# ndlongvn/MM-DTI

Measured on AMD Instinct MI355X. Metric: molecules/sec fwd+bwd (InfoNCE fine-tune), higher is better.
Workload: dtype fp16 forward / bf16 backward GEMM operands, fp32 accumulation

## Files before the change

### include/mmdti_hip.h

```cpp
#ifndef MMDTI_HIP_H
#define MMDTI_HIP_H

#ifdef __cplusplus
extern "C" {
#endif

typedef void* mmdti_stream_t;

#define MMDTI_OK 0
#define MMDTI_ERR_INVALID 1
#define MMDTI_ERR_LAUNCH 2

#define MMDTI_ACT_NONE 0
#define MMDTI_ACT_GELU 1
#define MMDTI_ACT_GELU_BWD 2
#define MMDTI_ACT_GELU_G 4
#define MMDTI_ACT_MUL_AUX 5

#define MMDTI_DT_F32 0
#define MMDTI_DT_BF16 1
#define MMDTI_DT_F32_ATOMIC 2
#define MMDTI_DT_F16 3
#define MMDTI_DT_AB_F16 16
#define MMDTI_DT_B_F16 32
// ... 105 lines not shown
                               float p_hid, float p_att, unsigned long long seed, unsigned int site_att, unsigned int site_o,
                               unsigned int site_f, const float* dout, float* ds1, float* ds2, const float* key_add,
                               const int* q_off, const int* k_off, const int* k_cnt, int q_rows, const void* q, const void* kv,
                               const float* stats, const float* y, const float* am, const float* ar, const void* u_aux,
                               int act_dx, const float* z, const float* zm, const float* zr, const void* w_q, const void* w_kv,
                               const void* w_o, const void* w_i, const void* w_o2, const float* g_ln1, const float* g_ln2,
                               float* db_o, float* db_o2, float* dg_ln1, float* dbt_ln1, float* dg_ln2, float* dbt_ln2, void* dzb,
                               void* du, void* dyb, void* dq, void* dkv, void* ws, long long ws_bytes);
int mmdti_bert_stack_layout(int Mq, int D, int F, long long stats_bytes, long long nrow, long long dw_slab_bytes, long long* out);
int mmdti_bert_stack_fwd(mmdti_stream_t stream, int nl, int Mq, int B, int L, int heads, int D, int F, float scale, float p_hid,
                         float p_att, unsigned long long seed, unsigned int site0, const float* s1_32_0, const void* s1_16_0,
                         const float* key_add, const int* q_off, const int* k_off, const int* k_cnt, int q_rows,
                         const void* const* params, int act_fwd, float eps, int ln_max_k, void* arena, long long arena_bytes,
                         long long stats_bytes, float* out32_last, int fwd_f16);
int mmdti_bert_stack_bwd(mmdti_stream_t stream, int nl, int Mq, int B, int L, int heads, int D, int F, float scale, float p_hid,
                         float p_att, unsigned long long seed, unsigned int site0, const float* dout, float* ds1_final,
                         const void* s1_16_0, const float* key_add, const int* q_off, const int* k_off, const int* k_cnt,
                         int q_rows, const void* const* bparams, int act_dx, void* const* grads, int lddw_qkv, const void* arena,
                         long long arena_bytes, long long stats_bytes, void* ws, long long ws_bytes, long long dw_slab_bytes,
                         int fwd_f16);


int mmdti_layernorm_fwd(mmdti_stream_t stream, const float* x, const float* gamma, const float* beta, float eps,
                        int rows, int D, float* y_f32, void* y_bf16, float* mean, float* rstd,
                        const unsigned char* row_zero, float drop_p, unsigned long long seed, unsigned int site,
                        int y16_f16 );
int mmdti_layernorm_bwd(mmdti_stream_t stream, const void* dy, int dy_dtype, const float* dy_add, const float* x, const float* gamma,
                        const float* mean, const float* rstd, int rows, int D, const float* dres, float* dx,
                        float* dgamma, float* dbeta, const unsigned char* row_zero, float drop_p,
                        unsigned long long seed, unsigned int site, void* dx_bf16, float drop2_p, unsigned int site2,
                        float* dx_colsum);

int mmdti_colsum_bf16(mmdti_stream_t stream, const void* x_bf16, int rows, int cols, int ld, float* out);
int mmdti_cast_f32_bf16(mmdti_stream_t stream, const float* x, void* y_bf16, long long n, float drop_p,
                        unsigned long long seed, unsigned int site);
int mmdti_cast_bf16_f32(mmdti_stream_t stream, const void* x_bf16, float* y, long long n);
int mmdti_cast_f32_f16(mmdti_stream_t stream, const float* x, void* y_f16, long long n, float drop_p, unsigned long long seed,
                       unsigned int site);
int mmdti_cast_f16_bf16(mmdti_stream_t stream, const void* x_f16, int rows, int cols, int ldx, void* y_bf16);
int mmdti_dropout_f32(mmdti_stream_t stream, const float* x, float* y, long long n, float drop_p,
                      unsigned long long seed, unsigned int site);
int mmdti_axpy_f32(mmdti_stream_t stream, const float* x, float* y, long long n, float a);

int mmdti_embedding_fwd(mmdti_stream_t stream, const long long* ids, const float* table, long long n, int D,
                        int vocab, float* out, int accumulate);
int mmdti_embedding_bwd(mmdti_stream_t stream, const long long* ids, const float* dout, long long n, int D,
                        int vocab, long long padding_idx, float* dtable);
int mmdti_embedding_fwd3(mmdti_stream_t stream, const long long* ids_a, const float* table_a, int vocab_a, const long long* ids_b,
                         const float* table_b, int vocab_b, const long long* ids_c, const float* table_c, int vocab_c, long long n, int D,
                         float* out);
int mmdti_onehot_bf16(mmdti_stream_t stream, const long long* ids, long long n, int vocab, int ld, long long padding_idx,
                      void* out_bf16);
int mmdti_roberta_position_ids(mmdti_stream_t stream, const long long* ids, int B, int L, long long pad_idx,
                               long long* out);

int mmdti_gbf_features_fwd(mmdti_stream_t stream, const float* dist, const long long* edge_type, const float* mul,
                           const float* bias, const float* means, const float* stds, long long P, int K, int E,
                           void* feat_bf16);
int mmdti_gbf_features_bwd(mmdti_stream_t stream, const float* dist, const long long* edge_type, const float* mul,
                           const float* bias, const float* means, const float* stds, long long P, int K, int E,
                           const void* dfeat_bf16, float* dmul, float* dbias, float* dmeans, float* dstds);
int mmdti_gbf_bias_fwd(mmdti_stream_t stream, const float* dist, const void* edge_type,
                       int edge_bytes , const float* mul,
                       const float* bias, const float* means, const float* stds, const void* w1_bf16, const float* b1,
                       const void* w2_bf16, const float* b2, int B, int N, int ld, int K, int F, int H, int E, void* out,
                       void* feat_bf16, void* u_bf16, void* h_bf16, int flags ,
                       const int* tile_prefix ,
                       const int* row_blocks );
int mmdti_gbf_bias_bwd(mmdti_stream_t stream, const void* g, const float* dist, const void* edge_type, int edge_bytes,
                       const float* mul, const float* bias, const float* means, const float* stds, const void* w1_bf16,
                       const void* w2_bf16, const void* u_bf16, int B, int N, int ld, int K, int F, int H, int E, int flags,
                       void* do_bf16, void* du_bf16, float* dmul, float* dbias, float* dmeans, float* dstds);
int mmdti_gbf_bias_bwd_full(mmdti_stream_t stream, const void* g, const float* dist, const void* edge_type, int edge_bytes,
                            const float* mul, const float* bias, const float* means, const float* stds, const void* w1_bf16,
                            const float* b1, const void* w2_bf16, int B, int N, int ld, int K, int F, int H, int E, int flags,
                            float* dw1, float* db1, float* dw2, float* db2, float* dmul, float* dbias, float* dmeans, float* dstds,
                            const int* tile_prefix ,
                            const int* row_blocks ,
                            void* workspace ,
                            long long workspace_bytes);
int mmdti_gbf_bias_bwd_full_workspace(int E);
int mmdti_pair_permute_fwd(mmdti_stream_t stream, const float* x, float* out, int B, int N, int H, int ld);
int mmdti_pair_permute_bwd(mmdti_stream_t stream, const float* g, void* out_bf16, int B, int N, int H, int ld, int tiled);

int mmdti_pair_attn_fwd(mmdti_stream_t stream, const void* qkv_bf16, const void* bias_in, void* s_out,
                        void* o_bf16, const unsigned char* key_pad, int B, int N, int H, int ld, float scale,
                        float drop_p, unsigned long long seed, unsigned int site, int layout,
                        const int* key_tiles ,
                        int rag_store,
                        const int* row_off ,
                        int qkv_f16 );
int mmdti_pair_attn_bwd(mmdti_stream_t stream, const void* qkv_bf16, const void* s, const void* do_bf16, void* g,
                        void* dqkv_bf16, int B, int N, int H, int ld, float scale, int g_in_zero, float drop_p,
                        unsigned long long seed, unsigned int site, int layout, const int* key_tiles,
                        const int* row_off ,
                        int qkv_f16 );

int mmdti_softmax_fwd(mmdti_stream_t stream, const float* s, const float* key_add, void* p_bf16, void* pd_bf16,
                      int B, int heads, int Lq, int Lk, int ld, float drop_p, unsigned long long seed,
                      unsigned int site);
int mmdti_softmax_bwd(mmdti_stream_t stream, const void* p_bf16, const float* dp, void* ds_bf16, int B, int heads,
                      int Lq, int Lk, int ld, float scale, float drop_p, unsigned long long seed,
                      unsigned int site);

int mmdti_attn_fwd(mmdti_stream_t stream, const void* q_bf16, const void* k_bf16, const void* v_bf16,
                   const float* key_add, void* ctx_bf16, float* stats, int B, int heads, int Lq, int Lk, int head_dim,
                   int ldq, int ldk, int ldo, float scale, float drop_p, unsigned long long seed, unsigned int site,
                   const int* q_off, const int* k_off, const int* k_cnt, int q_rows ,
                   int ctx_f16 );
int mmdti_attn_bwd(mmdti_stream_t stream, const void* q_bf16, const void* k_bf16, const void* v_bf16,
                   const float* key_add, const void* dctx_bf16, const float* stats, float* drow, void* dq_bf16,
                   void* dk_bf16, void* dv_bf16, int B, int heads, int Lq, int Lk, int head_dim, int ldq, int ldk, int ldo,
                   int lddq, int lddk, float scale, float drop_p, unsigned long long seed, unsigned int site,
                   const int* q_off, const int* k_off, const int* k_cnt, int q_rows );
int mmdti_attn_long_fwd(mmdti_stream_t stream, const void* q_bf16, const void* k_bf16, const void* v_bf16,
                        const float* key_add, void* ctx_bf16, float* stats, int B, int heads, int Lq, int Lk, int head_dim,
                        int ldq, int ldk, int ldo, float scale, float drop_p, unsigned long long seed, unsigned int site,
                        const int* q_off, const int* k_off, const int* k_cnt, int q_rows, int ctx_f16);
int mmdti_attn_long_bwd(mmdti_stream_t stream, const void* q_bf16, const void* k_bf16, const void* v_bf16,
                        const float* key_add, const void* dctx_bf16, const float* stats, float* drow, void* dq_bf16,
                        void* dk_bf16, void* dv_bf16, int B, int heads, int Lq, int Lk, int head_dim, int ldq, int ldk, int ldo,
                        int lddq, int lddk, float scale, float drop_p, unsigned long long seed, unsigned int site,
                        const int* q_off, const int* k_off, const int* k_cnt, int q_rows);

int mmdti_gelu_fwd_bf16(mmdti_stream_t stream, const void* u_bf16, void* y_bf16, long long n);

int mmdti_seq_mean_fwd(mmdti_stream_t stream, const void* x_bf16, int B, int S, int D, int ld, float* out);
int mmdti_seq_mean_bwd(mmdti_stream_t stream, const float* dout, int B, int S, int D, int ld, void* dx_bf16, const void* aux_bf16,
                       int ld_aux, int aux_mode);
int mmdti_seq_mean_packed_fwd(mmdti_stream_t stream, const void* x_bf16, int B, int S, int D, int ld, const int* row_off,
                              const int* n_real, float* out);
int mmdti_seq_mean_packed_bwd(mmdti_stream_t stream, const float* dout, int rows, int S, int D, int ld, const int* row_off,
                              const int* n_real, const int* row_seq, void* dx_bf16, const void* aux_bf16, int ld_aux, int aux_mode);
int mmdti_l2norm_fwd(mmdti_stream_t stream, const float* x, int B, int D, int ldx, float* xhat, float* inv_norm);
int mmdti_l2norm_bwd(mmdti_stream_t stream, const float* dxhat, const float* xhat, const float* inv_norm, int B,
                     int D, int ldx, float* dx);
int mmdti_infonce_dir(mmdti_stream_t stream, const float* qh_all, const float* kh_all, int Bg, int D, int row0,
                      int Bl, float temperature, float* loss_sum, float* dq_all, float* dk_all, float* scratch);

int mmdti_ct_loss_fwd(mmdti_stream_t stream, int mode, const float* fhat, int B, int D, const float* labels_f,
                      const long long* labels_i, int C, const float* pred, const float* weights, float w, float t,
                      float e, float coef, float* loss, float* G,
                      float* row_ws );
int mmdti_ct_loss_bwd(mmdti_stream_t stream, const float* fhat, const float* G, int B, int D, float t, float* dfhat);

int mmdti_fds_bins(mmdti_stream_t stream, const float* labels, int n, float min_value, float bin_width,
                   int bucket_start, int bucket_num, int* bins, int* flags);
int mmdti_fds_smooth(mmdti_stream_t stream, const float* x, const int* bins, const int* flags, int n, int D,
                     int bucket_start, int bucket_num, const float* m1, const float* v1, const float* m2,
                     const float* v2, float* y, float* scale_out);
int mmdti_fds_update_stats(mmdti_stream_t stream, const float* feats, const int* bins, const int* flags, int n,
                           int D, int bucket_start, int bucket_num, float factor, float* running_mean,
                           float* running_var, float* num_samples_tracked);
int mmdti_fds_smooth_stats(mmdti_stream_t stream, const float* stat, int nb, int D, const float* window, int ks,
                           float* out);

int mmdti_masked_pool_fwd(mmdti_stream_t stream, const float* a, const float* t, const unsigned char* mask_a,
                          const unsigned char* mask_t, int B, int Na, int Nt, int D, float* pooled);
int mmdti_masked_pool_bwd(mmdti_stream_t stream, const float* dpooled, const unsigned char* mask_a,
                          const unsigned char* mask_t, int B, int Na, int Nt, int D, float* da, float* dt);

int mmdti_masked_pool_packed_fwd(mmdti_stream_t stream, const float* a, const float* t, const int* a_off, const int* a_cnt,
                                 const int* t_off, const int* t_cnt, int B, int D, float* pooled);
int mmdti_masked_pool_packed_bwd(mmdti_stream_t stream, const float* dpooled, const int* a_off, const int* a_cnt, const int* a_seq,
                                 int rows_a, const int* t_off, const int* t_cnt, const int* t_seq, int rows_t, int D, float* da,
                                 float* dt);
// ... 40 lines not shown
```

### mm-dti_amd/csrc/common.h

```cpp
#pragma once
#include <hip/hip_runtime.h>
#include <stdint.h>
#include <math.h>

#include "../../include/mmdti_hip.h"

namespace mmdti {

typedef uint16_t bf16_t;

void set_error(const char* fmt, ...);
#define MMDTI_REQUIRE(cond, ...)                 \
  do {                                           \
    if (!(cond)) {                               \
      ::mmdti::set_error(__VA_ARGS__);           \
      return MMDTI_ERR_INVALID;                  \
    }                                            \
  } while (0)
#define MMDTI_LAUNCH_CHECK()                                              \
  do {                                                                    \
    hipError_t e__ = hipGetLastError();                                   \
    if (e__ != hipSuccess) {                                              \
      ::mmdti::set_error("%s:%d launch failed: %s", __FILE__, __LINE__,   \
                         hipGetErrorString(e__));                         \
// ... 16 lines not shown
  return __builtin_bit_cast(uint32_t, v);
}
__device__ __forceinline__ uint16_t f2h_sat(float f) { return (uint16_t)(f2h_sat2(f, f) & 0xffffu); }
__device__ __forceinline__ uint4 h2bf8(const uint4& u) {
  typedef _Float16 f16x8_t __attribute__((ext_vector_type(8)));
  typedef __bf16 bf16x8_t __attribute__((ext_vector_type(8)));
  const f16x8_t h = __builtin_bit_cast(f16x8_t, u);
  bf16x8_t o;
#pragma unroll
  for (int e = 0; e < 8; ++e) o[e] = (__bf16)(float)h[e];
  return __builtin_bit_cast(uint4, o);
}

template <int CTRL, int ROW_MASK = 0xf, int BANK_MASK = 0xf, bool BOUND_ZERO = true>
__device__ __forceinline__ float dpp_f32(float old, float src) {
  return __int_as_float(__builtin_amdgcn_update_dpp(__float_as_int(old), __float_as_int(src), CTRL, ROW_MASK, BANK_MASK, BOUND_ZERO));
}
constexpr int DPP_ROW_SHL = 0x100, DPP_ROW_SHR = 0x110, DPP_ROW_ROR = 0x120, DPP_ROW_BCAST15 = 0x142, DPP_ROW_BCAST31 = 0x143;
constexpr int DPP_QUAD_XOR1 = 0xB1, DPP_QUAD_XOR2 = 0x4E;

__device__ __forceinline__ float wave_sum(float v) {
  v += dpp_f32<DPP_ROW_SHR + 1>(0.f, v);
  v += dpp_f32<DPP_ROW_SHR + 2>(0.f, v);
  v += dpp_f32<DPP_ROW_SHR + 4>(0.f, v);
  v += dpp_f32<DPP_ROW_SHR + 8>(0.f, v);
  v += dpp_f32<DPP_ROW_BCAST15, 0xa>(0.f, v);
  v += dpp_f32<DPP_ROW_BCAST31, 0xc>(0.f, v);
  return __int_as_float(__builtin_amdgcn_readlane(__float_as_int(v), 63));
}
__device__ __forceinline__ float wave_max(float v) {
  const float NI = -INFINITY;
  v = fmaxf(v, dpp_f32<DPP_ROW_SHR + 1, 0xf, 0xf, false>(NI, v));
  v = fmaxf(v, dpp_f32<DPP_ROW_SHR + 2, 0xf, 0xf, false>(NI, v));
  v = fmaxf(v, dpp_f32<DPP_ROW_SHR + 4, 0xf, 0xf, false>(NI, v));
  v = fmaxf(v, dpp_f32<DPP_ROW_SHR + 8, 0xf, 0xf, false>(NI, v));
  v = fmaxf(v, dpp_f32<DPP_ROW_BCAST15, 0xa, 0xf, false>(NI, v));
  v = fmaxf(v, dpp_f32<DPP_ROW_BCAST31, 0xc, 0xf, false>(NI, v));
  return __int_as_float(__builtin_amdgcn_readlane(__float_as_int(v), 63));
}
__device__ __forceinline__ float wave_sum8_scatter(const float (&v)[8], int lane) {
  const bool b0 = lane & 1, b1 = lane & 2, b2 = lane & 4;
  float a[4];
#pragma unroll
  for (int i = 0; i < 4; ++i) {
    const float keep = b0 ? v[2 * i + 1] : v[2 * i];
    const float send = b0 ? v[2 * i] : v[2 * i + 1];
    a[i] = keep + dpp_f32<DPP_QUAD_XOR1>(0.f, send);
  }
  float b[2];
#pragma unroll
  for (int i = 0; i < 2; ++i) {
    const float keep = b1 ? a[2 * i + 1] : a[2 * i];
    const float send = b1 ? a[2 * i] : a[2 * i + 1];
    b[i] = keep + dpp_f32<DPP_QUAD_XOR2>(0.f, send);
  }
  const float keep = b2 ? b[1] : b[0];
  const float send = b2 ? b[0] : b[1];
  const float up = dpp_f32<DPP_ROW_SHL + 4>(0.f, send);
  const float dn = dpp_f32<DPP_ROW_SHR + 4>(0.f, send);
  float c = keep + (b2 ? dn : up);
  c += dpp_f32<DPP_ROW_ROR + 8>(0.f, c);
  c += __shfl_xor(c, 16, 64);
  c += __shfl_xor(c, 32, 64);
  return c;
}

struct Rand4 {
  uint32_t x, y, z, w;
};
static __device__ unsigned long long g_seed_salt = 0ull;
__device__ __forceinline__ uint64_t salted(uint64_t seed) { return seed ^ g_seed_salt; }
#define MMDTI_DEFINE_SALT_PULL(TU)                                                                                   \
  namespace mmdti {                                                                                                  \
  __global__ void seed_salt_pull_kernel_##TU(const unsigned long long* __restrict__ src) { g_seed_salt = *src; }     \
  void salt_pull_##TU(hipStream_t s, const unsigned long long* src) {                                                \
    hipLaunchKernelGGL(seed_salt_pull_kernel_##TU, dim3(1), dim3(1), 0, s, src);                                     \
  }                                                                                                                  \
  }
void salt_pull_gemm(hipStream_t s, const unsigned long long* src);
void salt_pull_layernorm(hipStream_t s, const unsigned long long* src);
void salt_pull_pair_attn(hipStream_t s, const unsigned long long* src);
void salt_pull_pair_attn_bwd(hipStream_t s, const unsigned long long* src);
void salt_pull_pair_attn_bwd_g16(hipStream_t s, const unsigned long long* src);
void salt_pull_attn(hipStream_t s, const unsigned long long* src);
void salt_pull_elementwise(hipStream_t s, const unsigned long long* src);
__device__ __forceinline__ uint32_t mix32(uint32_t x) {
  x ^= x >> 16; x *= 0x7feb352du; x ^= x >> 15; x *= 0x846ca68bu; x ^= x >> 16;
  return x;
}
__device__ __forceinline__ Rand4 philox4(uint64_t seed, uint32_t site, uint64_t ctr) {
  seed = salted(seed);
  const uint32_t k = mix32((uint32_t)seed ^ (site * 0x9E3779B9u)) ^ (uint32_t)(seed >> 32);
  const uint32_t a = mix32(((uint32_t)ctr ^ k) + (uint32_t)(ctr >> 32) * 0x85EBCA6Bu);
  const uint32_t b = mix32(a ^ 0xB5297A4Du);
  return Rand4{a << 16, a & 0xffff0000u, b << 16, b & 0xffff0000u};
}
__device__ __forceinline__ bool dropout_keep(uint64_t seed, uint32_t site, uint64_t idx, uint32_t thresh) {
  Rand4 r = philox4(seed, site, idx >> 2);
  uint32_t w = (idx & 3) == 0 ? r.x : (idx & 3) == 1 ? r.y : (idx & 3) == 2 ? r.z : r.w;
  return w >= thresh;
}
struct Rng24 {
  uint32_t k1, k2;
};
__device__ __forceinline__ Rng24 rng24_key(uint64_t seed, uint32_t site, uint32_t plane) {
  seed = salted(seed);
  const uint32_t a = mix32((mix32((uint32_t)seed ^ (site * 0x9E3779B9u)) ^ (uint32_t)(seed >> 32)) + plane * 0x85EBCA6Bu);
  return Rng24{a, mix32(a ^ 0xB5297A4Du)};
}
__device__ __forceinline__ uint32_t rng24_word(const Rng24& k, uint32_t ctr) {
  uint32_t h = __umul24(ctr ^ k.k1, 0x9E3779u);
  h = h ^ (h >> 12) ^ k.k2;
  h = __umul24(h, 0x85EBCBu);
  return h ^ (h >> 12);
}
__device__ __forceinline__ uint32_t rng24_row_t8(const Rng24& k, uint32_t row, uint32_t thresh8) {
  return (thresh8 >> 16) + ((rng24_word(k, row | 0x800000u) & 0xffffu) < (thresh8 & 0xffffu) ? 1u : 0u);
}
__device__ __forceinline__ bool rng24_kept(uint32_t word, int r, uint32_t t8) { return ((word >> (8 * r)) & 0xffu) >= t8; }
static inline uint32_t dropout_thresh8(float p) {
  if (!(p > 0.f)) return 0u;
  const double x = (double)p * 256.0;
  uint32_t t8 = (uint32_t)x, fr = (uint32_t)((x - (double)t8) * 65536.0 + 0.5);
  if (fr >= 65536u) { t8 += 1; fr = 0; }
  return (t8 << 16) | fr;
}
static inline uint32_t dropout_thresh(float p) {
  if (p <= 0.f) return 0u;
  double t = (double)p * 4294967296.0;
  if (t >= 4294967295.0) return 0xFFFFFFFFu;
  return (uint32_t)t;
}

__host__ __device__ __forceinline__ int pair_n4(int N) { return (N + 3) & ~3; }
__host__ __device__ __forceinline__ long long pair_plane(int N) { return ((long long)N * pair_n4(N) + 7) & ~7ll; }
__host__ __device__ __forceinline__ long long pair_off(int N, int i, int j) {
  const int q0 = i & ~15, vr = N - q0 < 16 ? N - q0 : 16;
  return (long long)q0 * pair_n4(N) + vr * (j & ~3) + ((i & 15) << 2) + (j & 3);
}

__device__ __forceinline__ float fast_erf(float x) {
  const float ax = fabsf(x);
  const float t = __builtin_amdgcn_rcpf(1.0f + 0.3275911f * ax);
  const float poly = ((((1.061405429f * t - 1.453152027f) * t + 1.421413741f) * t - 0.284496736f) * t + 0.254829592f) * t;
  const float r = 1.0f - poly * __expf(-ax * ax);
  return copysignf(r, x);
}
__device__ __forceinline__ float gelu_erf(float x) { return x * 0.5f * (1.0f + fast_erf(x * 0.70710678118654752440f)); }
__device__ __forceinline__ float gelu_erf_grad(float x) {
  const float kInvSqrt2Pi = 0.39894228040143267794f;
  const float ax = fabsf(x) * 0.70710678118654752440f;
  const float t = __builtin_amdgcn_rcpf(1.0f + 0.3275911f * ax);
  const float poly = ((((1.061405429f * t - 1.453152027f) * t + 1.421413741f) * t - 0.284496736f) * t + 0.254829592f) * t;
  const float e = __expf(-ax * ax);
  const float erfv = copysignf(1.0f - poly * e, x);
  return 0.5f * (1.0f + erfv) + x * kInvSqrt2Pi * e;
}

__device__ __forceinline__ int xcd_chunk(int orig, int nwg) {
  const int q = nwg >> 3, r = nwg & 7, xcd = orig & 7;
  return (xcd < r ? xcd * (q + 1) : r * (q + 1) + (xcd - r) * q) + (orig >> 3);
}

__device__ __forceinline__ void gelu_erf_both(float x, float& y, float& dy) {
  const float kInvSqrt2Pi = 0.39894228040143267794f;
  const float ax = fabsf(x) * 0.70710678118654752440f;
// ... 54 lines not shown
```

### mm-dti_amd/csrc/elementwise.hip

```cpp
#include "common.h"
#include <stdarg.h>
#include <stdio.h>

namespace mmdti {

static thread_local char g_err[512] = "";
void set_error(const char* fmt, ...) {
  va_list ap;
  va_start(ap, fmt);
  vsnprintf(g_err, sizeof(g_err), fmt, ap);
  va_end(ap);
}

static inline int grid_for(long long n, int per_block) {
  long long b = (n + per_block - 1) / per_block;
  if (b > 256 * 16) b = 256 * 16;
  if (b < 1) b = 1;
  return (int)b;
}

__device__ __forceinline__ bf16_t f2h16(float f) { return f2h_sat(f); }

template <bool F16>
__global__ __launch_bounds__(256) void cast_f32_bf16_kernel(const float* __restrict__ x, bf16_t* __restrict__ y,
// ... 813 lines not shown
  return MMDTI_OK;
}

extern "C" int mmdti_adam_step(mmdti_stream_t stream, float* p, const float* g, float* m, float* v, void* p_bf16,
                               long long n, float lr, float beta1, float beta2, float eps, float weight_decay,
                               int step, const float* grad_scale_dev, const float* step_state_dev, void* p_f16) {
  MMDTI_REQUIRE(p && g && m && v && n > 0 && (step >= 1 || step_state_dev), "adam_step: bad arguments");
  float bc1, bc2s;
  adam_bias_host(beta1, beta2, step, &bc1, &bc2s);
  hipLaunchKernelGGL(adam_kernel<false>, dim3(grid_for(n, 256 * 4)), dim3(256), 0, (hipStream_t)stream, p, g, m, v,
                     (bf16_t*)p_bf16, (bf16_t*)p_f16, n, lr, beta1, beta2, eps, weight_decay, bc1, bc2s, grad_scale_dev, step_state_dev, nullptr);
  MMDTI_LAUNCH_CHECK();
  return MMDTI_OK;
}

extern "C" int mmdti_sumsq_check_f32(mmdti_stream_t stream, const float* g, long long n, float* out, float* ws, int ws_floats, float* guard,
                                     const float* bias_table, int table_steps, float beta1, float beta2) {
  MMDTI_REQUIRE(g && out && ws && n > 0 && ws_floats >= 2, "sumsq_check_f32: bad arguments");
  MMDTI_REQUIRE(aligned16(g), "sumsq_check_f32: 16-byte alignment required");
  MMDTI_REQUIRE(!bias_table || table_steps >= 1, "sumsq_check_f32: empty bias-correction table");
  const int wgs = (int)min((long long)min(ws_floats / 2, SUMSQ_WGS), (n / 4 + 255) / 256 + 1);
  unsigned* cnt = reinterpret_cast<unsigned*>(ws + wgs);
  hipLaunchKernelGGL(sumsq_part_kernel<true>, dim3(wgs), dim3(256), 0, (hipStream_t)stream, g, n, ws, cnt);
  hipLaunchKernelGGL(sumsq_fold_kernel<true>, dim3(1), dim3(256), 0, (hipStream_t)stream, ws, wgs, out, cnt, guard, bias_table,
                     table_steps, beta1, beta2);
  MMDTI_LAUNCH_CHECK();
  return MMDTI_OK;
}

extern "C" int mmdti_adam_step_guarded(mmdti_stream_t stream, float* p, const float* g, float* m, float* v, void* p_bf16, long long n,
                                       float lr, float beta1, float beta2, float eps, float weight_decay, const float* grad_scale_dev,
                                       const float* step_state_dev, void* p_f16, const float* guard) {
  MMDTI_REQUIRE(p && g && m && v && n > 0 && guard, "adam_step_guarded: bad arguments");
  hipLaunchKernelGGL(adam_kernel<true>, dim3(grid_for(n, 256 * 4)), dim3(256), 0, (hipStream_t)stream, p, g, m, v,
                     (bf16_t*)p_bf16, (bf16_t*)p_f16, n, lr, beta1, beta2, eps, weight_decay, 1.f, 1.f, grad_scale_dev, step_state_dev,
                     guard);
  MMDTI_LAUNCH_CHECK();
  return MMDTI_OK;
}

extern "C" int mmdti_adam_step_masked(mmdti_stream_t stream, float* p, const float* g, float* m, float* v, void* p_bf16, long long n,
                                      float lr, float beta1, float beta2, float eps, float weight_decay, int step,
                                      const float* grad_scale_dev, const float* step_state_dev, void* p_f16, const float* guard,
                                      const unsigned char* skip) {
  MMDTI_REQUIRE(p && g && m && v && n > 0 && skip && (guard || step >= 1 || step_state_dev), "adam_step_masked: bad arguments");
  if (guard) {
    hipLaunchKernelGGL((adam_kernel<true, true>), dim3(grid_for(n, 256 * 4)), dim3(256), 0, (hipStream_t)stream, p, g, m, v,
                       (bf16_t*)p_bf16, (bf16_t*)p_f16, n, lr, beta1, beta2, eps, weight_decay, 1.f, 1.f, grad_scale_dev, step_state_dev,
                       guard, skip);
  } else {
    float bc1, bc2s;
    adam_bias_host(beta1, beta2, step, &bc1, &bc2s);
    hipLaunchKernelGGL((adam_kernel<false, true>), dim3(grid_for(n, 256 * 4)), dim3(256), 0, (hipStream_t)stream, p, g, m, v,
                       (bf16_t*)p_bf16, (bf16_t*)p_f16, n, lr, beta1, beta2, eps, weight_decay, bc1, bc2s, grad_scale_dev, step_state_dev,
                       nullptr, skip);
  }
  MMDTI_LAUNCH_CHECK();
  return MMDTI_OK;
}

extern "C" int mmdti_adam_bias_table(float beta1, float beta2, int steps, float* table_host) {
  MMDTI_REQUIRE(table_host && steps >= 1, "adam_bias_table: bad arguments");
  for (int t = 1; t <= steps; ++t) adam_bias_host(beta1, beta2, t, &table_host[2 * (t - 1)], &table_host[2 * (t - 1) + 1]);
  return MMDTI_OK;
}

extern "C" int mmdti_step_state_advance(mmdti_stream_t stream, float* state, unsigned long long* salt, float base_lr, int warmup_steps,
                                        int total_steps, float beta1, float beta2) {
  MMDTI_REQUIRE(state && salt, "step_state_advance: null pointer");
  MMDTI_REQUIRE(total_steps > 0 && warmup_steps >= 0, "step_state_advance: bad schedule");
  hipLaunchKernelGGL(step_state_advance_kernel, dim3(1), dim3(1), 0, (hipStream_t)stream, state, salt, base_lr, warmup_steps, total_steps, beta1, beta2);
  MMDTI_LAUNCH_CHECK();
  return MMDTI_OK;
}

extern "C" int mmdti_seed_salt_pull(mmdti_stream_t stream, const unsigned long long* salt) {
  MMDTI_REQUIRE(salt != nullptr, "seed_salt_pull: null pointer");
  hipStream_t s = (hipStream_t)stream;
  salt_pull_gemm(s, salt);
  salt_pull_layernorm(s, salt);
  salt_pull_pair_attn(s, salt);
  salt_pull_pair_attn_bwd(s, salt);
  salt_pull_pair_attn_bwd_g16(s, salt);
  salt_pull_attn(s, salt);
  salt_pull_elementwise(s, salt);
  MMDTI_LAUNCH_CHECK();
  return MMDTI_OK;
}

extern "C" int mmdti_probe_tr_read(mmdti_stream_t stream, int row_stride_elems, unsigned short* out) {
  MMDTI_REQUIRE(out && row_stride_elems >= 16 && row_stride_elems <= 64 && row_stride_elems % 4 == 0, "probe_tr_read: bad stride");
  hipLaunchKernelGGL(probe_tr_kernel, dim3(1), dim3(64), 0, (hipStream_t)stream, row_stride_elems, out);
  MMDTI_LAUNCH_CHECK();
  return MMDTI_OK;
}
```

### mm-dti_amd/csrc/gbf.hip

```cpp
#include "common.h"

namespace mmdti {

constexpr float GBF_A = 2.5066272160f;

__global__ __launch_bounds__(256) void gbf_fwd_kernel(const float* __restrict__ dist, const long long* __restrict__ et,
                                                      const float* __restrict__ mul, const float* __restrict__ bias,
                                                      const float* __restrict__ means, const float* __restrict__ stds,
                                                      long long P, int K, int E, bf16_t* __restrict__ feat) {
  const int kc = threadIdx.x & 15;
  const int pl = threadIdx.x >> 4;
  for (int k0 = kc * 8; k0 < K; k0 += 128) {
    float mu[8], sg[8], cf[8];
#pragma unroll
    for (int i = 0; i < 8; ++i) {
      mu[i] = means[k0 + i];
      sg[i] = fabsf(stds[k0 + i]) + 1e-5f;
      cf[i] = 1.0f / (GBF_A * sg[i]);
    }
    for (long long p = (long long)blockIdx.x * 16 + pl; p < P; p += (long long)gridDim.x * 16) {
      long long e = et[p];
      e = e < 0 ? 0 : (e >= E ? E - 1 : e);
      const float y = mul[e] * dist[p] + bias[e];
      uint32_t w[4];
#pragma unroll
      for (int i = 0; i < 4; ++i) {
        float z0 = (y - mu[2 * i]) / sg[2 * i], z1 = (y - mu[2 * i + 1]) / sg[2 * i + 1];
        float v0 = __expf(-0.5f * z0 * z0) * cf[2 * i], v1 = __expf(-0.5f * z1 * z1) * cf[2 * i + 1];
        w[i] = (uint32_t)f2bf(v0) | ((uint32_t)f2bf(v1) << 16);
      }
      *reinterpret_cast<uint4*>(feat + p * K + k0) = make_uint4(w[0], w[1], w[2], w[3]);
    }
  }
}

constexpr int GBF_MAXE = 4096;

__global__ __launch_bounds__(256) void gbf_bwd_kernel(const float* __restrict__ dist, const long long* __restrict__ et,
                                                      const float* __restrict__ mul, const float* __restrict__ bias,
                                                      const float* __restrict__ means, const float* __restrict__ stds,
                                                      long long P, int K, int E, const bf16_t* __restrict__ dfeat,
                                                      float* __restrict__ dmul, float* __restrict__ dbias,
                                                      float* __restrict__ dmeans, float* __restrict__ dstds) {
  extern __shared__ float hist[];
  const bool use_hist = E <= GBF_MAXE;
  if (use_hist) {
    for (int i = threadIdx.x; i < 2 * E; i += 256) hist[i] = 0.f;
    __syncthreads();
  }
  const int kc = threadIdx.x & 15, pl = threadIdx.x >> 4;
  for (int kb = 0; kb < K; kb += 128) {
    const int k0 = kb + kc * 8;
    const bool kact = k0 < K;
    float mu[8], sg[8], cf[8], amu[8], asg[8];
#pragma unroll
    for (int i = 0; i < 8; ++i) {
      mu[i] = kact ? means[k0 + i] : 0.f;
      sg[i] = kact ? fabsf(stds[k0 + i]) + 1e-5f : 1.f;
      cf[i] = 1.0f / (GBF_A * sg[i]);
      amu[i] = asg[i] = 0.f;
    }
    for (long long p0 = (long long)blockIdx.x * 16; p0 < P; p0 += (long long)gridDim.x * 16) {
      const long long p = p0 + pl;
      float dy = 0.f;
      long long e = 0;
      float d = 0.f;
      if (p < P && kact) {
        e = et[p];
        e = e < 0 ? 0 : (e >= E ? E - 1 : e);
        d = dist[p];
        const float y = mul[e] * d + bias[e];
        const uint4 u = *reinterpret_cast<const uint4*>(dfeat + p * K + k0);
        const uint32_t w[4] = {u.x, u.y, u.z, u.w};
#pragma unroll
        for (int i = 0; i < 8; ++i) {
          const float dv = __uint_as_float((i & 1) ? (w[i >> 1] & 0xffff0000u) : (w[i >> 1] << 16));
          const float z = (y - mu[i]) / sg[i];
          const float val = __expf(-0.5f * z * z) * cf[i];
          const float t = dv * val;
          const float zs = z / sg[i];
          dy -= t * zs;
          amu[i] += t * zs;
          asg[i] += t * (z * zs - 1.0f / sg[i]);
// ... 41 lines not shown
  const float* src = x + (long long)bi * N * H;
  const int HP = H + 1;
  for (int t = threadIdx.x; t < N * H; t += 256) tile[(t / H) * HP + (t % H)] = src[t];
  __syncthreads();
  for (int t = threadIdx.x; t < H * N; t += 256) {
    const int h = t / N, j = t - h * N;
    out[(((long long)b * H + h) * N + i) * ld + j] = tile[j * HP + h];
  }
}

__global__ __launch_bounds__(256) void pair_permute_bwd_kernel(const float* __restrict__ g, bf16_t* __restrict__ out,
                                                               int N, int H, int ld, int tiled) {
  extern __shared__ float tile[];
  const int bi = blockIdx.x, b = bi / N, i = bi - b * N;
  const int NP = N | 1;
  for (int t = threadIdx.x; t < H * N; t += 256) {
    const int h = t / N, j = t - h * N;
    const long long off = tiled ? (long long)(b * H + h) * pair_plane(N) + pair_off(N, i, j) : (((long long)b * H + h) * N + i) * ld + j;
    tile[h * NP + j] = g[off];
  }
  __syncthreads();
  bf16_t* dst = out + (long long)bi * N * H;
  for (int t = threadIdx.x; t < N * H; t += 256) {
    const int j = t / H, h = t - j * H;
    dst[t] = f2bf(tile[h * NP + j]);
  }
}

typedef __bf16 gbf16x8 __attribute__((ext_vector_type(8)));
typedef float gf32x4 __attribute__((ext_vector_type(4)));
constexpr int GBF_K = 128, GBF_F = 128, GBF_H = 64;
constexpr int GBF_WS = 136;

__device__ __forceinline__ gbf16x8 gbf_pack8(const float* v) {
  gbf16x8 r;
#pragma unroll
  for (int e = 0; e < 8; ++e) r[e] = (__bf16)v[e];
  return r;
}
__device__ __forceinline__ uint2 gbf_pack4(const gf32x4& a) {
  uint2 pk;
  pk.x = (uint32_t)f2bf(a[0]) | ((uint32_t)f2bf(a[1]) << 16);
  pk.y = (uint32_t)f2bf(a[2]) | ((uint32_t)f2bf(a[3]) << 16);
  return pk;
}

__device__ __forceinline__ int gbf_edge(const void* et, long long base, unsigned off, int esz) {
  const char* pb = reinterpret_cast<const char*>(et) + base * esz;
  const unsigned bo = off * (unsigned)esz;
  const int w = *reinterpret_cast<const int*>(pb + (bo & ~3u));
  return esz == 2 ? (int)(short)(w >> ((bo & 2u) * 8u)) : w;
}
__device__ __forceinline__ int gbf_edge(const void* et, long long p, int esz) { return gbf_edge(et, p, 0u, esz); }

typedef float gf32x2 __attribute__((ext_vector_type(2)));
constexpr float GBF_SQ = 0.84932180028801907f;

__device__ __forceinline__ gbf16x8 gbf_basis8(float y, const float* mu, const float* isq, const float* cf) {
  const gf32x4 m0 = *reinterpret_cast<const gf32x4*>(mu), m1 = *reinterpret_cast<const gf32x4*>(mu + 4);
  const gf32x4 s0 = *reinterpret_cast<const gf32x4*>(isq), s1 = *reinterpret_cast<const gf32x4*>(isq + 4);
  const gf32x4 c0 = *reinterpret_cast<const gf32x4*>(cf), c1 = *reinterpret_cast<const gf32x4*>(cf + 4);
  const gf32x2 yy = {y, y};
  float v[8];
#define GBF_B2(M, S, C, LO, OUT)                                                       \
  {                                                                                    \
    const gf32x2 z = (yy - gf32x2{M[LO], M[LO + 1]}) * gf32x2{S[LO], S[LO + 1]};       \
    const gf32x2 q = -(z * z);                                                         \
    const gf32x2 e = {__builtin_amdgcn_exp2f(q[0]), __builtin_amdgcn_exp2f(q[1])};     \
    const gf32x2 r = e * gf32x2{C[LO], C[LO + 1]};                                     \
    v[OUT] = r[0]; v[OUT + 1] = r[1];                                                  \
  }
  GBF_B2(m0, s0, c0, 0, 0) GBF_B2(m0, s0, c0, 2, 2) GBF_B2(m1, s1, c1, 0, 4) GBF_B2(m1, s1, c1, 2, 6)
#undef GBF_B2
  return gbf_pack8(v);
}

constexpr int GBF_FWD_MAXE = 4096;
__device__ __forceinline__ void gbf_put(float* p, float v) { *p = v; }
__device__ __forceinline__ void gbf_put(_Float16* p, float v) { *p = (_Float16)fminf(v, 65504.f); }
__device__ __forceinline__ float gbf_get(const float* p) { return *p; }
__device__ __forceinline__ float gbf_get(const __bf16* p) {
  return __builtin_bit_cast(float, (uint32_t)(*reinterpret_cast<const unsigned short*>(p)) << 16);
}

template <bool SAVE, bool TILED, typename OT>
__global__ __launch_bounds__(512, 2) void gbf_bias_fwd_kernel(const float* __restrict__ dist, const void* __restrict__ et, int esz,
                                                              const float* __restrict__ mul, const float* __restrict__ bias,
                                                              const float* __restrict__ means, const float* __restrict__ stds,
                                                              const bf16_t* __restrict__ W1, const float* __restrict__ b1,
                                                              const bf16_t* __restrict__ W2, const float* __restrict__ b2,
                                                              OT* __restrict__ out, bf16_t* __restrict__ feat_out,
                                                              bf16_t* __restrict__ u_out, bf16_t* __restrict__ h_out, int B, int N,
                                                              int ld, int E, int tpm, int ugrad, int ltab,
                                                              const int* __restrict__ tile_prefix, const int* __restrict__ row_blocks) {
  static_assert(TILED || sizeof(OT) == 4, "compact pair planes exist in the tiled layout only");
  extern __shared__ __attribute__((aligned(16))) unsigned char gbf_smem[];
  bf16_t* sW1 = reinterpret_cast<bf16_t*>(gbf_smem);
  bf16_t* sW2 = sW1 + GBF_F * GBF_WS;
  float* sMu = reinterpret_cast<float*>(sW2 + GBF_H * GBF_WS);
  float* sIq = sMu + GBF_K;
  float* sCf = sIq + GBF_K;
  float* sB1 = sCf + GBF_K;
  float* sB2 = sB1 + GBF_F;
  float* sMul = sB2 + GBF_H;
  float* sBia = sMul + E;
  const int tid = threadIdx.x, lane = tid & 63;
  for (int c = tid; c < GBF_F * (GBF_K / 8); c += 512) {
    const int row = c >> 4, col = (c & 15) * 8;
    *reinterpret_cast<uint4*>(sW1 + row * GBF_WS + col) = *reinterpret_cast<const uint4*>(W1 + row * GBF_K + col);
  }
  for (int c = tid; c < GBF_H * 32; c += 512) {
    const int row = c >> 5, pc = c & 31, u = pc >> 3, g = (pc >> 1) & 3, hf = pc & 1;
    *reinterpret_cast<uint2*>(sW2 + row * GBF_WS + 32 * u + 8 * g + 4 * hf) =
        *reinterpret_cast<const uint2*>(W2 + row * GBF_F + 32 * u + 16 * hf + 4 * g);
  }
  if (tid < GBF_K) {
    const float sg = fabsf(stds[tid]) + 1e-5f;
    sMu[tid] = means[tid];
    sIq[tid] = GBF_SQ / sg;
    sCf[tid] = 1.0f / (GBF_A * sg);
    sB1[tid] = b1[tid];
    if (tid < GBF_H) sB2[tid] = b2[tid];
  }
  if (ltab)
    for (int c = tid; c < E; c += 512) {
      sMul[c] = mul[c];
      sBia[c] = bias[c];
    }
  __syncthreads();
  const int g = lane >> 4, i = lane & 15;
  const bool rag = TILED && tile_prefix != nullptr;
  const int ntiles = rag ? tile_prefix[B] : B * tpm;
  const int nwaves = (int)gridDim.x * 8;
  int b_run = 0;
  const int nblk = (N + 3) >> 2;
  const long long plane = TILED ? pair_plane(N) : (long long)N * ld;
  auto fetch = [&](int tile, int& b, int& q, int& flags, unsigned& pl, int& e, float& d) {
    tile = __builtin_amdgcn_readfirstlane(tile < ntiles ? tile : ntiles - 1);
    int tq;
    if (rag) {
      while (b_run + 1 < B && tile >= tile_prefix[b_run + 1]) ++b_run;
      b = b_run;
      tq = tile - tile_prefix[b];
    } else {
      b = (int)((unsigned)tile / (unsigned)tpm);
      tq = tile - b * tpm;
    }
    int ii, jj;
    bool inplane = true, past = false;
    if (TILED) {
      const int rbk = (rag && row_blocks) ? row_blocks[b] : nblk;
      const int cb = (int)((unsigned)tq / (unsigned)rbk), rb = tq - cb * rbk;
      past = 4 * rb >= N || 4 * cb >= N;
      ii = 4 * rb + (i >> 2);
      jj = 4 * cb + (i & 3);
      inplane = ii < N;
      q = (int)pair_off(N, inplane ? ii : 0, jj);
    } else {
      q = tq * 16 + i;
      ii = (int)((unsigned)q / (unsigned)ld);
      jj = q - ii * ld;
      inplane = q < plane;
    }
    const bool valid = ii < N && jj < N;
    flags = (valid ? 1 : 0) | (inplane ? 2 : 0) | (past ? 4 : 0);
    pl = (unsigned)((valid ? ii : 0) * N + (valid ? jj : 0));
// ... 218 lines not shown
    float dy = 0.f;
#pragma unroll
    for (int kt = 0; kt < 8; ++kt) {
      gf32x4 acc = {0.f, 0.f, 0.f, 0.f};
#pragma unroll
      for (int u = 0; u < 4; ++u) {
        const gbf16x8 wf = *reinterpret_cast<const gbf16x8*>(sW1T + (16 * kt + i) * GBF_WS + 32 * u + 8 * g);
        acc = __builtin_amdgcn_mfma_f32_16x16x32_bf16(wf, uB[u], acc, 0, 0, 0);
      }
      const gf32x4 mu = *reinterpret_cast<const gf32x4*>(sMu + 16 * kt + 4 * g);
      const gf32x4 is = *reinterpret_cast<const gf32x4*>(sIs + 16 * kt + 4 * g);
      const gf32x4 cf = *reinterpret_cast<const gf32x4*>(sCf + 16 * kt + 4 * g);
#pragma unroll
      for (int r = 0; r < 4; ++r) {
        const float dvr = __uint_as_float(((uint32_t)f2bf(acc[r])) << 16);
        const float z = (y - mu[r]) * is[r];
        const float val = __expf(-0.5f * z * z) * cf[r];
        const float t = valid ? dvr * val : 0.f;
        const float zs = z * is[r];
        dy -= t * zs;
        amu[kt][r] += t * zs;
        asg[kt][r] += t * (z * zs - is[r]);
      }
      __builtin_amdgcn_sched_barrier(0);
    }
    dy += __shfl_xor(dy, 16, 64);
    dy += __shfl_xor(dy, 32, 64);
    if (g == 0 && valid) {
      atomicAdd(&hist[e], dy * d);
      atomicAdd(&hist[E + e], dy);
    }
    }
    act = n_act; valid = n_valid; p = n_p; e = n_e; d = n_d;
#pragma unroll
    for (int j = 0; j < 16; ++j) gv[j] = n_gv[j];
#pragma unroll
    for (int j = 0; j < 8; ++j) upre[j] = n_up[j];
  }
#pragma unroll
  for (int kt = 0; kt < 8; ++kt)
#pragma unroll
    for (int r = 0; r < 4; ++r) {
      float a = amu[kt][r], sgv = asg[kt][r];
      a += __shfl_xor(a, 1, 64); a += __shfl_xor(a, 2, 64); a += __shfl_xor(a, 4, 64); a += __shfl_xor(a, 8, 64);
      sgv += __shfl_xor(sgv, 1, 64); sgv += __shfl_xor(sgv, 2, 64); sgv += __shfl_xor(sgv, 4, 64); sgv += __shfl_xor(sgv, 8, 64);
      if (i == 0) {
        const int k = 16 * kt + 4 * g + r;
        atomicAdd(dmeans + k, a);
        atomicAdd(dstds + k, stds[k] < 0.f ? -sgv : sgv);
      }
    }
  __syncthreads();
  for (int c = tid; c < E; c += 256) {
    const float a = hist[c], bb = hist[E + c];
    if (a != 0.f) atomicAdd(dmul + c, a);
    if (bb != 0.f) atomicAdd(dbias + c, bb);
  }
}

constexpr int GBF_LW = 144;
constexpr int GBF_FULL_MAXE = 1536;
constexpr int GBF_SLAB_B1 = GBF_F * GBF_K + GBF_H * GBF_F, GBF_SLAB_B2 = GBF_SLAB_B1 + GBF_F, GBF_SLAB_MU = GBF_SLAB_B2 + GBF_H,
              GBF_SLAB_SG = GBF_SLAB_MU + GBF_K, GBF_SLAB = GBF_SLAB_SG + GBF_K;
constexpr size_t gbf_full_smem(int E) {
  return (size_t)(GBF_F * GBF_LW + GBF_F * GBF_W2S + 2 * 128 * GBF_LW) * 2 + (size_t)(4 * GBF_K + GBF_F + 2 * 128 + 4 * E) * 4;
}

typedef short gs16x4 __attribute__((ext_vector_type(4)));
typedef short gs16x8 __attribute__((ext_vector_type(8)));
typedef __attribute__((address_space(3))) gs16x4 glds_s16x4;
__device__ __forceinline__ gbf16x8 gbf_tr8(const bf16_t* a0, const bf16_t* a1) {
  const gs16x4 lo = __builtin_amdgcn_ds_read_tr16_b64_v4i16((glds_s16x4*)a0);
  const gs16x4 hi = __builtin_amdgcn_ds_read_tr16_b64_v4i16((glds_s16x4*)a1);
  const gs16x8 v = __builtin_shufflevector(lo, hi, 0, 1, 2, 3, 4, 5, 6, 7);
  return __builtin_bit_cast(gbf16x8, v);
}

template <bool TILED, typename GT>
__global__ __launch_bounds__(512, 1) void gbf_bias_bwd_full_kernel(
    const GT* __restrict__ gsrc, const float* __restrict__ dist, const void* __restrict__ et, int esz, const float* __restrict__ mul,
    const float* __restrict__ bias, const float* __restrict__ means, const float* __restrict__ stds, const bf16_t* __restrict__ W1,
    const float* __restrict__ b1, const bf16_t* __restrict__ W2, float* __restrict__ dW1, float* __restrict__ db1, float* __restrict__ dW2,
    float* __restrict__ db2, float* __restrict__ dmul, float* __restrict__ dbias, float* __restrict__ dmeans, float* __restrict__ dstds, int B,
    int N, int ld, int E, int tpm, const int* __restrict__ tile_prefix, const int* __restrict__ row_blocks, float* __restrict__ slab) {
  extern __shared__ __attribute__((aligned(16))) unsigned char gbf_smem[];
  bf16_t* sW1 = reinterpret_cast<bf16_t*>(gbf_smem);
  bf16_t* sW2T = sW1 + GBF_F * GBF_LW;
  bf16_t* T0 = sW2T + GBF_F * GBF_W2S;
  bf16_t* T1 = T0 + 128 * GBF_LW;
  float* sMu = reinterpret_cast<float*>(T1 + 128 * GBF_LW);
  float* sIs = sMu + GBF_K;
  float* sCf = sIs + GBF_K;
  float* sIq = sCf + GBF_K;
  float* sB1 = sIq + GBF_K;
  float* sY = sB1 + GBF_F;
  float* sDy = sY + 128;
  float* hist = sDy + 128;
  float* sMul = hist + 2 * E;
  float* sBia = sMul + E;
  const int tid = threadIdx.x, lane = tid & 63, wave = tid >> 6;
  for (int c = tid; c < E; c += 512) {
    sMul[c] = mul[c];
    sBia[c] = bias[c];
  }
  for (int c = tid; c < GBF_F * (GBF_K / 8); c += 512) {
    const int row = c >> 4, col = (c & 15) * 8;
    *reinterpret_cast<uint4*>(sW1 + row * GBF_LW + col) = *reinterpret_cast<const uint4*>(W1 + row * GBF_K + col);
  }
  for (int c = tid; c < GBF_H * GBF_F; c += 512) {
    const int h = c >> 7, f = c & 127;
    sW2T[f * GBF_W2S + h] = W2[c];
  }
  if (tid < GBF_K) {
    const float sg = fabsf(stds[tid]) + 1e-5f;
    sMu[tid] = means[tid];
    sIs[tid] = 1.0f / sg;
    sCf[tid] = 1.0f / (GBF_A * sg);
    sIq[tid] = GBF_SQ / sg;
    sB1[tid] = b1[tid];
    sDy[tid] = 0.f;
  }
  for (int c = tid; c < 2 * E; c += 512) hist[c] = 0.f;
  __syncthreads();
  const int g = lane >> 4, i = lane & 15;
  const int ploc = 16 * wave + i;
  const int pswz = ((ploc >> 3) & 1) << 6;
#define GBF_SWZ(lo, hi, c) ((c) < 64 ? (lo) + (c) : (hi) + ((c) - 64))
  bf16_t* const r0lo = T0 + ploc * GBF_LW + pswz;
  bf16_t* const r0hi = T0 + ploc * GBF_LW + (64 ^ pswz);
  bf16_t* const r1lo = r0lo + 128 * GBF_LW;
  bf16_t* const r1hi = r0hi + 128 * GBF_LW;
  const int tswz = (g & 1) << 6;
  const int trow = (8 * g + (i >> 2)) * GBF_LW + 4 * (i & 3);
  const bf16_t* const t0lo = T0 + trow + tswz;
  const bf16_t* const t0hi = T0 + trow + (64 ^ tswz);
  const bf16_t* const t1lo = t0lo + 128 * GBF_LW;
  const bf16_t* const t1hi = t0hi + 128 * GBF_LW;
  const bf16_t* const t0w = T0 + trow + ((16 * wave) ^ tswz);
  const bf16_t* const t1w = t0w + 128 * GBF_LW;
  const int rswz = ((i >> 3) & 1) << 6;
  const bf16_t* const d1lo = T1 + i * GBF_LW + 8 * g + rswz;
  const bf16_t* const d1hi = T1 + i * GBF_LW + 8 * g + (64 ^ rswz);
  unsigned o_w1row = (unsigned)(i * GBF_LW + 8 * g) * 2;
  unsigned o_w2row = (unsigned)(GBF_F * GBF_LW + i * GBF_W2S + 8 * g) * 2;
  unsigned o_w1tr = (unsigned)((8 * g + (i >> 2)) * GBF_LW + 16 * wave + 4 * (i & 3)) * 2;
  const unsigned o_f32 = (unsigned)(GBF_F * GBF_LW + GBF_F * GBF_W2S + 2 * 128 * GBF_LW) * 2;
  unsigned o_gconst = o_f32 + (unsigned)(8 * g) * 4;
  unsigned o_b1row = o_f32 + (unsigned)(4 * GBF_K + 4 * g) * 4;
  unsigned o_kconst = o_f32 + (unsigned)(16 * wave + 4 * g) * 4;
  const bool rag = TILED && tile_prefix != nullptr;
  const int ntiles = rag ? tile_prefix[B] : B * tpm;
  int b_run = 0;
  const int nb = (N + 3) >> 2;
  const long long plane = TILED ? pair_plane(N) : (long long)N * ld;
  gf32x4 amu = {0.f, 0.f, 0.f, 0.f}, asg = {0.f, 0.f, 0.f, 0.f};
  gf32x4 aW1[8], aW2[4], aB1 = {0.f, 0.f, 0.f, 0.f}, aB2 = {0.f, 0.f, 0.f, 0.f};
#pragma unroll
  for (int t = 0; t < 8; ++t) aW1[t] = gf32x4{0.f, 0.f, 0.f, 0.f};
#pragma unroll
  for (int t = 0; t < 4; ++t) aW2[t] = gf32x4{0.f, 0.f, 0.f, 0.f};
  const gs16x8 o16 = {0x3F80, 0x3F80, 0x3F80, 0x3F80, 0x3F80, 0x3F80, 0x3F80, 0x3F80};
  const gbf16x8 ones = __builtin_bit_cast(gbf16x8, o16);

  auto fetch = [&](int tile, bool& act, bool& valid, float& d, int& e, float (&gv)[16]) {
    tile = __builtin_amdgcn_readfirstlane(tile);
    act = tile < ntiles;
    tile = act ? tile : ntiles - 1;
    int b, tq;
    if (rag) {
      while (b_run + 1 < B && tile >= tile_prefix[b_run + 1]) ++b_run;
      b = b_run;
      tq = tile - tile_prefix[b];
    } else {
      b = (int)((unsigned)tile / (unsigned)tpm);
      tq = tile - b * tpm;
    }
    int q, ii, jj;
    if (TILED) {
      const int rbk = (rag && row_blocks) ? row_blocks[b] : nb;
      const int cb = (int)((unsigned)tq / (unsigned)rbk), rb = tq - cb * rbk;
      ii = 4 * rb + (i >> 2);
      jj = 4 * cb + (i & 3);
      q = (int)pair_off(N, ii < N ? ii : 0, jj);
    } else {
      q = tq * 16 + i;
      ii = (int)((unsigned)q / (unsigned)ld);
      jj = q - ii * ld;
    }
    valid = act && ii < N && jj < N;
    const long long mol = (long long)b * N * N;
    const unsigned pl = (unsigned)((valid ? ii : 0) * N + (valid ? jj : 0));
    const int e32 = gbf_edge(et, mol, pl, esz);
    e = e32 < 0 ? 0 : (e32 >= E ? E - 1 : e32);
    d = (dist + mol)[pl];
    const GT* mb = gsrc + (long long)b * GBF_H * plane;
    const unsigned voff = (unsigned)(8 * g) * (unsigned)plane + (unsigned)(valid ? q : 0);
#pragma unroll
    for (int c = 0; c < 2; ++c)
#pragma unroll
      for (int j = 0; j < 8; ++j) gv[c * 8 + j] = gbf_get(mb + (long long)(32 * c + j) * plane + voff);
  };

  bool act, valid, n_act, n_valid;
  float d, n_d, gv[16], n_gv[16];
  int e, n_e;
  const int stride = (int)gridDim.x * 8;
  int tile = (int)blockIdx.x * 8 + wave;
  fetch(tile, act, valid, d, e, gv);
  for (int base = (int)blockIdx.x * 8; base < ntiles; base += stride, tile += stride) {
    asm volatile("" : "+v"(o_w1row), "+v"(o_w2row), "+v"(o_w1tr), "+v"(o_gconst), "+v"(o_b1row), "+v"(o_kconst));
    const bf16_t* w1row = reinterpret_cast<const bf16_t*>(gbf_smem + o_w1row);
    const bf16_t* w2row = reinterpret_cast<const bf16_t*>(gbf_smem + o_w2row);
    const bf16_t* w1tr = reinterpret_cast<const bf16_t*>(gbf_smem + o_w1tr);
    const float* gconst = reinterpret_cast<const float*>(gbf_smem + o_gconst);
    const float* b1row = reinterpret_cast<const float*>(gbf_smem + o_b1row);
    const float* kconst = reinterpret_cast<const float*>(gbf_smem + o_kconst);
    fetch(tile + stride, n_act, n_valid, n_d, n_e, n_gv);
    constexpr bool SPLIT_G = sizeof(GT) == 4;
    gbf16x8 oB[2], oL[2], hB[4];
    if (!valid) {
#pragma unroll
      for (int j = 0; j < 16; ++j) gv[j] = 0.f;
    }
    oB[0] = gbf_pack8(gv);
    oB[1] = gbf_pack8(gv + 8);
    if constexpr (SPLIT_G) {
      float lo[16];
#pragma unroll
      for (int j = 0; j < 16; ++j) lo[j] = gv[j] - (float)oB[j >> 3][j & 7];
      oL[0] = gbf_pack8(lo);
      oL[1] = gbf_pack8(lo + 8);
    }
    const float y = sMul[e] * d + sBia[e];
    if (g == 0) sY[ploc] = y;
    if (act) {
      gbf16x8 fB[4];
#pragma unroll
      for (int c = 0; c < 4; ++c) {
        const float* gc = gconst + 32 * c;
        fB[c] = gbf_basis8(y, gc, gc + 3 * GBF_K, gc + 2 * GBF_K);
        *reinterpret_cast<gbf16x8*>(GBF_SWZ(r0lo, r0hi, 32 * c) + 8 * g) = fB[c];
      }
#pragma unroll
      for (int u = 0; u < 4; ++u) {
        gf32x4 hv[2];
#pragma unroll
        for (int hf = 0; hf < 2; ++hf) {
          const int ft = 2 * u + hf;
          gf32x4 acc = {0.f, 0.f, 0.f, 0.f}, ua = {0.f, 0.f, 0.f, 0.f};
#pragma unroll
          for (int c = 0; c < 2; ++c) {
            const gbf16x8 wf = *reinterpret_cast<const gbf16x8*>(w2row + 16 * ft * GBF_W2S + 32 * c);
            acc = __builtin_amdgcn_mfma_f32_16x16x32_bf16(wf, oB[c], acc, 0, 0, 0);
            if constexpr (SPLIT_G) acc = __builtin_amdgcn_mfma_f32_16x16x32_bf16(wf, oL[c], acc, 0, 0, 0);
          }
#pragma unroll
          for (int c = 0; c < 4; ++c) {
            const gbf16x8 wf = *reinterpret_cast<const gbf16x8*>(w1row + 16 * ft * GBF_LW + 32 * c);
            ua = __builtin_amdgcn_mfma_f32_16x16x32_bf16(wf, fB[c], ua, 0, 0, 0);
          }
          ua += *reinterpret_cast<const gf32x4*>(b1row + 16 * ft);
          {
            f32x2_t y0, g0, y1, g1;
            gelu_erf_both2(f32x2_t{ua[0], ua[1]}, y0, g0);
            gelu_erf_both2(f32x2_t{ua[2], ua[3]}, y1, g1);
            hv[hf] = gf32x4{y0[0], y0[1], y1[0], y1[1]};
            const uint2 gb = gbf_pack4(gf32x4{g0[0], g0[1], g1[0], g1[1]});
            acc[0] *= __uint_as_float(gb.x << 16);
            acc[1] *= __uint_as_float(gb.x & 0xffff0000u);
            acc[2] *= __uint_as_float(gb.y << 16);
            acc[3] *= __uint_as_float(gb.y & 0xffff0000u);
          }
          *reinterpret_cast<uint2*>(GBF_SWZ(r1lo, r1hi, 16 * ft) + 4 * g) = gbf_pack4(acc);
          __builtin_amdgcn_sched_barrier(0);
        }
        float w[8] = {hv[0][0], hv[0][1], hv[0][2], hv[0][3], hv[1][0], hv[1][1], hv[1][2], hv[1][3]};
        hB[u] = gbf_pack8(w);
      }
    } else {
      const uint4 z4 = make_uint4(0u, 0u, 0u, 0u);
#pragma unroll
      for (int c = 0; c < 4; ++c) {
        *reinterpret_cast<uint4*>(GBF_SWZ(r0lo, r0hi, 32 * c) + 8 * g) = z4;
        *reinterpret_cast<uint4*>(GBF_SWZ(r1lo, r1hi, 32 * c) + 8 * g) = z4;
        hB[c] = __builtin_bit_cast(gbf16x8, z4);
      }
    }
    __syncthreads();
#define GBF_TFRAG(P, S) gbf_tr8((P) + 32 * (S) * GBF_LW, (P) + (32 * (S) + 4) * GBF_LW)
#pragma unroll
    for (int sstep = 0; sstep < 4; ++sstep) {
      const gbf16x8 fa = GBF_TFRAG(t1w, sstep);
      aB1 = __builtin_amdgcn_mfma_f32_16x16x32_bf16(fa, ones, aB1, 0, 0, 0);
#pragma unroll
      for (int kb = 0; kb < 8; ++kb) {
        const gbf16x8 fb = GBF_TFRAG(GBF_SWZ(t0lo, t0hi, 16 * kb), sstep);
        aW1[kb] = __builtin_amdgcn_mfma_f32_16x16x32_bf16(fa, fb, aW1[kb], 0, 0, 0);
      }
    }
    {
      gbf16x8 wfr[4];
// ... 283 lines not shown
                GBF_K, GBF_F, GBF_H, K, F, H);
  MMDTI_REQUIRE(B > 0 && N > 0 && ld >= N && ld % 4 == 0 && E > 0, "gbf_bias_fwd: bad shape");
  MMDTI_REQUIRE(aligned16(w1_bf16) && aligned16(w2_bf16) && aligned16(out), "gbf_bias_fwd: 16-byte alignment required");
  const bool save = feat_bf16 || u_bf16 || h_bf16;
  MMDTI_REQUIRE(!save || (feat_bf16 && u_bf16 && h_bf16 && aligned16(feat_bf16) && aligned16(u_bf16) && aligned16(h_bf16)),
                "gbf_bias_fwd: the three saved intermediates come together, 16-byte aligned");
  const int nb4 = (N + 3) / 4;
  const int tpm = tiled ? nb4 * nb4 : cdiv((long long)N * ld, 16);
  const long long ntiles = (long long)B * tpm;
  MMDTI_REQUIRE(ntiles < (1ll << 30) && (long long)N * N < (1ll << 30), "gbf_bias_fwd: batch too large for 32-bit tile indices");
  const int grid = (int)((ntiles + 7) / 8 < 512 ? (ntiles + 7) / 8 : 512);
  const int ltab = E <= GBF_FWD_MAXE ? 1 : 0;
  const size_t smem = (size_t)(GBF_F + GBF_H) * GBF_WS * 2 + (size_t)(3 * GBF_K + GBF_F + GBF_H + (ltab ? 2 * E : 0)) * 4;
  static bool attr_done = false;
  if (!attr_done) {
    const int cap = (int)((size_t)(GBF_F + GBF_H) * GBF_WS * 2 + (size_t)(3 * GBF_K + GBF_F + GBF_H + 2 * GBF_FWD_MAXE) * 4);
    const void* fns[6] = {reinterpret_cast<const void*>(gbf_bias_fwd_kernel<true, true, float>), reinterpret_cast<const void*>(gbf_bias_fwd_kernel<true, false, float>),
                          reinterpret_cast<const void*>(gbf_bias_fwd_kernel<false, true, float>), reinterpret_cast<const void*>(gbf_bias_fwd_kernel<false, false, float>),
                          reinterpret_cast<const void*>(gbf_bias_fwd_kernel<true, true, _Float16>), reinterpret_cast<const void*>(gbf_bias_fwd_kernel<false, true, _Float16>)};
    for (int f = 0; f < 6; ++f)
      if (hipFuncSetAttribute(fns[f], hipFuncAttributeMaxDynamicSharedMemorySize, cap) != hipSuccess) {
        set_error("gbf_bias_fwd: hipFuncSetAttribute failed");
        return MMDTI_ERR_LAUNCH;
      }
    attr_done = true;
  }
#define GBF_L(SAVE, TILED, OT)                                                                                                      \
  hipLaunchKernelGGL((gbf_bias_fwd_kernel<SAVE, TILED, OT>), dim3(grid), dim3(512), smem, (hipStream_t)stream, dist, edge_type, edge_bytes, mul, bias, \
                     means, stds, (const bf16_t*)w1_bf16, b1, (const bf16_t*)w2_bf16, b2, (OT*)out, (bf16_t*)feat_bf16, (bf16_t*)u_bf16, \
                     (bf16_t*)h_bf16, B, N, ld, E, tpm, ugrad, ltab, tile_prefix, row_blocks)
  if (compact) { if (save) GBF_L(true, true, _Float16); else GBF_L(false, true, _Float16); }
  else if (save) { if (tiled) GBF_L(true, true, float); else GBF_L(true, false, float); }
  else           { if (tiled) GBF_L(false, true, float); else GBF_L(false, false, float); }
#undef GBF_L
  MMDTI_LAUNCH_CHECK();
  return MMDTI_OK;
}

extern "C" int mmdti_gbf_bias_bwd(mmdti_stream_t stream, const void* g, const float* dist, const void* edge_type, int edge_bytes,
                                  const float* mul, const float* bias, const float* means, const float* stds,
                                  const void* w1_bf16, const void* w2_bf16, const void* u_bf16, int B, int N, int ld, int K,
                                  int F, int H, int E, int flags, void* do_bf16, void* du_bf16, float* dmul, float* dbias,
                                  float* dmeans, float* dstds) {
  const int tiled = flags & 1, ugrad = (flags >> 1) & 1, compact = (flags >> 2) & 1;
  MMDTI_REQUIRE(!compact || tiled, "gbf_bias_bwd: compact planes (flags bit 2) exist in the tiled layout only");
  MMDTI_REQUIRE(g && dist && edge_type && mul && bias && means && stds && w1_bf16 && w2_bf16 && u_bf16 && do_bf16 && du_bf16 && dmul &&
                    dbias && dmeans && dstds, "gbf_bias_bwd: null argument");
  MMDTI_REQUIRE(K == GBF_K && F == GBF_F && H == GBF_H, "gbf_bias_bwd: built for %d gaussians, %d hidden, %d heads (got %d,%d,%d)",
                GBF_K, GBF_F, GBF_H, K, F, H);
  MMDTI_REQUIRE(B > 0 && N > 0 && ld >= N && ld % 4 == 0 && E > 0 && E <= GBF_MAXE, "gbf_bias_bwd: bad shape (E <= %d)", GBF_MAXE);
  MMDTI_REQUIRE(edge_bytes_ok(edge_bytes), "gbf_bias_bwd: edge types must be int64, int32 or int16 (edge_bytes=%d)", edge_bytes);
  MMDTI_REQUIRE(aligned16(u_bf16) && aligned16(do_bf16) && aligned16(du_bf16), "gbf_bias_bwd: 16-byte alignment required");
  const int nb4 = (N + 3) / 4;
  const int tpm = tiled ? nb4 * nb4 : cdiv((long long)N * ld, 16);
  const long long ntiles = (long long)B * tpm;
  const int grid = (int)(ntiles / 4 + 1 < 1024 ? ntiles / 4 + 1 : 1024);
  const size_t smem = (size_t)GBF_K * GBF_WS * 2 + (size_t)GBF_F * GBF_W2S * 2 + (size_t)(3 * GBF_K + 4 * E) * 4;
  MMDTI_REQUIRE(smem <= 96 * 1024, "gbf_bias_bwd: %d edge types do not fit the LDS tables", E);
  static bool attr_done = false;
  if (!attr_done) {
    if (hipFuncSetAttribute(reinterpret_cast<const void*>(gbf_bias_bwd_kernel<true, float>), hipFuncAttributeMaxDynamicSharedMemorySize, 96 * 1024) != hipSuccess ||
        hipFuncSetAttribute(reinterpret_cast<const void*>(gbf_bias_bwd_kernel<false, float>), hipFuncAttributeMaxDynamicSharedMemorySize, 96 * 1024) != hipSuccess ||
        hipFuncSetAttribute(reinterpret_cast<const void*>(gbf_bias_bwd_kernel<true, __bf16>), hipFuncAttributeMaxDynamicSharedMemorySize, 96 * 1024) != hipSuccess) {
      set_error("gbf_bias_bwd: hipFuncSetAttribute failed");
      return MMDTI_ERR_LAUNCH;
    }
    attr_done = true;
  }
#define GBF_B(TILED, GT)                                                                                                      \
  hipLaunchKernelGGL((gbf_bias_bwd_kernel<TILED, GT>), dim3(grid), dim3(256), smem, (hipStream_t)stream, (const GT*)g, dist, edge_type, edge_bytes, mul, bias, \
                     means, stds, (const bf16_t*)w1_bf16, (const bf16_t*)w2_bf16, (const bf16_t*)u_bf16, (bf16_t*)do_bf16,    \
                     (bf16_t*)du_bf16, dmul, dbias, dmeans, dstds, B, N, ld, E, tpm, ugrad)
  if (compact) GBF_B(true, __bf16); else if (tiled) GBF_B(true, float); else GBF_B(false, float);
#undef GBF_B
  MMDTI_LAUNCH_CHECK();
  return MMDTI_OK;
}

extern "C" int mmdti_gbf_bias_bwd_full(mmdti_stream_t stream, const void* g, const float* dist, const void* edge_type, int edge_bytes,
                                       const float* mul, const float* bias, const float* means, const float* stds, const void* w1_bf16,
                                       const float* b1, const void* w2_bf16, int B, int N, int ld, int K, int F, int H, int E, int flags,
                                       float* dw1, float* db1, float* dw2, float* db2, float* dmul, float* dbias, float* dmeans,
                                       float* dstds, const int* tile_prefix, const int* row_blocks, void* workspace, long long workspace_bytes) {
  const int tiled = flags & 1, compact = (flags >> 2) & 1;
  MMDTI_REQUIRE(!compact || tiled, "gbf_bias_bwd_full: compact planes (flags bit 2) exist in the tiled layout only");
  MMDTI_REQUIRE(!tile_prefix || tiled, "gbf_bias_bwd_full: tile_prefix (ragged batches) needs the tiled pair layout");
  MMDTI_REQUIRE(!row_blocks || tile_prefix, "gbf_bias_bwd_full: row_blocks (packed token rows) comes with tile_prefix");
  MMDTI_REQUIRE(g && dist && edge_type && mul && bias && means && stds && w1_bf16 && b1 && w2_bf16 && dw1 && db1 && dw2 && db2 && dmul && dbias &&
                    dmeans && dstds, "gbf_bias_bwd_full: null argument");
  MMDTI_REQUIRE(edge_bytes_ok(edge_bytes), "gbf_bias_bwd_full: edge types must be int64, int32 or int16 (edge_bytes=%d)", edge_bytes);
  MMDTI_REQUIRE(K == GBF_K && F == GBF_F && H == GBF_H, "gbf_bias_bwd_full: built for %d gaussians, %d hidden, %d heads (got %d,%d,%d)",
                GBF_K, GBF_F, GBF_H, K, F, H);
  MMDTI_REQUIRE(B > 0 && N > 0 && ld >= N && ld % 4 == 0 && E > 0 && E <= GBF_FULL_MAXE, "gbf_bias_bwd_full: bad shape (E <= %d)", GBF_FULL_MAXE);
  MMDTI_REQUIRE((long long)N * ld * GBF_H < (1ll << 29) && (long long)B * N * ld / 16 < (1ll << 30), "gbf_bias_bwd_full: batch too large for 32-bit tile offsets");
  MMDTI_REQUIRE(aligned16(w1_bf16), "gbf_bias_bwd_full: W1 must be 16-byte aligned");
  const int nb = (N + 3) / 4;
  const int tpm = tiled ? nb * nb : cdiv((long long)N * ld, 16);
  const long long ntiles = (long long)B * tpm;
  const int grid = (int)((ntiles + 7) / 8 < 256 ? (ntiles + 7) / 8 : 256);
  const size_t smem = gbf_full_smem(E);
  static bool attr_done = false;
  if (!attr_done) {
    const int cap = (int)gbf_full_smem(GBF_FULL_MAXE);
    if (hipFuncSetAttribute(reinterpret_cast<const void*>(gbf_bias_bwd_full_kernel<true, float>), hipFuncAttributeMaxDynamicSharedMemorySize, cap) != hipSuccess ||
        hipFuncSetAttribute(reinterpret_cast<const void*>(gbf_bias_bwd_full_kernel<false, float>), hipFuncAttributeMaxDynamicSharedMemorySize, cap) != hipSuccess ||
        hipFuncSetAttribute(reinterpret_cast<const void*>(gbf_bias_bwd_full_kernel<true, __bf16>), hipFuncAttributeMaxDynamicSharedMemorySize, cap) != hipSuccess) {
      set_error("gbf_bias_bwd_full: hipFuncSetAttribute failed");
      return MMDTI_ERR_LAUNCH;
    }
    attr_done = true;
  }
#define GBF_FB(TILED, GT)                                                                                                          \
  hipLaunchKernelGGL((gbf_bias_bwd_full_kernel<TILED, GT>), dim3(grid), dim3(512), smem, (hipStream_t)stream, (const GT*)g, dist, edge_type, edge_bytes, mul, \
                     bias, means, stds, (const bf16_t*)w1_bf16, b1, (const bf16_t*)w2_bf16, dw1, db1, dw2, db2, dmul, dbias, dmeans, dstds, B, \
                     N, ld, E, tpm, tile_prefix, row_blocks, slab)
  const long long SL = GBF_SLAB + 2 * (long long)E;
  float* slab = (workspace && aligned16(workspace) && workspace_bytes >= (long long)grid * SL * 4) ? reinterpret_cast<float*>(workspace) : nullptr;
  if (compact) GBF_FB(true, __bf16); else if (tiled) GBF_FB(true, float); else GBF_FB(false, float);
#undef GBF_FB
  if (slab)
    hipLaunchKernelGGL(gbf_slab_reduce_kernel, dim3(cdiv(SL, 64)), dim3(256), 0, (hipStream_t)stream, slab, grid, E, dw1, db1, dw2, db2, dmul, dbias, dmeans, dstds);
  MMDTI_LAUNCH_CHECK();
  return MMDTI_OK;
}

extern "C" int mmdti_gbf_bias_bwd_full_workspace(int E) { return (int)(256ll * (GBF_SLAB + 2ll * (E > 0 ? E : 0)) * 4); }
```

### mm-dti_amd/csrc/pair_attn.h

```cpp
#pragma once
#include <type_traits>

#include "common.h"

namespace mmdti {

constexpr int HD = 8;

__device__ __forceinline__ void load8_bf16(const bf16_t* p, float (&o)[8]) {
  uint4 u = *reinterpret_cast<const uint4*>(p);
  uint32_t w[4] = {u.x, u.y, u.z, u.w};
#pragma unroll
  for (int i = 0; i < 4; ++i) {
    o[2 * i] = __uint_as_float(w[i] << 16);
    o[2 * i + 1] = __uint_as_float(w[i] & 0xffff0000u);
  }
}
__device__ __forceinline__ void store8_bf16(bf16_t* p, const float (&v)[8]) {
  uint4 u;
  u.x = (uint32_t)f2bf(v[0]) | ((uint32_t)f2bf(v[1]) << 16);
  u.y = (uint32_t)f2bf(v[2]) | ((uint32_t)f2bf(v[3]) << 16);
  u.z = (uint32_t)f2bf(v[4]) | ((uint32_t)f2bf(v[5]) << 16);
  u.w = (uint32_t)f2bf(v[6]) | ((uint32_t)f2bf(v[7]) << 16);
  *reinterpret_cast<uint4*>(p) = u;
// ... 5 lines not shown
typedef short pa_s16x4 __attribute__((ext_vector_type(4)));
typedef __bf16 pa_bf16x4 __attribute__((ext_vector_type(4)));
typedef __attribute__((address_space(3))) pa_s16x4 pa_lds_s16x4;

__device__ __forceinline__ pa_s16x4 pa_pack4(const f32x4& v) {
  pa_bf16x4 h;
  h[0] = (__bf16)v[0]; h[1] = (__bf16)v[1]; h[2] = (__bf16)v[2]; h[3] = (__bf16)v[3];
  return __builtin_bit_cast(pa_s16x4, h);
}
__device__ __forceinline__ void pa_split4(const f32x4& v, pa_s16x4& hi, pa_s16x4& lo) {
  pa_bf16x4 h;
  h[0] = (__bf16)v[0]; h[1] = (__bf16)v[1]; h[2] = (__bf16)v[2]; h[3] = (__bf16)v[3];
  f32x4 r;
  r[0] = v[0] - (float)h[0]; r[1] = v[1] - (float)h[1]; r[2] = v[2] - (float)h[2]; r[3] = v[3] - (float)h[3];
  hi = __builtin_bit_cast(pa_s16x4, h);
  lo = pa_pack4(r);
}
#define PA_MFMA16(A, B, C) __builtin_amdgcn_mfma_f32_16x16x16bf16_1k(A, B, C, 0, 0, 0)
typedef _Float16 pa_h16x4 __attribute__((ext_vector_type(4)));
template <bool F16>
__device__ __forceinline__ f32x4 pa_mfma16(const pa_s16x4& a, const pa_s16x4& b, const f32x4& c) {
  if constexpr (F16) return __builtin_amdgcn_mfma_f32_16x16x16f16(__builtin_bit_cast(pa_h16x4, a), __builtin_bit_cast(pa_h16x4, b), c, 0, 0, 0);
  else return __builtin_amdgcn_mfma_f32_16x16x16bf16_1k(a, b, c, 0, 0, 0);
}
template <bool F16>
__device__ __forceinline__ void pa_split4_t(const f32x4& v, pa_s16x4& hi, pa_s16x4& lo) {
  if constexpr (F16) {
    pa_h16x4 h, l;
#pragma unroll
    for (int r = 0; r < 4; ++r) {
      h[r] = (_Float16)v[r];
      l[r] = (_Float16)(v[r] - (float)h[r]);
    }
    hi = __builtin_bit_cast(pa_s16x4, h);
    lo = __builtin_bit_cast(pa_s16x4, l);
  } else {
    pa_split4(v, hi, lo);
  }
}
#define PA_LOG2E 1.44269504088896340736f

typedef _Float16 pa_f16x4 __attribute__((ext_vector_type(4)));
__device__ __forceinline__ f32x4 pa_load4(const float* p) { return *reinterpret_cast<const f32x4*>(p); }
__device__ __forceinline__ f32x4 pa_load4_nt(const float* p) { return __builtin_nontemporal_load(reinterpret_cast<const f32x4*>(p)); }
__device__ __forceinline__ void pa_store4_nt(float* p, f32x4 v) { __builtin_nontemporal_store(v, reinterpret_cast<f32x4*>(p)); }
__device__ __forceinline__ f32x4 pa_round4(f32x4& keep, f32x4 v) { keep = v; return v; }

__device__ __forceinline__ f32x4 pa_widen_f16(const pa_f16x4& h) {
  f32x4 v;
#pragma unroll
  for (int r = 0; r < 4; ++r) v[r] = (float)h[r];
  return v;
}
__device__ __forceinline__ pa_f16x4 pa_narrow_f16(const f32x4& v) {
  pa_f16x4 h;
#pragma unroll
  for (int r = 0; r < 4; ++r) h[r] = (_Float16)v[r];
  return h;
}
__device__ __forceinline__ f32x4 pa_load4(const _Float16* p) { return pa_widen_f16(*reinterpret_cast<const pa_f16x4*>(p)); }
__device__ __forceinline__ f32x4 pa_load4_nt(const _Float16* p) { return pa_widen_f16(__builtin_nontemporal_load(reinterpret_cast<const pa_f16x4*>(p))); }
__device__ __forceinline__ void pa_store4_nt(_Float16* p, const f32x4& v) {
  __builtin_nontemporal_store(pa_narrow_f16(v), reinterpret_cast<pa_f16x4*>(p));
}
__device__ __forceinline__ f32x4 pa_round4(pa_f16x4& keep, const f32x4& v) {
  f32x4 c;
#pragma unroll
  for (int r = 0; r < 4; ++r) c[r] = __builtin_amdgcn_fmed3f(v[r], -INFINITY, 65504.f);
  keep = pa_narrow_f16(c);
  return pa_widen_f16(keep);
}
__device__ __forceinline__ void pa_store4_nt(_Float16* p, const pa_f16x4& h) { __builtin_nontemporal_store(h, reinterpret_cast<pa_f16x4*>(p)); }

__device__ __forceinline__ f32x4 pa_widen_bf16(const pa_s16x4& h) {
  f32x4 v;
#pragma unroll
  for (int r = 0; r < 4; ++r) v[r] = __builtin_bit_cast(float, (uint32_t)(uint16_t)h[r] << 16);
  return v;
}
__device__ __forceinline__ f32x4 pa_load4(const __bf16* p) { return pa_widen_bf16(*reinterpret_cast<const pa_s16x4*>(p)); }
__device__ __forceinline__ f32x4 pa_load4_nt(const __bf16* p) { return pa_widen_bf16(__builtin_nontemporal_load(reinterpret_cast<const pa_s16x4*>(p))); }
__device__ __forceinline__ void pa_store4_nt(__bf16* p, const f32x4& v) { __builtin_nontemporal_store(pa_pack4(v), reinterpret_cast<pa_s16x4*>(p)); }

__host__ __device__ constexpr int pa_kt_step(int nt) { return nt <= 9 ? 1 : (nt <= 13 ? 2 : 4); }
__host__ __device__ constexpr int pa_kt_effective(int kt, int nt) {
  const int s = pa_kt_step(nt), k = ((kt < 1 ? 1 : kt) + s - 1) / s * s;
  return k >= nt ? nt : k;
}
template <int NT, int K, typename F>
__device__ __forceinline__ void pa_dispatch_kt(int ke, F&& f) {
  constexpr int step = pa_kt_step(NT);
  constexpr int below = (K == NT) ? ((NT - 1) / step) * step : K - step;
  if constexpr (below < 1) {
    f(std::integral_constant<int, K>{});
  } else {
    if (ke >= K) f(std::integral_constant<int, K>{});
    else pa_dispatch_kt<NT, below>(ke, f);
  }
}

}

#define PA_MAX_NT 17

static inline int check_common(const char* fn, int B, int N, int H, int ld) {
  MMDTI_REQUIRE(B > 0 && N > 0 && H > 0, "%s: B,N,H must be positive", fn);
  MMDTI_REQUIRE(N <= 320, "%s: N=%d exceeds the supported 320 atoms (+BOS/EOS)", fn, N);
  MMDTI_REQUIRE(ld >= N, "%s: ld (%d) < N (%d)", fn, ld, N);
  MMDTI_REQUIRE((long long)B * H <= 2147483647LL, "%s: grid too large", fn);
  return MMDTI_OK;
}
```

### mm-dti_amd/csrc/pair_attn_bwd.hip

```cpp
#include "pair_attn_bwd_mfma.h"

namespace mmdti {

template <int NCH>
__global__ __launch_bounds__(256) void pair_attn_bwd_kernel(const bf16_t* __restrict__ qkv, const float* __restrict__ s,
                                                            const bf16_t* __restrict__ dO, float* __restrict__ g,
                                                            bf16_t* __restrict__ dqkv, int N, int H, int ld,
                                                            float scale, int g_in_zero, uint32_t thresh, float dscale,
                                                            uint64_t seed, uint32_t site) {
  __shared__ __attribute__((aligned(16))) float sq[NCH * 64][HD];
  __shared__ __attribute__((aligned(16))) float sdo[NCH * 64][HD];
  __shared__ __attribute__((aligned(16))) float red[NCH * 64][2 * HD];
  const int bh = xcd_chunk(blockIdx.x, gridDim.x), b = bh / H, h = bh - b * H;
  const int D = H * HD, D3 = 3 * D;
  const int tid = threadIdx.x, lane = tid & 63, wave = tid >> 6;
  const bf16_t* base = qkv + (long long)b * N * D3 + h * HD;
  for (int t = tid; t < NCH * 64; t += 256) {
    float q[8] = {0, 0, 0, 0, 0, 0, 0, 0}, d_[8] = {0, 0, 0, 0, 0, 0, 0, 0};
    if (t < N) {
      load8_bf16(base + (long long)t * D3, q);
      load8_bf16(dO + ((long long)b * N + t) * D + h * HD, d_);
    }
#pragma unroll
    for (int d = 0; d < 8; ++d) {
// ... 45 lines not shown
#pragma unroll
      for (int c = 0; c < NCH; ++c) {
        const int j = c * 64 + lane;
        ns[c] = (j < N) ? s[rowoff + 4LL * ld + j] : NEG_INF;
        ng[c] = (j < N && !g_in_zero) ? g[rowoff + 4LL * ld + j] : 0.f;
      }
    }
    m = wave_max(m);
    float sum = 0.f;
#pragma unroll
    for (int c = 0; c < NCH; ++c) {
      p[c] = __expf(p[c] - m);
      sum += p[c];
    }
    const float inv = 1.0f / wave_sum(sum);
    float dl = 0.f;
#pragma unroll
    for (int c = 0; c < NCH; ++c) {
      p[c] *= inv;
      float dp = 0.f;
#pragma unroll
      for (int d = 0; d < 8; ++d) dp += dd[d] * v[c][d];
      float keepscale = 1.f;
      if (thresh) {
        const int j = c * 64 + lane;
        keepscale = dropout_keep(seed, site, ((uint64_t)bh * N + i) * ld + j, thresh) ? dscale : 0.f;
      }
      dpp[c] = dp * keepscale;
      pd[c] = p[c] * keepscale;
      dl += dpp[c] * p[c];
    }
    dl = wave_sum(dl);
    float dq[8] = {0.f, 0.f, 0.f, 0.f, 0.f, 0.f, 0.f, 0.f};
#pragma unroll
    for (int c = 0; c < NCH; ++c) {
      const int j = c * 64 + lane;
      float gg = 0.f;
      if (j < N) {
        gg = p[c] * (dpp[c] - dl) + gin[c];
        g[rowoff + j] = gg;
      }
#pragma unroll
      for (int d = 0; d < 8; ++d) {
        dq[d] += gg * k[c][d];
        dk[c][d] += gg * q[d];
        dv[c][d] += pd[c] * dd[d];
      }
    }
    const float tot = wave_sum8_scatter(dq, lane) * scale;
    if (lane < 8) dqkv[((long long)b * N + i) * D3 + h * HD + lane] = f2bf(tot);
  }
#pragma unroll
  for (int c = 0; c < NCH; ++c) {
    const int j = c * 64 + lane;
    if (j < N) {
#pragma unroll
      for (int d = 0; d < 8; ++d) {
        atomicAdd(&red[j][d], dk[c][d] * scale);
        atomicAdd(&red[j][8 + d], dv[c][d]);
      }
    }
  }
  __syncthreads();
  for (int t = tid; t < N; t += 256) {
    float a[8], c2[8];
#pragma unroll
    for (int d = 0; d < 8; ++d) {
      a[d] = red[t][d];
      c2[d] = red[t][8 + d];
    }
    bf16_t* dst = dqkv + ((long long)b * N + t) * D3 + h * HD;
    store8_bf16(dst + D, a);
    store8_bf16(dst + 2 * D, c2);
  }
}
}
MMDTI_DEFINE_SALT_PULL(pair_attn_bwd)
using namespace mmdti;

extern "C" int mmdti_pair_attn_bwd(mmdti_stream_t stream, const void* qkv_bf16, const void* s, const void* do_bf16,
                                   void* g, void* dqkv_bf16, int B, int N, int H, int ld, float scale,
                                   int g_in_zero, float drop_p, unsigned long long seed, unsigned int site, int layout,
                                   const int* key_tiles, const int* row_off, int qkv_f16) {
  const int tiled = layout & 1, compact = (layout >> 1) & 1, g16 = (layout >> 2) & 1;
  if (int e = check_common("pair_attn_bwd", B, N, H, ld)) return e;
  MMDTI_REQUIRE((layout & ~7) == 0 && (!compact || tiled) && (!g16 || compact),
                "pair_attn_bwd: layout must be 0 (row-major fp32), 1 (tiled fp32), 3 (tiled, fp16 logits) or 7 (tiled, fp16 logits, bf16 gradients)");
  MMDTI_REQUIRE(!key_tiles || compact, "pair_attn_bwd: key_tiles (ragged batches) needs the compact planes (layout 3 or 7: tiled, fp16 logits)");
  MMDTI_REQUIRE(!row_off || key_tiles, "pair_attn_bwd: packed token rows (row_off) need key_tiles");
  MMDTI_REQUIRE(!tiled || (ld % 4 == 0 && N <= 16 * PA_MAX_NT), "pair_attn_bwd: the tiled pair layout needs ld %% 4 == 0 and N <= 272");
  MMDTI_REQUIRE(qkv_bf16 && s && do_bf16 && g && dqkv_bf16, "pair_attn_bwd: null pointer");
  MMDTI_REQUIRE(aligned16(qkv_bf16) && aligned16(do_bf16) && aligned16(dqkv_bf16), "pair_attn_bwd: alignment");
  MMDTI_REQUIRE(!tiled || (aligned16(s) && aligned16(g)), "pair_attn_bwd: tiled pair tensors must be 16-byte aligned");
  const uint32_t th = dropout_thresh(drop_p);
  const uint32_t th8 = dropout_thresh8(drop_p);
  const float sc = drop_p > 0.f ? 1.f / (1.f - drop_p) : 1.f;
  dim3 grid(B * H), block(256);
  hipStream_t st = (hipStream_t)stream;
  if (ld % 4 == 0 && aligned16(s) && aligned16(g) && N <= 16 * PA_MAX_NT) {
    const int nqb = (N + 15) / 16;
    dim3 blk((nqb % 3 == 0 || nqb >= 16 || nqb == 5) ? 192 : (nqb < 4 ? 64 * nqb : 256));
#define PA_MB(NT, TL, FL, NWV, RG, ST, GT)                                                                                     \
  hipLaunchKernelGGL((pair_attn_bwd_mfma_kernel<NT, TL, FL, NWV, RG, ST, GT>), grid, blk, 0, st, (const bf16_t*)qkv_bf16,      \
                     (const ST*)s, (const bf16_t*)do_bf16, (const GT*)g, (GT*)g, (bf16_t*)dqkv_bf16, N, H, ld, scale,           \
                     g_in_zero, th8, sc, (uint64_t)seed, (uint32_t)site, key_tiles, row_off, qkv_f16)
#define PA_MBW(NT, TL, FL, RG, ST, GT)                                                      \
  do {                                                                                      \
    if (blk.x == 192) PA_MB(NT, TL, FL, 3, RG, ST, GT); else PA_MB(NT, TL, FL, 4, RG, ST, GT); \
  } while (0)
#define PA_MBT(NT)                                                                          \
  do {                                                                                      \
    if (!tiled) PA_MBW(NT, false, false, false, float, float);                              \
    else { if (nqb == NT) PA_MBW(NT, true, true, false, float, float); else PA_MBW(NT, true, false, false, float, float); } \
  } while (0)
    if (compact) {
      if (g16) pa_bwd_compact_launch_g16(nqb, grid, blk, st, qkv_bf16, s, do_bf16, g, dqkv_bf16, N, H, ld, scale, g_in_zero, th8, sc, seed, site, key_tiles, row_off, qkv_f16);
      else pa_bwd_compact_launch<float>(nqb, grid, blk, st, qkv_bf16, s, do_bf16, g, dqkv_bf16, N, H, ld, scale, g_in_zero, th8, sc, seed, site, key_tiles, row_off, qkv_f16);
    } else if (nqb <= 5) PA_MBT(5); else if (nqb <= 9) PA_MBT(9); else if (nqb <= 13) PA_MBT(13); else PA_MBT(17);
#undef PA_MBW
#undef PA_MBT
#undef PA_MB
    MMDTI_LAUNCH_CHECK();
    return MMDTI_OK;
  }
  MMDTI_REQUIRE(!qkv_f16, "pair_attn_bwd: fp16 q | k | v are read by the MFMA kernels only (ld %% 4 == 0, N <= 272, 16-byte aligned pair tensors)");
#define PA_B(NCH)                                                                                                   \
  hipLaunchKernelGGL((pair_attn_bwd_kernel<NCH>), grid, block, 0, st, (const bf16_t*)qkv_bf16, (const float*)s,    \
                     (const bf16_t*)do_bf16, (float*)g, (bf16_t*)dqkv_bf16, N, H, ld, scale, g_in_zero, th, sc,            \
                     (uint64_t)seed, (uint32_t)site)
  switch ((N + 63) / 64) {
    case 1: PA_B(1); break;
    case 2: PA_B(2); break;
    case 3: PA_B(3); break;
    case 4: PA_B(4); break;
    default: PA_B(5); break;
  }
#undef PA_B
  MMDTI_LAUNCH_CHECK();
  return MMDTI_OK;
}
```

### mm-dti_amd/csrc/pair_attn_bwd_mfma.h

```cpp
#pragma once
#include "pair_attn.h"

namespace mmdti {

template <int NT, bool TILED, bool FULL, int NW, bool RAG, typename ST, typename GT>
__global__ __launch_bounds__(64 * NW, NT > 9 ? ((NT >= 16 && NW == 3) ? 2 : 1) : 3) void pair_attn_bwd_mfma_kernel(const bf16_t* __restrict__ qkv, const ST* __restrict__ s_in,
                                                                 const bf16_t* __restrict__ dO, const GT* __restrict__ gin, GT* __restrict__ gout,
                                                                 bf16_t* __restrict__ dqkv, int N, int H, int ld, float scale,
                                                                 int g_in_zero, uint32_t thresh, float dscale, uint64_t seed,
                                                                 uint32_t site, const int* __restrict__ key_tiles,
                                                                 const int* __restrict__ row_off, int qkv_f16) {
  static_assert(TILED || (sizeof(ST) == 4 && sizeof(GT) == 4), "compact pair tensors exist in the tiled layout only");
  static_assert(!RAG || sizeof(ST) == 2, "key-tile skipping is built for the compact layout only");
  constexpr int NP = NT * 16;
  constexpr int KSTR = NP + 8;
  __shared__ __attribute__((aligned(16))) bf16_t sQ[NP * 8 + 16];
  __shared__ __attribute__((aligned(16))) bf16_t sD[NP * 8 + 16];
  __shared__ __attribute__((aligned(16))) bf16_t sV[NP * 8];
  __shared__ __attribute__((aligned(16))) bf16_t sKT[8 * KSTR];
  __shared__ __attribute__((aligned(16))) float redw[NW * NT * 2 * 128];
  __shared__ __attribute__((aligned(16))) bf16_t patch[NW][2][256];
  const int bh = xcd_chunk(blockIdx.x, gridDim.x), b = bh / H, h = bh - b * H;
  const int D = H * HD, D3 = 3 * D;
  const int tid = threadIdx.x, lane = tid & 63, wave = tid >> 6, nwaves = blockDim.x >> 6;
  const int nKB = (N + 15) >> 4;
  const int kt = RAG ? pa_kt_effective(min(__builtin_amdgcn_readfirstlane(key_tiles[b]), nKB), NT) : NT;
  const bool packed = RAG && row_off != nullptr;
  const int row0 = packed ? __builtin_amdgcn_readfirstlane(row_off[b]) : b * N;
  const int rows = packed ? __builtin_amdgcn_readfirstlane(row_off[b + 1]) - row0 : N;
  const bf16_t* base = qkv + (long long)row0 * D3 + h * HD;
  for (int t = tid; t < NP + 2; t += blockDim.x) {
    uint4 q = make_uint4(0u, 0u, 0u, 0u), kk = q, vv = q, dd = q;
    if (t < rows) {
      q = *reinterpret_cast<const uint4*>(base + (long long)t * D3);
      kk = *reinterpret_cast<const uint4*>(base + (long long)t * D3 + D);
      vv = *reinterpret_cast<const uint4*>(base + (long long)t * D3 + 2 * D);
      dd = *reinterpret_cast<const uint4*>(dO + ((long long)row0 + t) * D + h * HD);
      if (qkv_f16) { q = h2bf8(q); kk = h2bf8(kk); vv = h2bf8(vv); }
    }
    *reinterpret_cast<uint4*>(sQ + t * 8) = q;
    *reinterpret_cast<uint4*>(sD + t * 8) = dd;
    if (t < NP) {
      *reinterpret_cast<uint4*>(sV + t * 8) = vv;
      const uint32_t kw[4] = {kk.x, kk.y, kk.z, kk.w};
#pragma unroll
      for (int d = 0; d < 8; ++d) sKT[d * KSTR + t] = (bf16_t)((d & 1) ? (kw[d >> 1] >> 16) : (kw[d >> 1] & 0xffffu));
    }
  }
  for (int t = tid; t < 8 * 8; t += blockDim.x) sKT[(t >> 3) * KSTR + NP + (t & 7)] = 0;
  for (int t = tid; t < NW * NT * 2 * 128; t += blockDim.x) redw[t] = 0.f;
  __syncthreads();
  const int g = lane >> 4, c16 = lane & 15;
  const bool dlane = c16 < 8;
  const float NEG_INF = -INFINITY;
  bf16_t* pw = &patch[wave][0][0];
  const int pwr = c16 * 16 + ((g ^ ((c16 >> 3) << 1)) << 2);
  const int prd = (4 * g + (c16 >> 2)) * 16 + (((c16 & 3) ^ ((g >> 1) << 1)) << 2);
  const pa_s16x4 zero4 = {0, 0, 0, 0};
  const int nlast = nKB - 1;
  const bool colok = 4 * g < N - 16 * nlast;
  const Rng24 rk = rng24_key(seed, site, (uint32_t)bh);
  auto body = [&](int qb, auto edge_c, auto kt_c) {
    constexpr bool EDGE = decltype(edge_c)::value;
    constexpr int KT = decltype(kt_c)::value;
    const int qi = qb * 16 + c16;
    const uint32_t t8 = thresh ? rng24_row_t8(rk, (uint32_t)qi, thresh) : 0u;
    const bool qvalid = EDGE ? qi < rows : true;
    const long long rowoff = ((long long)bh * N + (qvalid ? qi : 0)) * ld;
    const int vr = EDGE ? min(16, N - qb * 16) : 16;
    const long long tbase = (long long)bh * pair_plane(N) + (long long)qb * 16 * pair_n4(N) + ((4 * g < pair_n4(N) ? g : 0) * vr + (qvalid ? c16 : 0)) * 4;
    const ST* sin_p = s_in + (TILED ? tbase : rowoff);
    const GT* gin_p = gin + (TILED ? tbase : rowoff);
    GT* gout_p = gout + (TILED ? tbase : rowoff);
    const int TSTEP = TILED ? (EDGE ? vr * 16 : 256) : 16;
    const int goff = TILED ? 0 : 4 * g;
#define PA_PRED(T) (!TILED ? (qvalid && (T) * 16 + 4 * g < N) \
                           : (qvalid && (FULL ? ((T) < NT - 1 || colok) : ((T) < nlast || ((T) == nlast && colok)))))
#define PA_FAST(T) (TILED && !EDGE && (FULL ? (T) < NT - 1 : false))
    const pa_s16x4 dob = g < 2 ? *reinterpret_cast<const pa_s16x4*>(sD + (qb * 16 + c16) * 8 + 4 * g) : zero4;
    const int trq = (qb * 16 + 4 * g + (c16 >> 2)) * 8 + 4 * (c16 & 3);
    const pa_s16x4 bD = __builtin_amdgcn_ds_read_tr16_b64_v4i16((pa_lds_s16x4*)(sD + trq));
    const pa_s16x4 bQ = __builtin_amdgcn_ds_read_tr16_b64_v4i16((pa_lds_s16x4*)(sQ + trq));
    f32x4 P[KT];
    float m = NEG_INF;
#pragma unroll
    for (int t = 0; t < KT; ++t) {
      {
        const int kcol = t * 16 + 4 * g;
        f32x4 c;
        if (PA_FAST(t)) {
          c = pa_load4_nt(sin_p + t * TSTEP + goff);
        } else {
          const bool inrow = PA_PRED(t);
          const f32x4 ld4 = pa_load4(sin_p + (inrow ? t * TSTEP + goff : 0));
          c = inrow ? ld4 : f32x4{NEG_INF, NEG_INF, NEG_INF, NEG_INF};
        }
        if (!TILED) {
#pragma unroll
          for (int r = 0; r < 4; ++r) c[r] = (kcol + r < N) ? c[r] : NEG_INF;
        }
        P[t] = c;
        m = fmaxf(fmaxf(m, c[0]), c[1]);
        m = fmaxf(fmaxf(m, c[2]), c[3]);
      }
    }
    m = fmaxf(m, __shfl_xor(m, 16, 64));
    m = fmaxf(m, __shfl_xor(m, 32, 64));
    if (m == NEG_INF) m = 0.f;
    const float mneg = -m * PA_LOG2E;
    float lsum = 0.f;
#pragma unroll
    for (int t = 0; t < KT; ++t) {
      {
#pragma unroll
        for (int r = 0; r < 4; ++r) {
          const float e = __builtin_amdgcn_exp2f(fmaf(P[t][r], PA_LOG2E, mneg));
          P[t][r] = e;
          lsum += e;
        }
      }
    }
    lsum += __shfl_xor(lsum, 16, 64);
    lsum += __shfl_xor(lsum, 32, 64);
    const float inv = lsum > 0.f ? 1.0f / lsum : 0.f;
    float dl = 0.f;
#pragma unroll
    for (int t = 0; t < KT; ++t) {
      {
        const pa_s16x4 va = g < 2 ? *reinterpret_cast<const pa_s16x4*>(sV + (t * 16 + c16) * 8 + 4 * g) : zero4;
        f32x4 dp = {0.f, 0.f, 0.f, 0.f};
        dp = PA_MFMA16(va, dob, dp);
        f32x4 pr = P[t] * inv;
        if (thresh) {
          const uint32_t kw = rng24_word(rk, ((uint32_t)qi * (uint32_t)ld + t * 16 + 4 * g) >> 2);
#pragma unroll
          for (int r = 0; r < 4; ++r) {
            const bool kp = rng24_kept(kw, r, t8);
            dp[r] = kp ? dp[r] * dscale : 0.f;
            dl += dp[r] * pr[r];
            pr[r] = kp ? pr[r] : -pr[r];
          }
        } else {
          dl += dp[0] * pr[0] + dp[1] * pr[1] + dp[2] * pr[2] + dp[3] * pr[3];
        }
        P[t] = pr;
      }
    }
    dl += __shfl_xor(dl, 16, 64);
    dl += __shfl_xor(dl, 32, 64);
    constexpr int PA_LA = 3;
    auto load_gin = [&](int t) -> f32x4 {
      if (PA_FAST(t)) {
        const f32x4 ld4 = pa_load4_nt(gin_p + (g_in_zero ? 0 : t * TSTEP + goff));
        return g_in_zero ? f32x4{0.f, 0.f, 0.f, 0.f} : ld4;
      }
      const bool inrow = PA_PRED(t) && !g_in_zero;
      const f32x4 ld4 = pa_load4(gin_p + (inrow ? t * TSTEP + goff : 0));
      return inrow ? ld4 : f32x4{0.f, 0.f, 0.f, 0.f};
    };
    f32x4 Gq[PA_LA];
#pragma unroll
    for (int t = 0; t < PA_LA && t < KT; ++t) Gq[t] = load_gin(t);
    f32x4 dq = {0.f, 0.f, 0.f, 0.f};
    const int dcol = dlane ? c16 : 0;
#pragma unroll
    for (int t = 0; t < KT; ++t) {
      const int kcol = t * 16 + 4 * g;
      const f32x4 Gin = Gq[t % PA_LA];
      if (t + PA_LA < KT) Gq[t % PA_LA] = load_gin(t + PA_LA);
      __builtin_amdgcn_sched_barrier(0);
      const pa_s16x4 va = g < 2 ? *reinterpret_cast<const pa_s16x4*>(sV + (t * 16 + c16) * 8 + 4 * g) : zero4;
      f32x4 dp = {0.f, 0.f, 0.f, 0.f};
      dp = PA_MFMA16(va, dob, dp);
      f32x4 G;
#pragma unroll
      for (int r = 0; r < 4; ++r) G[r] = fabsf(P[t][r]) * ((P[t][r] > 0.f ? dp[r] * dscale : 0.f) - dl) + Gin[r];
      if (!TILED && t * 16 + 16 > N) {
#pragma unroll
        for (int r = 0; r < 4; ++r) G[r] = (kcol + r < N) ? G[r] : 0.f;
      }
      if (EDGE && !qvalid) G = f32x4{0.f, 0.f, 0.f, 0.f};
      if (PA_FAST(t)) {
        pa_store4_nt(gout_p + t * TSTEP + goff, G);
      } else if (PA_PRED(t)) {
        pa_store4_nt(gout_p + t * TSTEP + goff, G);
      }
      f32x4 Pd;
#pragma unroll
      for (int r = 0; r < 4; ++r) Pd[r] = P[t][r] > 0.f ? P[t][r] * dscale : 0.f;
      if (EDGE && !qvalid) Pd = f32x4{0.f, 0.f, 0.f, 0.f};
      pa_s16x4 Gh, Gl, Ph, Pl;
      pa_split4(G, Gh, Gl);
      pa_split4(Pd, Ph, Pl);
      *reinterpret_cast<pa_s16x4*>(pw + pwr) = Ph;
      *reinterpret_cast<pa_s16x4*>(pw + 256 + pwr) = Gh;
      const pa_s16x4 ka = *reinterpret_cast<const pa_s16x4*>(sKT + (c16 & 7) * KSTR + t * 16 + 4 * g);
      dq = PA_MFMA16(ka, Gh, dq);
      dq = PA_MFMA16(ka, Gl, dq);
      __builtin_amdgcn_fence(__ATOMIC_RELEASE, "wavefront");
      __builtin_amdgcn_wave_barrier();
      __builtin_amdgcn_fence(__ATOMIC_ACQUIRE, "wavefront");
      const pa_s16x4 aPh = __builtin_amdgcn_ds_read_tr16_b64_v4i16((pa_lds_s16x4*)(pw + prd));
      const pa_s16x4 aGh = __builtin_amdgcn_ds_read_tr16_b64_v4i16((pa_lds_s16x4*)(pw + 256 + prd));
      __builtin_amdgcn_fence(__ATOMIC_RELEASE, "wavefront");
      __builtin_amdgcn_wave_barrier();
      __builtin_amdgcn_fence(__ATOMIC_ACQUIRE, "wavefront");
      *reinterpret_cast<pa_s16x4*>(pw + pwr) = Pl;
      *reinterpret_cast<pa_s16x4*>(pw + 256 + pwr) = Gl;
      __builtin_amdgcn_fence(__ATOMIC_RELEASE, "wavefront");
      __builtin_amdgcn_wave_barrier();
      __builtin_amdgcn_fence(__ATOMIC_ACQUIRE, "wavefront");
      const pa_s16x4 aPl = __builtin_amdgcn_ds_read_tr16_b64_v4i16((pa_lds_s16x4*)(pw + prd));
      const pa_s16x4 aGl = __builtin_amdgcn_ds_read_tr16_b64_v4i16((pa_lds_s16x4*)(pw + 256 + prd));
      float* accK = redw + ((wave * NT + t) * 2 + 0) * 128 + (g * 8 + dcol) * 4;
      float* accV = accK + 128;
      f32x4 dKt = *reinterpret_cast<const f32x4*>(accK), dVt = *reinterpret_cast<const f32x4*>(accV);
      dVt = PA_MFMA16(aPh, bD, dVt);
      dKt = PA_MFMA16(aGh, bQ, dKt);
      dVt = PA_MFMA16(aPl, bD, dVt);
      dKt = PA_MFMA16(aGl, bQ, dKt);
      if (dlane) {
        *reinterpret_cast<f32x4*>(accK) = dKt;
        *reinterpret_cast<f32x4*>(accV) = dVt;
      }
      __builtin_amdgcn_fence(__ATOMIC_RELEASE, "wavefront");
      __builtin_amdgcn_wave_barrier();
      __builtin_amdgcn_fence(__ATOMIC_ACQUIRE, "wavefront");
    }
    if (qvalid && g < 2) {
      uint2 pk;
      pk.x = (uint32_t)f2bf(dq[0] * scale) | ((uint32_t)f2bf(dq[1] * scale) << 16);
      pk.y = (uint32_t)f2bf(dq[2] * scale) | ((uint32_t)f2bf(dq[3] * scale) << 16);
      *reinterpret_cast<uint2*>(dqkv + ((long long)row0 + qi) * D3 + h * HD + 4 * g) = pk;
    }
#undef PA_PRED
#undef PA_FAST
  };
  const int nQB = packed ? (rows + 15) >> 4 : nKB;
  auto run = [&](auto kt_c) {
    for (int qb = wave; qb < nQB; qb += nwaves) {
      if (TILED && qb * 16 + 16 <= rows) body(qb, std::false_type{}, kt_c);
      else body(qb, std::true_type{}, kt_c);
    }
  };
  if constexpr (RAG) pa_dispatch_kt<NT, NT>(kt, run);
  else run(std::integral_constant<int, NT>{});
  __syncthreads();
  for (int key = tid; key < rows; key += blockDim.x) {
    const int t = key >> 4, kg = (key & 15) >> 2, r = key & 3;
    float a[8] = {0, 0, 0, 0, 0, 0, 0, 0}, c2[8] = {0, 0, 0, 0, 0, 0, 0, 0};
    for (int w = 0; w < nwaves; ++w) {
      const float* bk = redw + ((w * NT + t) * 2) * 128 + kg * 32 + r;
#pragma unroll
      for (int d = 0; d < 8; ++d) {
        a[d] += bk[d * 4];
        c2[d] += bk[128 + d * 4];
      }
    }
#pragma unroll
    for (int d = 0; d < 8; ++d) a[d] *= scale;
    bf16_t* dst = dqkv + ((long long)row0 + key) * D3 + h * HD;
    store8_bf16(dst + D, a);
    store8_bf16(dst + 2 * D, c2);
  }
}


template <typename GT>
static inline void pa_bwd_compact_launch(int nqb, dim3 grid, dim3 blk, hipStream_t st, const void* qkv_bf16, const void* s, const void* do_bf16,
                                         void* g, void* dqkv_bf16, int N, int H, int ld, float scale, int g_in_zero, uint32_t th8, float sc,
                                         unsigned long long seed, unsigned int site, const int* key_tiles, const int* row_off, int qkv_f16) {
#define PA_MBH(NT, NWV, RG)                                                                                                   \
  hipLaunchKernelGGL((pair_attn_bwd_mfma_kernel<NT, true, true, NWV, RG, _Float16, GT>), grid, blk, 0, st, (const bf16_t*)qkv_bf16, \
                     (const _Float16*)s, (const bf16_t*)do_bf16, (const GT*)g, (GT*)g, (bf16_t*)dqkv_bf16, N, H, ld, scale,    \
                     g_in_zero, th8, sc, (uint64_t)seed, (uint32_t)site, key_tiles, row_off, qkv_f16)
#define PA_MBC(NT)                                                                                   \
  case NT:                                                                                           \
    if (key_tiles) PA_MBH(NT, ((NT % 3 == 0 || NT >= 16 || NT == 5) ? 3 : 4), true);                 \
    else PA_MBH(NT, ((NT % 3 == 0 || NT >= 16 || NT == 5) ? 3 : 4), false);                          \
    break
  switch (nqb) {
    PA_MBC(1); PA_MBC(2); PA_MBC(3); PA_MBC(4); PA_MBC(5); PA_MBC(6); PA_MBC(7); PA_MBC(8); PA_MBC(9); PA_MBC(10); PA_MBC(11);
    PA_MBC(12); PA_MBC(13); PA_MBC(14); PA_MBC(15); PA_MBC(16); PA_MBC(17);
  }
#undef PA_MBC
#undef PA_MBH
}
void pa_bwd_compact_launch_g16(int nqb, dim3 grid, dim3 blk, hipStream_t st, const void* qkv_bf16, const void* s, const void* do_bf16, void* g,
                               void* dqkv_bf16, int N, int H, int ld, float scale, int g_in_zero, uint32_t th8, float sc,
                               unsigned long long seed, unsigned int site, const int* key_tiles, const int* row_off, int qkv_f16);

}
```

### mm-dti_amd/mmdti_hip/functional.py

```python
from __future__ import annotations

import ctypes
import os
import weakref

import math
from types import SimpleNamespace
from typing import List, Optional

import torch

from . import ops, paths
from .ops import BF16, F32
from .runtime import fused_views, wbf16, wfwd, gbuf, dropout_state, notify_grads_ready
from .freeze import layer_trainable, plan_tower, trainable_flags


def _lin_bwd_params(dy_bf16, x_bf16, weight, bias, rows=None, bias_done=False):
    gw = gbuf(weight)
    gb = gbuf(bias) if (bias is not None and not bias_done) else None
    if gw is not None:
        ops.linear_bwd_weight(dy_bf16, x_bf16, gw, rows=rows, db=gb if (gb is not None and gb.numel() == gw.shape[0]) else None)
        if gb is not None and gb.numel() == gw.shape[0]:
            gb = None
    if gb is not None:
        ops.colsum(dy_bf16, gb, cols=bias.numel())


def _lin_bwd_params_many(calls, raw_items=()):
    items, late = list(raw_items), []
    for args, kw in calls:
        dy, x, weight, bias = args[:4]
        rows, bias_done = kw.get("rows"), kw.get("bias_done", False)
        gw = gbuf(weight)
        gb = gbuf(bias) if (bias is not None and not bias_done) else None
        if gw is None:
            if gb is not None:
                late.append((dy, gb, bias.numel()))
            continue
        rides = gb is not None and gb.numel() == gw.shape[0]
        items.append((dy, x, gw, gb if rides else None, rows))
        if gb is not None and not rides:
            late.append((dy, gb, bias.numel()))
    if items:
        ops.linear_bwd_weight_grouped(items)
    for dy, gb, cols in late:
        ops.colsum(dy, gb, cols=cols)


LAYER_SEQ = os.environ.get("MMDTI_LAYER_SEQ", "1") != "0"
POOL_THEN_PROJECT = os.environ.get("MMDTI_INFONCE_POOL_FIRST", "1") != "0"


def _join_stream_after_backward():
    here = torch.cuda.current_stream()
    if here == torch.cuda.default_stream():
        return

    def _join(stream=here):
        cur = torch.cuda.current_stream()
        if cur != stream:
            cur.wait_stream(stream)

    torch.autograd.Variable._execution_engine.queue_callback(_join)


DEFER_WGRAD_LAYERS = int(os.environ.get("MMDTI_DEFER_WGRAD", "4"))
_wgrad_stream_obj = None
_wgrad_keep = []


def _launch_deferred_wgrads(deferred, layers):
    if not deferred:
        return
    main = torch.cuda.current_stream()
    ws = _wgrad_stream()
    ws.wait_stream(main)
    with torch.cuda.stream(ws):
        for group in deferred:
            _lin_bwd_params_many(group)
        for layer in layers:
            notify_grads_ready(layer.parameters())
    _wgrad_keep.append(deferred)

    def _join(stream=ws):
        torch.cuda.current_stream().wait_stream(stream)
        _wgrad_keep.clear()

    torch.autograd.Variable._execution_engine.queue_callback(_join)


def _wgrad_stream():
    global _wgrad_stream_obj
    if _wgrad_stream_obj is None:
        _wgrad_stream_obj = torch.cuda.Stream()
    return _wgrad_stream_obj


def _switches():
    return paths.Switches(LAYER_SEQ, STACK_SEQ, STACK_MAX_ROWS, ops.GROUPED_DW, ops.GROUPED_DW_MIN_ROWS, ops.FWD_F16, bool(ops.kernel_timer.names))


def _pair_grad_chain(s, key_tiles):
    return (torch.empty if key_tiles is None else torch.zeros)(s.shape, device=s.device, dtype=ops.pair_grad_dtype(s))


def _kept(L, li, plan):
    if li >= plan.lowest:
        return L
    return SimpleNamespace(site_f=getattr(L, "site_f", None))


class _Sites:

    def __init__(self):
        self.n = 0

    def next(self):
        self.n += 1
        return self.n


class PairEncoderFn(torch.autograd.Function):

    @staticmethod
    def forward(ctx, emb, bias, padding_mask, mod, training, key_tiles=None, pack=None, aux_grads=False, anchor=None):
        if pack is not None:
            B, N, D = pack.B, pack.S, emb.shape[-1]
            if emb.dim() != 2 or emb.shape[0] != pack.M:
                raise ops.MMDTIError("PairEncoderFn: packed rows expect emb [pack.M, D]")
        else:
            B, N, D = emb.shape
        H = mod.attention_heads
        tiled = ops.pair_is_tiled(bias)
        compact = tiled and bias.dtype == torch.float16
        if not compact:
            key_tiles = None
        if pack is not None and key_tiles is None:
            raise ops.MMDTIError("PairEncoderFn: packed rows need the compact tiled pair layout and key_tiles")
        if aux_grads and (compact or pack is not None):
            raise ops.MMDTIError("PairEncoderFn: differentiable auxiliary outputs need fp32 pair planes on padded rows")
        row_off = None if pack is None else pack.off
        slot = getattr(bias, "_mmdti_grad_slot", None) if compact else None
        if compact and slot is None and bias.requires_grad:
            raise ops.MMDTIError("PairEncoderFn: an fp16 pair bias that needs a gradient must come from PairBiasFn")
        ld = ops.pair_ld(N) if tiled else bias.shape[-1]
        M = B * N if pack is None else pack.M
        p_emb = mod.emb_dropout if training else 0.0
        p_res = mod.dropout if training else 0.0
        p_att = mod.attention_dropout if training else 0.0
        seed = dropout_state.next_seed()
        sites = _Sites()
        st = SimpleNamespace(B=B, N=N, D=D, H=H, ld=ld, M=M, seed=seed, p_emb=p_emb, p_res=p_res, p_att=p_att, layers=[], kt=key_tiles, slot=slot,
                             row_off=row_off, packed=pack is not None)
        keep = any(ctx.needs_input_grad)
        if keep:
            eln = mod.emb_layer_norm
            st.plan = plan_tower(layer_trainable(mod.layers), ctx.needs_input_grad[0] or eln.weight.requires_grad or eln.bias.requires_grad,
                                 ctx.needs_input_grad[1])
        emb = emb.contiguous()
        st.emb = emb
        st.pad = padding_mask
        st.site_emb = sites.next()
        eln = mod.emb_layer_norm
        x, _, st.emb_mean, st.emb_rstd = ops.layernorm_fwd(emb.view(M, D), eln.weight, eln.bias, eln.eps, want_f32=True, want_bf16=False,
                                                           row_zero=None if padding_mask is None else padding_mask.reshape(-1),
                                                           drop_p=p_emb, seed=seed, site=st.site_emb)
        scale = (D // H) ** -0.5
        s_prev = bias.contiguous()
        st.bias0 = s_prev if not mod.layers else None
        nlayers = len(mod.layers)
        nxt = None
        out = None
        sw = _switches()
        path = paths.unimol_layer_fwd(sw, emb.is_cuda, compact, D, H)
        seq = path == paths.LAYER
        kp0 = ops._u8(padding_mask) if seq else None
        st.stack = None
        T = None
        if paths.unimol_tower_fwd(sw, path, keep, nlayers, M, aux_grads, mod.final_layer_norm is not None) == paths.STACK:
            T = _stack_tables(_unimol_stack_desc, mod, M, sw)
        if T is not None:
            x, out, s_prev = _unimol_stack_fwd(st, T, mod, x, s_prev, kp0, key_tiles, pack is None, row_off, scale, sites, tiled)
        for li, layer in enumerate(mod.layers if T is None else ()):
            L = SimpleNamespace(x=x)
            ln1, ln2 = layer.self_attn_layer_norm, layer.final_layer_norm
            att = layer.self_attn
# ... 27 lines not shown
            L.a = ops.linear_fwd(L.h2, wfwd(layer.fc1.weight), layer.fc1.bias, act=ops.ACT_GELU_FWD, aux_out=L.u)
            L.site_f = sites.next()
            if li + 1 < nlayers:
                nl = mod.layers[li + 1].self_attn_layer_norm
                x, _, h1n, m1n, r1n = ops.linear_ln_fwd(L.a, wfwd(layer.fc2.weight), layer.fc2.bias, nl.weight, nl.bias, nl.eps, residual=L.x1,
                                                        drop_p=p_res, seed=seed, site=L.site_f)
                nxt = (h1n, m1n, r1n)
            elif mod.final_layer_norm is not None:
                fl = mod.final_layer_norm
                x, out, _, st.f_mean, st.f_rstd = ops.linear_ln_fwd(L.a, wfwd(layer.fc2.weight), layer.fc2.bias, fl.weight, fl.bias, fl.eps,
                                                                    residual=L.x1, drop_p=p_res, seed=seed, site=L.site_f, want_f32=True, want_bf16=False)
            else:
                x = ops.linear_fwd(L.a, wfwd(layer.fc2.weight), layer.fc2.bias, residual=L.x1, out_dtype=F32, drop_p=p_res, seed=seed, site=L.site_f)
            if keep:
                st.layers.append(_kept(L, li, st.plan))
        st.x_last = x
        if out is None:
            if mod.final_layer_norm is not None:
                fl = mod.final_layer_norm
                out, _, st.f_mean, st.f_rstd = ops.layernorm_fwd(x, fl.weight, fl.bias, fl.eps, want_f32=True, want_bf16=False)
            else:
                out = x
        if keep:
            ctx.st, ctx.mod = st, mod
        x_last = x.view(B, N, D) if pack is None else x
        if not aux_grads:
            ctx.mark_non_differentiable(s_prev, x_last)
        ctx.set_materialize_grads(False)
        return (out.view(B, N, D) if pack is None else out), s_prev, x_last

    @staticmethod
    def backward(ctx, dout, ds_last, dx_pre):
        st, mod = ctx.st, ctx.mod
        if getattr(st, "consumed", False):
            raise ops.MMDTIError("PairEncoderFn: backward through the same forward twice (retain_graph) is not supported")
        st.consumed = True
        B, N, D, H, ld, M, seed = st.B, st.N, st.D, st.H, st.ld, st.M, st.seed
        scale = (D // H) ** -0.5
        if dout is None:
            dout = torch.zeros(M, D, device=st.emb.device, dtype=F32)
        dout = dout.contiguous().view(M, D)
        if dx_pre is not None:
            dx_pre = dx_pre.contiguous().view(M, D).float()
        if mod.final_layer_norm is not None:
            fl = mod.final_layer_norm
            nxt = (st.p_res, st.layers[-1].site_f, gbuf(mod.layers[-1].fc2.bias)) if st.layers else None
            if st.stack is not None:
                nxt = (st.p_res, st.stack.site0 + 3 * (st.stack.T.nl - 1) + 2, gbuf(mod.layers[-1].fc2.bias))
            dx = ops.layernorm_bwd(dout, st.x_last, fl.weight, st.f_mean, st.f_rstd, gbuf(fl.weight), gbuf(fl.bias), dres=dx_pre, bf16_copy=nxt)
            dx, dx16 = dx if nxt is not None else (dx, None)
        else:
            dx, dx16 = (dout if dx_pre is None else dout + dx_pre), None
        G = None
        if ds_last is not None:
            G = ds_last.to(F32).contiguous().clone()
            if st.pad is not None and not ops.pair_is_tiled(G):
                G.masked_fill_(st.pad.view(B, 1, 1, N), 0.0)
            if G.shape[-1] > N and not ops.pair_is_tiled(G):
                G[..., N:] = 0.0
        if st.stack is not None:
            dx, G = _unimol_stack_bwd(st, dx, dx16, scale)
            notify_grads_ready(st.stack.T.params)
            st.stack = None
        below = [Lb.site_f for Lb in st.layers[:-1]]
        deferred, deferred_layers = [], []
        n_defer = DEFER_WGRAD_LAYERS if (dout.is_cuda and M >= 8192) else 0
        plan = st.plan
        full = [all(p.requires_grad for p in l.parameters()) for l in mod.layers] if st.layers else []
        seq_path, seq_ws = _unimol_seq_workspace(st, mod, full, dout.is_cuda)
        for li, layer, L in zip(range(len(st.layers) - 1, -1, -1), reversed(mod.layers), reversed(st.layers)):
            if li < plan.lowest:
                L.__dict__.clear()
                continue
            att, ln1, ln2 = layer.self_attn, layer.self_attn_layer_norm, layer.final_layer_norm
            hold = li < n_defer
            pending = []
            lowest = not plan.needs_dx(li)

            def _wgrad(*args, **kw):
                pending.append((args, kw))
            if paths.unimol_layer_bwd(seq_path, dx16 is not None, hold, full[li]) == paths.LAYER:
                g_zero = G is None
                if g_zero:
                    G = _pair_grad_chain(L.s, st.kt)
                dx, dx16 = _unimol_layer_bwd_seq(st, layer, L, dx, dx16, G, g_zero, scale, seq_ws,
                                                 None if (li == 0 or lowest) else (below[li - 1], gbuf(mod.layers[li - 1].fc2.bias)))
                L.__dict__.clear()
                notify_grads_ready(layer.parameters())
                continue
            dy2 = dx16 if dx16 is not None else ops.cast_bf16(dx, st.p_res, seed, L.site_f)
            _wgrad(dy2, L.a, layer.fc2.weight, layer.fc2.bias, bias_done=dx16 is not None)
            du = ops.linear_bwd_input(dy2, wbf16(layer.fc2.weight), act=ops.ACT_GELU_DX, aux_in=L.u)
            _wgrad(du, L.h2, layer.fc1.weight, layer.fc1.bias)
            dh2 = ops.linear_bwd_input(du, wbf16(layer.fc1.weight))
            dx, dy1 = ops.layernorm_bwd(dh2, L.x1, ln2.weight, L.m2, L.r2, gbuf(ln2.weight), gbuf(ln2.bias), dres=dx,
                                        bf16_copy=(st.p_res, L.site_o, gbuf(att.out_proj.bias)))
            _wgrad(dy1, L.o, att.out_proj.weight, att.out_proj.bias, bias_done=True)
            do = ops.linear_bwd_input(dy1, wbf16(att.out_proj.weight))
            g_zero = G is None
            if g_zero:
                G = _pair_grad_chain(L.s, st.kt)
            dqkv = ops.pair_attn_bwd(L.qkv, L.s, do, G, B, N, H, ld, scale, g_zero, st.p_att, seed, L.site_att, key_tiles=st.kt, row_off=st.row_off)
            _wgrad(dqkv, L.h1, att.in_proj.weight, att.in_proj.bias)
            if lowest and not (ln1.weight.requires_grad or ln1.bias.requires_grad):
                dh1 = None
            else:
                dh1 = ops.linear_bwd_input(dqkv, wbf16(att.in_proj.weight))
            if dh1 is None:
                dx, dx16 = None, None
            elif lowest or li == 0:
                dx, dx16 = ops.layernorm_bwd(dh1, L.x, ln1.weight, L.m1, L.r1, gbuf(ln1.weight), gbuf(ln1.bias), dres=dx), None
            else:
                dx, dx16 = ops.layernorm_bwd(dh1, L.x, ln1.weight, L.m1, L.r1, gbuf(ln1.weight), gbuf(ln1.bias), dres=dx,
                                             bf16_copy=(st.p_res, below[li - 1], gbuf(mod.layers[li - 1].fc2.bias)))
            if hold:
                deferred.append(pending)
                deferred_layers.append(layer)
            else:
                _lin_bwd_params_many(pending)
            L.__dict__.clear()
            if not hold:
                notify_grads_ready(layer.parameters())
        eln = mod.emb_layer_norm
        demb = None
        if plan.below:
            demb = ops.layernorm_bwd(dx, st.emb.view(M, D), eln.weight, st.emb_mean, st.emb_rstd, gbuf(eln.weight), gbuf(eln.bias),
                                     row_zero=None if st.pad is None else st.pad.reshape(-1), drop_p=st.p_emb, seed=seed, site=st.site_emb)
            if not ctx.needs_input_grad[0]:
                demb = None
        notify_grads_ready(list(eln.parameters()) + ([] if mod.final_layer_norm is None else list(mod.final_layer_norm.parameters())))
        if not ctx.needs_input_grad[1]:
            G = None
        elif G is None:
            G = torch.zeros_like(st.bias0)
        if G is not None and st.slot is not None:
            st.slot.g = G
            G = torch.zeros((), device=G.device, dtype=torch.float16).expand(G.shape)
        _launch_deferred_wgrads(deferred, deferred_layers)
        _join_stream_after_backward()
        if demb is not None and not st.packed:
            demb = demb.view(B, N, D)
        return demb, G, None, None, None, None, None, None, None


STACK_SEQ = os.environ.get("MMDTI_STACK_SEQ", "1") != "0"
STACK_MAX_ROWS = int(os.environ.get("MMDTI_STACK_MAX_ROWS", "8192"))
STACK_SIDE_WGRAD = os.environ.get("MMDTI_STACK_SIDE_WGRAD", "0") != "0"
_stack_layouts = {}
_stack_sides = {}


def _ptr_table(ptrs):
    arr = (ctypes.c_void_p * len(ptrs))(*ptrs)
    return arr, ctypes.addressof(arr)


def bert_weights(layer) -> SimpleNamespace:
    a, o = layer.attention.self, layer.attention.output
    return SimpleNamespace(q_w=a.query.weight, q_b=a.query.bias, k_w=a.key.weight, k_b=a.key.bias, v_w=a.value.weight, v_b=a.value.bias,
                           o_w=o.dense.weight, o_b=o.dense.bias, ln1_w=o.LayerNorm.weight, ln1_b=o.LayerNorm.bias,
                           i_w=layer.intermediate.dense.weight, i_b=layer.intermediate.dense.bias,
                           o2_w=layer.output.dense.weight, o2_b=layer.output.dense.bias,
                           ln2_w=layer.output.LayerNorm.weight, ln2_b=layer.output.LayerNorm.bias)


def _unimol_stack_desc(l):
    a, ln1, ln2 = l.self_attn, l.self_attn_layer_norm, l.final_layer_norm
    w_in, b_in, w_out, b_out, w1, b1, w2, b2 = a.in_proj.weight, a.in_proj.bias, a.out_proj.weight, a.out_proj.bias, l.fc1.weight, l.fc1.bias, l.fc2.weight, l.fc2.bias
    g1, bt1, g2, bt2 = ln1.weight, ln1.bias, ln2.weight, ln2.bias
    ps = [w_in, b_in, w_out, b_out, g2, bt2, w1, b1, w2, b2, g1, bt1]
    return SimpleNamespace(params=ps, w16=(w_in, w_out, w1, w2), fwd=ps, bwd=(w2, w1, w_out, w_in, g2, g1), recast=(w_in, w_out, w1, w2), probe=w1,
                           grads=(w2, w1, w_out, w_in, b2, b1, b_out, b_in, g2, bt2, g1, bt1), eps=(ln2.eps, ln1.eps), runs=())


def _bert_stack_desc(l):
    W = bert_weights(l)
    return SimpleNamespace(params=[W.q_w, W.k_w, W.v_w, W.q_b, W.k_b, W.v_b, W.o_w, W.o_b, W.ln1_w, W.ln1_b, W.i_w, W.i_b, W.o2_w, W.o2_b, W.ln2_w, W.ln2_b],
                           w16=(W.q_w, W.o_w, W.i_w, W.o2_w),
                           fwd=(W.q_w, W.q_b, W.o_w, W.o_b, W.ln1_w, W.ln1_b, W.i_w, W.i_b, W.o2_w, W.o2_b, W.ln2_w, W.ln2_b),
                           bwd=(W.q_w, W.o_w, W.i_w, W.o2_w, W.ln1_w, W.ln2_w), recast=(W.q_w, W.k_w, W.v_w, W.o_w, W.i_w, W.o2_w), probe=W.i_w,
                           grads=(W.q_w, W.q_b, W.o_w, W.o_b, W.i_w, W.i_b, W.o2_w, W.o2_b, W.ln1_w, W.ln1_b, W.ln2_w, W.ln2_b), eps=(),
                           runs=((W.q_w, W.k_w, W.v_w), (W.q_b, W.k_b, W.v_b)))


_unimol_stack_desc.probe = lambda l: l.fc1.weight
_bert_stack_desc.probe = lambda l: l.intermediate.dense.weight


def _stack_tables(desc, mod, rows, sw, attn_ok=True):
    layers = list(mod.layers)
    probe0 = desc.probe(layers[0])
    arena = getattr(probe0, "_mmdti_arena", None)
    F, D = probe0.shape
    if paths.stack_call(sw, arena is not None, D, F, rows, attn_ok) != paths.STACK:
        return None
    cache = arena.__dict__.setdefault("_stack_tables", {})
    flags = trainable_flags(q for l in layers for q in l.parameters())
    key = (weakref.ref(mod), ops.FWD_F16, desc, flags)
    T = cache.get(key)
    if T is None:
        ds = [desc(l) for l in layers]
        d0 = ds[0]
        off = arena.offsets
        same_arena = all(q is not None and getattr(q, "_mmdti_arena", None) is arena for d in ds for q in d.params)
        uniform = all(tuple(d.probe.shape) == (F, D) and len(list(l.parameters())) == len(d.params) and all(e == d0.eps[0] for e in d.eps)
                      for l, d in zip(layers, ds))
        adjacent = same_arena and all(off[id(q)] == off[id(p)] + p.numel() for d in ds for run in d.runs for p, q in zip(run, run[1:]))
        if paths.stack_model(flags, same_arena, uniform, adjacent) != paths.STACK:
            cache[key] = False
            return None
        if ops.FWD_F16:
            arena._fresh16()
        sh16 = (arena.shadow16 if ops.FWD_F16 else arena.shadow).data_ptr()
        shb, gr = arena.shadow.data_ptr(), arena.grad.data_ptr()
        fwd, bwd, grads, weights, probes = [], [], [], [], []
        for d in ds:
            w16 = {id(q) for q in d.w16}
# ... 19 lines not shown
    return T


def _dw_slab_bytes(D, F, rows):
    tiles = (D // 256) * (F // 256) * 2 + (D // 256) ** 2 * 4
    return ops.lib()._dll.mmdti_linear_dw_grouped_splits(tiles, rows) * (2 * D * F + 4 * D * D) * 4


def _unimol_layer_ws_bytes(M, D, F):
    return (M * F + 7 * M * D) * 2 + M * D * 4 + _dw_slab_bytes(D, F, M)


def _bert_layer_ws_bytes(Mq, D, F, nrow):
    return (Mq * F + 7 * Mq * D) * 2 + Mq * D * 4 + (nrow * 4 + 15) // 16 * 16 + _dw_slab_bytes(D, F, Mq)


def _bert_cross_layer_ws_bytes(Mq, D, nrow):
    return 4 * Mq * D + 4 * Mq * D + (nrow * 4 + 15) // 16 * 16


def _attn_stat_rows(st, heads):
    return heads * st.Mq if st.vl is not None else st.B * heads * st.Lq


def _stack_layout(query, rows, D, F, *sizes):
    key = (query, rows, D, F) + sizes
    r = _stack_layouts.get(key)
    if r is None:
        slab = _dw_slab_bytes(D, F, rows)
        out = (ctypes.c_longlong * 2)()
        getattr(ops.lib(), query)(rows, D, F, *sizes, slab, ctypes.addressof(out))
        if len(_stack_layouts) > 4096:
            _stack_layouts.clear()
        r = _stack_layouts[key] = (int(out[0]), int(out[1]), slab)
    return r


def _stack_side():
    if not STACK_SIDE_WGRAD or torch.cuda.is_current_stream_capturing():
        return 0, 0
    main = torch.cuda.current_stream()
    key = (main.device.index, main.cuda_stream)
    ent = _stack_sides.get(key)
    if ent is None:
        side = torch.cuda.Stream(device=main.device)
        evs = [torch.cuda.Event() for _ in range(3)]
        for e in evs:
            e.record(main)
        ent = _stack_sides[key] = (side, evs, _ptr_table([e.cuda_event for e in evs]))
    return ent[0].cuda_stream, ent[2][1]


def _unimol_stack_fwd(st, T, mod, x, s_prev, key_pad, key_tiles, rag_store_last, row_off, scale, sites, tiled):
    M, D, F, B, N, H, ld = st.M, st.D, T.F, st.B, st.N, st.H, st.ld
    dev = x.device
    l0 = mod.layers[0]
    ln1, fl = l0.self_attn_layer_norm, mod.final_layer_norm
    _, h1, m1, r1 = ops.layernorm_fwd(x, ln1.weight, ln1.bias, ln1.eps)
    e = torch.empty
    s_last = torch.empty_like(s_prev) if tiled else e(B, H, N, ld, device=dev, dtype=F32)
    s_bytes = s_last.numel() * s_last.element_size()
    stride, ws_bytes, slab = _stack_layout("mmdti_unimol_stack_layout", M, D, F, s_bytes)
    arena = e(stride * T.nl, device=dev, dtype=torch.uint8)
    x_last, out = e(M, D, device=dev, dtype=F32), e(M, D, device=dev, dtype=F32)
    st.f_mean, st.f_rstd = e(M, device=dev, dtype=F32), e(M, device=dev, dtype=F32)
    site0 = sites.n + 1
    sites.n += 3 * T.nl
    p = ops._p
    ops.lib().mmdti_unimol_stack_fwd(
        ops._stream(), T.nl, M, B, N, H, D, F, ld, float(scale), float(st.p_res), float(st.p_att), int(st.seed), site0, x.data_ptr(), h1.data_ptr(),
        s_prev.data_ptr(), p(key_pad), ops._pair_layout_s(s_prev, "pair_attn.bias"), p(key_tiles), int(rag_store_last), p(row_off), T.fwd[1],
        ops.ACT_GELU_FWD, float(l0.final_layer_norm.eps), fl.weight.data_ptr(), fl.bias.data_ptr(), float(fl.eps), ops.GEMM_LN_MAX_K if ops.GEMM_LN else 0, arena.data_ptr(),
        arena.numel(), s_bytes, x_last.data_ptr(), s_last.data_ptr(), out.data_ptr(), st.f_mean.data_ptr(), st.f_rstd.data_ptr(),
        int(h1.dtype == torch.float16))
    st.stack = SimpleNamespace(T=T, arena=arena, s_bytes=s_bytes, ws_bytes=ws_bytes, slab=slab, site0=site0, x0=x, h1=h1, m1=m1, r1=r1, s_last=s_last)
    return x_last, out, s_last


def _unimol_stack_bwd(st, dx, dx16, scale):
    S = st.stack
    T = S.T
    M, D = st.M, st.D
    dev = dx.device
    G = _pair_grad_chain(S.s_last, st.kt)
    layout = ops._pair_layout_s(S.s_last, "pair_attn_bwd.s") | (4 if G.dtype == BF16 else 0)
    dx_final = torch.empty_like(dx)
    ws = torch.empty(S.ws_bytes, device=dev, dtype=torch.uint8)
    side, events = _stack_side()
    p = ops._p
    ops.lib().mmdti_unimol_stack_bwd(
        ops._stream(), T.nl, M, st.B, st.N, st.H, D, T.F, st.ld, float(scale), float(st.p_res), float(st.p_att), int(st.seed), S.site0, dx.data_ptr(),
        dx16.data_ptr(), dx_final.data_ptr(), S.x0.data_ptr(), S.h1.data_ptr(), S.m1.data_ptr(), S.r1.data_ptr(), S.s_last.data_ptr(), T.bwd[1],
        ops.ACT_GELU_DX, T.grads[1], G.data_ptr(), layout, 1, p(st.kt), p(st.row_off), S.arena.data_ptr(), S.arena.numel(), S.s_bytes, ws.data_ptr(),
        ws.numel(), S.slab, int(S.h1.dtype == torch.float16), side, events)
    return dx_final, G


def _unimol_layer_fwd_seq(st, layer, L, s_prev, key_pad, key_tiles, rag_store, row_off, scale, nl, next_mode):
    att, ln2 = layer.self_attn, layer.final_layer_norm
    M, D, F = st.M, st.D, layer.fc1.weight.shape[0]
    dev = L.x.device
    e = torch.empty
    a16 = L.h1.dtype
    L.qkv, L.o = e(M, 3 * D, device=dev, dtype=a16), e(M, D, device=dev, dtype=a16)
    L.s = torch.empty_like(s_prev) if ops.pair_is_tiled(s_prev) else e(st.B, st.H, st.N, st.ld, device=dev, dtype=F32)
    L.x1, L.h2 = e(M, D, device=dev, dtype=F32), e(M, D, device=dev, dtype=a16)
    L.m2, L.r2 = e(M, device=dev, dtype=F32), e(M, device=dev, dtype=F32)
    L.u, L.a = e(M, F, device=dev, dtype=BF16), e(M, F, device=dev, dtype=a16)
    x_out = e(M, D, device=dev, dtype=F32)
    ln_out = mn = rn = None
    if next_mode:
        ln_out = e(M, D, device=dev, dtype=a16 if next_mode == 1 else F32)
        mn, rn = e(M, device=dev, dtype=F32), e(M, device=dev, dtype=F32)
    p = ops._p
    ops.lib().mmdti_unimol_layer_fwd(
        ops._stream(), M, st.B, st.N, st.H, D, F, st.ld, float(scale), float(st.p_res), float(st.p_att), int(st.seed), int(L.site_att), int(L.site_o),
        int(L.site_f), L.x.data_ptr(), L.h1.data_ptr(), s_prev.data_ptr(), p(key_pad), ops._pair_layout_s(s_prev, "pair_attn.bias"), p(key_tiles),
        int(rag_store), p(row_off), wfwd(att.in_proj.weight).data_ptr(), p(att.in_proj.bias), wfwd(att.out_proj.weight).data_ptr(), p(att.out_proj.bias),
        ln2.weight.data_ptr(), ln2.bias.data_ptr(), float(ln2.eps), wfwd(layer.fc1.weight).data_ptr(), p(layer.fc1.bias), ops.ACT_GELU_FWD,
        wfwd(layer.fc2.weight).data_ptr(), p(layer.fc2.bias), next_mode, p(nl.weight) if nl is not None else 0, p(nl.bias) if nl is not None else 0,
        float(nl.eps) if nl is not None else 0.0, ops.GEMM_LN_MAX_K if ops.GEMM_LN else 0, L.qkv.data_ptr(), L.s.data_ptr(), L.o.data_ptr(),
        L.x1.data_ptr(), L.h2.data_ptr(), L.m2.data_ptr(), L.r2.data_ptr(), L.u.data_ptr(), L.a.data_ptr(), x_out.data_ptr(), p(ln_out), p(mn), p(rn),
        int(a16 == torch.float16))
    return x_out, ln_out, mn, rn


def _unimol_seq_workspace(st, mod, full, on_gpu):
    nkept, lowest = len(st.layers), st.plan.lowest
    D, F, M = st.D, (mod.layers[0].fc1.weight.shape[0] if nkept else 0), st.M
    L0 = st.layers[lowest] if lowest < nkept else None
    path = paths.unimol_tower_bwd(_switches(), on_gpu, nkept, lowest, L0 is not None and L0.h1.dtype == torch.float16,
                                  L0 is not None and L0.s.dtype == torch.float16, D, F, M, full)
    if path != paths.LAYER:
        return path, None
    return path, torch.empty(_unimol_layer_ws_bytes(M, D, F) + 256, device=st.emb.device, dtype=torch.uint8)


def _unimol_layer_bwd_seq(st, layer, L, dx, dx16, G, g_zero, scale, ws, below):
    att, ln1, ln2 = layer.self_attn, layer.self_attn_layer_norm, layer.final_layer_norm
    M, D, F = st.M, st.D, layer.fc1.weight.shape[0]
    dx_out = torch.empty_like(dx)
    dx16_out = torch.empty(M, D, device=dx.device, dtype=BF16) if below is not None else None
    layout = ops._pair_layout_s(L.s, "pair_attn_bwd.s") | (4 if G.dtype == BF16 else 0)
    p = ops._p
    ops.lib().mmdti_unimol_layer_bwd(
        ops._stream(), M, st.B, st.N, st.H, D, F, st.ld, float(scale), float(st.p_res), float(st.p_att), int(st.seed),
        int(below[0]) if below is not None else 0, int(L.site_o), int(L.site_att), dx.data_ptr(), dx16.data_ptr(), dx_out.data_ptr(), p(dx16_out),
        p(below[1]) if below is not None else 0, L.a.data_ptr(), L.u.data_ptr(), ops.ACT_GELU_DX, L.h2.data_ptr(), L.x1.data_ptr(), L.m2.data_ptr(),
        L.r2.data_ptr(), L.o.data_ptr(), L.qkv.data_ptr(), L.s.data_ptr(), L.h1.data_ptr(), L.x.data_ptr(), L.m1.data_ptr(), L.r1.data_ptr(),
        wbf16(layer.fc2.weight).data_ptr(), wbf16(layer.fc1.weight).data_ptr(), wbf16(att.out_proj.weight).data_ptr(), wbf16(att.in_proj.weight).data_ptr(),
        ln2.weight.data_ptr(), ln1.weight.data_ptr(), gbuf(layer.fc2.weight).data_ptr(), gbuf(layer.fc1.weight).data_ptr(),
        gbuf(att.out_proj.weight).data_ptr(), gbuf(att.in_proj.weight).data_ptr(), gbuf(layer.fc1.bias).data_ptr(), gbuf(att.out_proj.bias).data_ptr(),
        gbuf(att.in_proj.bias).data_ptr(), gbuf(ln2.weight).data_ptr(), gbuf(ln2.bias).data_ptr(), gbuf(ln1.weight).data_ptr(), gbuf(ln1.bias).data_ptr(),
        G.data_ptr(), layout, int(g_zero), p(st.kt), p(st.row_off), (ws.data_ptr() + 255) // 256 * 256, ws.numel() - 256,
        int(L.h1.dtype == torch.float16))
    return dx_out, dx16_out


class PairBiasFn(torch.autograd.Function):

    @staticmethod
    def forward(ctx, anchor, dist, edge_type, gbf, proj, ld, key_tiles_host=None, rows_host=None):
        B, N, _ = dist.shape
        H = proj.linear2.weight.shape[0]
        dist, edge_type = dist.contiguous(), edge_type.contiguous()
        args = [gbf.mul.weight.view(-1), gbf.bias.weight.view(-1), gbf.means.weight.view(-1), gbf.stds.weight.view(-1)]
        fused = ops.gbf_bias_eligible(args[2].numel(), proj.linear1.weight.shape[0], H, ld)
        full = fused and ops.GBF_FULL_BWD and args[0].numel() <= ops.GBF_FULL_MAXE
        if edge_type.dtype != torch.int64 and not fused:
            edge_type = edge_type.long()
        if fused:
            keep = any(ctx.needs_input_grad) and not full
            tiled = ops.pair_tiled_ok(N)
            compact = tiled and ops.PAIR_COMPACT
            pre_f = pre_b = rb_f = rb_b = None
            if key_tiles_host is not None and compact and full:
                if rows_host is not None:
                    pre_f, pre_b, rb_f, rb_b = ops.gbf_tile_prefixes(key_tiles_host, N, dist.device, rows_host)
                else:
                    pre_f, pre_b = ops.gbf_tile_prefixes(key_tiles_host, N, dist.device)
            out, saved = ops.gbf_bias_fwd(dist, edge_type, *args, wbf16(proj.linear1.weight), proj.linear1.bias,
                                          wbf16(proj.linear2.weight), proj.linear2.bias, ld, save=keep, tiled=tiled,
                                          save_grad=ops.GELU_SAVE_GRAD, compact=compact, tile_prefix=pre_f, row_blocks=rb_f)
            feat, u, h = saved if keep else (None, None, None)
            ugrad = ops.GELU_SAVE_GRAD
        else:
            feat = ops.gbf_features_fwd(dist, edge_type, *args)
            u = torch.empty(feat.shape[0], proj.linear1.weight.shape[0], device=dist.device, dtype=BF16)
            h = ops.linear_fwd(feat, wbf16(proj.linear1.weight), proj.linear1.bias, act=ops.ACT_GELU_FWD, aux_out=u)
            ugrad = ops.GELU_SAVE_GRAD
            o = ops.linear_fwd(h, wbf16(proj.linear2.weight), proj.linear2.bias, out_dtype=F32)
            out = ops.pair_permute_fwd(o, B, N, H, ld)
        ctx.st = SimpleNamespace(dist=dist, et=edge_type, feat=feat, u=u, h=h, B=B, N=N, H=H, ld=ld, fused=fused, ugrad=ugrad, full=full, slot=None,
                                 pre_b=pre_b if fused else None, rb_b=rb_b if fused else None)
        ctx.gbf, ctx.proj = gbf, proj
        if out.dtype == torch.float16:
            ctx.st.slot = out._mmdti_grad_slot = SimpleNamespace(g=None)
        return out

    @staticmethod
    def backward(ctx, g):
        st, gbf, proj = ctx.st, ctx.gbf, ctx.proj
        ps = [gbf.mul.weight, gbf.bias.weight, gbf.means.weight, gbf.stds.weight]
        if st.slot is not None:
            real = any(sd != 0 for sd in g.stride())
            chain, st.slot.g = st.slot.g, None
            if chain is None:
                g = g.float()
            elif real:
                g = chain.float().add_(g) if chain.dtype != F32 else chain.add_(g)
            else:
                g = chain
        if st.full:
            l1, l2 = proj.linear1, proj.linear2
            allp = [l1.weight, l1.bias, l2.weight, l2.bias] + ps
            grads = [gbuf(p) if p.requires_grad else torch.zeros_like(p) for p in allp]
            ops.gbf_bias_bwd_full(g.contiguous(), st.dist, st.et, *[p.view(-1) for p in ps], wbf16(l1.weight), l1.bias, wbf16(l2.weight),
                                  st.ld, *[gr.view(-1) for gr in grads], tile_prefix=st.pre_b, row_blocks=st.rb_b)
        elif st.fused and ps[0].numel() <= 4096:
            grads = [gbuf(p) if p.requires_grad else torch.zeros_like(p) for p in ps]
            do, du = ops.gbf_bias_bwd(g.contiguous(), st.dist, st.et, *[p.view(-1) for p in ps], wbf16(proj.linear1.weight),
                                      wbf16(proj.linear2.weight), st.u, st.ld, *[gr.view(-1) for gr in grads], u_is_grad=st.ugrad)
            _lin_bwd_params(do, st.h, proj.linear2.weight, proj.linear2.bias)
            _lin_bwd_params(du, st.feat, proj.linear1.weight, proj.linear1.bias)
        else:
            do = ops.pair_permute_bwd(g.contiguous(), st.B, st.N, st.H, st.ld)
            _lin_bwd_params(do, st.h, proj.linear2.weight, proj.linear2.bias)
            du = ops.linear_bwd_input(do, wbf16(proj.linear2.weight), act=ops.ACT_MUL_AUX if st.ugrad else ops.ACT_GELU_BWD, aux_in=st.u)
            _lin_bwd_params(du, st.feat, proj.linear1.weight, proj.linear1.bias)
            dfeat = ops.linear_bwd_input(du, wbf16(proj.linear1.weight))
            if any(p.requires_grad for p in ps):
                grads = [gbuf(p) if p.requires_grad else torch.zeros_like(p) for p in ps]
                ops.gbf_features_bwd(st.dist, st.et, *[p.view(-1) for p in ps], dfeat, *[gr.view(-1) for gr in grads])
        notify_grads_ready(list(gbf.parameters()) + list(proj.parameters()))
        _join_stream_after_backward()
        return None, None, None, None, None, None, None, None


class PairCompactFn(torch.autograd.Function):

    @staticmethod
    def forward(ctx, bias, N):
        out = ops.pair_tile(bias[..., :N].float().clamp(max=65504.0), N).to(torch.float16)
        ctx.N, ctx.ld = N, bias.shape[-1]
        ctx.slot = out._mmdti_grad_slot = SimpleNamespace(g=None)
        return out

    @staticmethod
    def backward(ctx, g):
        chain, ctx.slot.g = ctx.slot.g, None
        real = any(sd != 0 for sd in g.stride())
        if chain is None:
            chain = g.float()
        elif real:
            chain = chain.float() + g.float()
        d = ops.pair_untile(chain.float(), ctx.N)
        if ctx.ld != ctx.N:
            d = torch.nn.functional.pad(d, (0, ctx.ld - ctx.N))
        return d, None


class EmbeddingFn(torch.autograd.Function):

    @staticmethod
    def forward(ctx, weight, ids, padding_idx):
        ctx.ids, ctx.w, ctx.pad = ids.contiguous(), weight, -1 if padding_idx is None else padding_idx
        return ops.embedding_fwd(ctx.ids, weight)

    @staticmethod
    def backward(ctx, dout):
        g = gbuf(ctx.w)
        if g is not None:
            ops.embedding_bwd_gemm(ctx.ids, ops.cast_bf16(dout.contiguous()), g, ctx.pad)
        notify_grads_ready([ctx.w])
        _join_stream_after_backward()
        return None, None, None


def _bert_layer_fwd(st, s1_32, s1_16, s2_16, key_add, W, heads, p_hid, p_att, eps, seed, sites, self_attn):
    B, Lq, Lk, D = st.B, st.Lq, st.Lk, st.D
    Mq, vl = st.Mq, st.vl
    hd = D // heads
    ld = (Lk + 7) // 8 * 8
    L = SimpleNamespace(s1_16=s1_16, s2_16=s2_16, ld=ld, heads=heads, self_attn=self_attn, W=W, eps=eps)
    L.site_att = sites.next()
    L.key_add, L.fused = key_add, ops.attn_eligible(Lq, Lk, hd, D)
    if not L.fused:
        ops.warn_unfused_length(Lq, Lk)
    L.fw = L.fb = None
    if L.fused and W.q_b is not None:
        plist_w, plist_b = ((W.q_w, W.k_w, W.v_w), (W.q_b, W.k_b, W.v_b)) if self_attn else ((W.k_w, W.v_w), (W.k_b, W.v_b))
        L.fw, L.fb = fused_views(plist_w), fused_views(plist_b)
        if L.fw is None or L.fb is None:
            L.fw = L.fb = None
    L.path = paths.bert_layer_fwd(_switches(), self_attn, L.fw is not None, s1_32.is_cuda, D, W.i_w.shape[0], Mq)
    if L.path == paths.LAYER:
        if self_attn:
            return _bert_layer_fwd_seq(st, L, s1_32, s1_16, key_add, W, heads, p_hid, p_att, eps, seed, sites)
        return _bert_cross_layer_fwd_seq(st, L, s1_32, s1_16, s2_16, key_add, W, heads, p_hid, p_att, eps, seed, sites)
    if L.fw is not None:
        if self_attn:
            L.qkv = ops.linear_fwd(s1_16, L.fw[3], L.fb[1], out_dtype=BF16)
            L.q, L.k, L.v = L.qkv[:, :D], L.qkv[:, D:2 * D], L.qkv[:, 2 * D:]
        else:
            L.q = ops.linear_fwd(s1_16, wfwd(W.q_w), W.q_b, out_dtype=BF16)
            L.qkv = ops.linear_fwd(s2_16, L.fw[3], L.fb[1], out_dtype=BF16)
            L.k, L.v = L.qkv[:, :D], L.qkv[:, D:]
    else:
        L.q = ops.linear_fwd(s1_16, wfwd(W.q_w), W.q_b, out_dtype=BF16)
        L.k = ops.linear_fwd(s2_16, wfwd(W.k_w), W.k_b, out_dtype=BF16)
        L.v = ops.linear_fwd(s2_16, wfwd(W.v_w), W.v_b, out_dtype=BF16)
    if L.fused:
        L.ctx, L.stats = ops.attn_dispatch(Lq, Lk)[0](L.q, L.k, L.v, key_add, B, heads, Lq, Lk, 1.0 / math.sqrt(hd), p_att, seed, L.site_att, vl=vl)
    else:
        if vl is not None:
            raise ops.MMDTIError("packed sequences need the fused attention kernels (head_dim 16 / 32 / 64, at most 512 tokens)")
        S = torch.empty(B, heads, Lq, ld, device=s1_32.device, dtype=F32)
        ops.gemm(L.q, L.k, M=Lq, N=Lk, K=hd, lda=D, ldb=D, out=S, ldc=ld, batch=(B, heads), sA=(Lq * D, hd), sB=(Lk * D, hd),
                 sC=(heads * Lq * ld, Lq * ld), alpha=1.0 / math.sqrt(hd))
        L.p, L.pd = ops.softmax_fwd(S, key_add, B, heads, Lq, Lk, ld, p_att, seed, L.site_att)
        del S
        L.ctx = torch.empty(B * Lq, D, device=s1_32.device, dtype=ops.act16())
        ops.gemm(L.pd, L.v, M=Lq, N=hd, K=Lk, lda=ld, ldb=D, transB=True, out=L.ctx, ldc=D, batch=(B, heads),
                 sA=(heads * Lq * ld, Lq * ld), sB=(Lk * D, hd), sC=(Lq * D, hd))
    L.site_o = sites.next()
    L.y, L.a32, L.a16, L.am, L.ar = ops.linear_ln_fwd(L.ctx, wfwd(W.o_w), W.o_b, W.ln1_w, W.ln1_b, eps, residual=s1_32, drop_p=p_hid, seed=seed,
                                                      site=L.site_o, want_f32=True, want_bf16=True)
    L.u = torch.empty(Mq, W.i_w.shape[0], device=s1_32.device, dtype=BF16)
    L.i = ops.linear_fwd(L.a16, wfwd(W.i_w), W.i_b, act=ops.ACT_GELU_FWD, aux_out=L.u)
    L.site_f = sites.next()
    L.z, out32, out16, L.zm, L.zr = ops.linear_ln_fwd(L.i, wfwd(W.o2_w), W.o2_b, W.ln2_w, W.ln2_b, eps, residual=L.a32, drop_p=p_hid, seed=seed,
                                                      site=L.site_f, want_f32=True, want_bf16=True)
    L.p_hid, L.p_att = p_hid, p_att
    return L, out32, out16
# ... 623 lines not shown
```

### mm-dti_amd/mmdti_hip/ops.py

```python
from __future__ import annotations

import os

import torch

from ._abi import lib, MMDTIError

BF16 = torch.bfloat16
F32 = torch.float32
F16 = torch.float16

ACT_NONE, ACT_GELU, ACT_GELU_BWD, ACT_TANH, ACT_GELU_G, ACT_MUL_AUX = 0, 1, 2, 3, 4, 5
GELU_SAVE_GRAD = os.environ.get("MMDTI_GELU_SAVE_GRAD", "1") != "0"
GBF_FULL_BWD = os.environ.get("MMDTI_GBF_FULL_BWD", "1") != "0"
ACT_GELU_FWD = ACT_GELU_G if GELU_SAVE_GRAD else ACT_GELU
ACT_GELU_DX = ACT_MUL_AUX if GELU_SAVE_GRAD else ACT_GELU_BWD
DT_F32, DT_BF16, DT_F32_ATOMIC, DT_F16, DT_AB_F16, DT_B_F16 = 0, 1, 2, 3, 16, 32

FWD_F16 = os.environ.get("MMDTI_FWD_FP16", "1") != "0"


def set_forward_fp16(on: bool):
    global FWD_F16
    FWD_F16 = bool(on)
# ... 416 lines not shown
    du = torch.empty(P, Fh, device=g.device, dtype=BF16)
    t0 = kernel_timer.begin("gbf_bias_bwd")
    _chk_edge(edge_type)
    lib().mmdti_gbf_bias_bwd(_stream(), g.data_ptr(), dist.data_ptr(), edge_type.data_ptr(), edge_type.element_size(), mul.data_ptr(), bias.data_ptr(), means.data_ptr(),
                             stds.data_ptr(), w1.data_ptr(), w2.data_ptr(), u.data_ptr(), B, N, ld, w1.shape[1], Fh, Hh, mul.numel(),
                             _pair_layout_g(g, "gbf_bias_bwd") | (2 if u_is_grad else 0), do.data_ptr(), du.data_ptr(), dmul.data_ptr(), dbias.data_ptr(), dmeans.data_ptr(),
                             dstds.data_ptr())
    kernel_timer.end("gbf_bias_bwd", t0, float(P) * (Hh * g.element_size() + 256 + 4 + edge_type.element_size() + 2 * Hh + 2 * Fh))
    return do, du


GBF_FULL_MAXE = 1536
GBF_SLABS = os.environ.get("MMDTI_GBF_SLABS", "1") != "0"


def gbf_bias_bwd_full(g, dist, edge_type, mul, bias, means, stds, w1, b1, w2, ld, dw1, db1, dw2, db2, dmul, dbias, dmeans, dstds,
                      tile_prefix=None, row_blocks=None):
    _chk(dist, F32, "gbf.dist"); _chk_edge(edge_type); _chk(w1, BF16, "gbf.w1"); _chk(w2, BF16, "gbf.w2")
    for t, nm in ((dw1, "dw1"), (db1, "db1"), (dw2, "dw2"), (db2, "db2"), (dmul, "dmul"), (dbias, "dbias"), (dmeans, "dmeans"), (dstds, "dstds")):
        _chk(t, F32, "gbf." + nm)
    B, N, _ = dist.shape
    Hh, Fh = w2.shape
    P = B * N * N
    ws = torch.empty(lib()._dll.mmdti_gbf_bias_bwd_full_workspace(mul.numel()), device=dist.device, dtype=torch.uint8) if GBF_SLABS else None
    t0 = kernel_timer.begin("gbf_bias_bwd")
    lib().mmdti_gbf_bias_bwd_full(_stream(), g.data_ptr(), dist.data_ptr(), edge_type.data_ptr(), edge_type.element_size(), mul.data_ptr(),
                                  bias.data_ptr(), means.data_ptr(), stds.data_ptr(), w1.data_ptr(), b1.data_ptr(), w2.data_ptr(), B, N, ld,
                                  w1.shape[1], Fh, Hh, mul.numel(), _pair_layout_g(g, "gbf_bias_bwd_full"), dw1.data_ptr(), db1.data_ptr(), dw2.data_ptr(),
                                  db2.data_ptr(), dmul.data_ptr(), dbias.data_ptr(), dmeans.data_ptr(), dstds.data_ptr(), _p(tile_prefix), _p(row_blocks),
                                  _p(ws), 0 if ws is None else ws.numel())
    K = w1.shape[1]
    kept = _pair_kept if tile_prefix is not None else 1.0
    kernel_timer.end("gbf_bias_bwd", t0, kept * float(P) * (6.0 * Fh * K + 4.0 * Hh * Fh))


def gbf_bias_eligible(K, Fh, Hh, ld):
    return K == 128 and Fh == 128 and Hh == 64 and ld % 4 == 0


def pair_ld(N):
    return (N + 3) // 4 * 4


def pair_permute_fwd(x, B, N, H, ld):
    _chk(x, F32, "pair_permute_fwd.x")
    out = torch.empty(B, H, N, ld, device=x.device, dtype=F32)
    lib().mmdti_pair_permute_fwd(_stream(), x.data_ptr(), out.data_ptr(), B, N, H, ld)
    return out


def pair_permute_bwd(g, B, N, H, ld):
    _chk(g, F32, "pair_permute_bwd.g")
    out = torch.empty(B * N * N, H, device=g.device, dtype=BF16)
    lib().mmdti_pair_permute_bwd(_stream(), g.data_ptr(), out.data_ptr(), B, N, H, ld, int(pair_is_tiled(g)))
    return out


def pair_is_tiled(t):
    return t.dim() == 3


def pair_plane(N):
    return (N * pair_ld(N) + 7) // 8 * 8


def pair_tiles(N):
    return (N + 15) // 16


def pair_tiled_ok(N):
    return N <= 272


def pair_empty(B, H, N, device, tiled, zero=False, dtype=F32):
    shape = (B, H, pair_plane(N)) if tiled else (B, H, N, pair_ld(N))
    t = (torch.zeros if zero else torch.empty)(shape, device=device, dtype=dtype)
    if tiled and not zero and shape[2] != N * pair_ld(N):
        t[:, :, N * pair_ld(N):] = 0
    return t


PAIR_COMPACT = os.environ.get("MMDTI_PAIR_COMPACT", "1") != "0"
PAIR_G_BF16 = os.environ.get("MMDTI_PAIR_G_BF16", "0") == "1"


def pair_grad_dtype(s):
    return BF16 if (s.dtype == F16 and PAIR_G_BF16) else F32


def _pair_layout_s(s, what):
    tiled = pair_is_tiled(s)
    if s.dtype == F16:
        if not tiled:
            raise MMDTIError(f"{what}: fp16 pair logits exist in the tiled layout only")
        return 3
    _chk(s, F32, what)
    return int(tiled)


def _pair_layout_g(g, what):
    tiled = pair_is_tiled(g)
    if g.dtype == BF16:
        if not tiled:
            raise MMDTIError(f"{what}: bf16 pair gradients exist in the tiled layout only")
        return 5
    _chk(g, F32, what)
    return int(tiled)


def _tile_index(N, device, cols=None):
    q = torch.arange(N, device=device).view(N, 1)
    k = torch.arange(N if cols is None else cols, device=device).view(1, -1)
    vr = torch.clamp(N - q // 16 * 16, max=16)
    return (q // 16 * 16) * pair_ld(N) + vr * (k - k % 4) + (q % 16) * 4 + k % 4


def pair_slots(N, device, q_lo=0, q_hi=None, k_lo=0, k_hi=None):
    idx = _tile_index(N, device, pair_ld(N))
    return idx[q_lo:(N if q_hi is None else q_hi), k_lo:(pair_ld(N) if k_hi is None else k_hi)].reshape(-1)


def pair_tile(x, N, pad=float("-inf")):
    B, H = x.shape[:2]
    out = torch.full((B, H, pair_plane(N)), pad, device=x.device, dtype=x.dtype)
    out[:, :, _tile_index(N, x.device).reshape(-1)] = x[..., :N, :N].reshape(B, H, N * N)
    return out


def pair_untile(t, N):
    B, H = t.shape[:2]
    return t.reshape(B, H, -1)[:, :, _tile_index(N, t.device).reshape(-1)].view(B, H, N, N)


def pair_key_tiles_effective(kt, nt):
    step = 1 if nt <= 9 else (2 if nt <= 13 else 4)
    k = (max(int(kt), 1) + step - 1) // step * step
    return nt if k >= nt else k


_pair_kept = 1.0


def set_pair_kept(frac):
    global _pair_kept
    _pair_kept = float(frac)


def pair_attn_fwd(qkv, bias_in, key_pad, B, N, H, ld, scale, drop_p=0.0, seed=0, site=0, key_tiles=None, rag_store=False, row_off=None):
    _chk16(qkv, "pair_attn.qkv")
    layout = _pair_layout_s(bias_in, "pair_attn.bias")
    tiled = pair_is_tiled(bias_in)
    o_f16 = False
    if qkv.dtype == F16 and layout != 3:
        qkv, o_f16 = to_bf16(qkv), True
    rows = qkv.shape[0] if row_off is not None else B * N
    if row_off is not None:
        _chk(row_off, torch.int32, "pair_attn.row_off")
        if row_off.numel() != B + 1 or key_tiles is None:
            raise MMDTIError("pair_attn_fwd: row_off must be [B+1] and come with key_tiles")
        if key_pad is not None and key_pad.numel() != rows:
            raise MMDTIError("pair_attn_fwd: with packed rows key_pad is indexed by packed row")
    elif qkv.shape[0] != B * N:
        raise MMDTIError(f"pair_attn_fwd: qkv has {qkv.shape[0]} rows, expected B*N = {B * N}")
    s_out = torch.empty_like(bias_in) if tiled else torch.empty(B, H, N, ld, device=qkv.device, dtype=F32)
    o = torch.empty(rows, H * 8, device=qkv.device, dtype=qkv.dtype)
    kp = _u8(key_pad)
    t0 = kernel_timer.begin("pair_attn_fwd")
    if key_tiles is not None:
        _chk(key_tiles, torch.int32, "pair_attn.key_tiles")
    lib().mmdti_pair_attn_fwd(_stream(), qkv.data_ptr(), bias_in.data_ptr(), s_out.data_ptr(), o.data_ptr(), _p(kp), B, N, H, ld,
                              float(scale), float(drop_p), int(seed), int(site), layout, _p(key_tiles), int(rag_store), _p(row_off),
                              int(qkv.dtype == F16))
    kept, es = _pair_kept if key_tiles is not None else 1.0, float(s_out.element_size())
    kernel_timer.end("pair_attn_fwd", t0, float(H) * (B * N * N * (es * kept + es * (1.0 if rag_store else kept)) + rows * 64.0))
    if o_f16:
        o = cast_act16(cast_f32(o)) if FWD_F16 else o
    return s_out, o


def pair_attn_bwd(qkv, s, do, g, B, N, H, ld, scale, g_in_zero, drop_p=0.0, seed=0, site=0, key_tiles=None, row_off=None):
    if (row_off is None and qkv.shape[0] != B * N) or do.shape[0] != qkv.shape[0]:
        raise MMDTIError("pair_attn_bwd: qkv / do row counts do not match the layout")
    if row_off is not None:
        _chk(row_off, torch.int32, "pair_attn.row_off")
    tiled = pair_is_tiled(s)
    if qkv.dtype == F16 and not (tiled and N <= 272):
        qkv = to_bf16(qkv)
    dqkv = torch.empty(qkv.shape, device=qkv.device, dtype=BF16)
    layout = _pair_layout_s(s, "pair_attn_bwd.s")
    if pair_is_tiled(g) != tiled or not (g.dtype == F32 or (g.dtype == BF16 and s.dtype == F16)):
        raise MMDTIError("pair_attn_bwd: S and G must share one pair layout (fp32 gradients, or bf16 gradients with fp16 logits)")
    if g.dtype == BF16:
        layout |= 4
    t0 = kernel_timer.begin("pair_attn_bwd")
    lib().mmdti_pair_attn_bwd(_stream(), qkv.data_ptr(), s.data_ptr(), do.data_ptr(), g.data_ptr(), dqkv.data_ptr(), B, N, H, ld,
                              float(scale), int(g_in_zero), float(drop_p), int(seed), int(site), layout, _p(key_tiles), _p(row_off), int(qkv.dtype == F16))
    kept = _pair_kept if key_tiles is not None else 1.0
    kernel_timer.end("pair_attn_bwd", t0, float(H) * (B * N * N * kept * (s.element_size() + g.element_size() * (1 if g_in_zero else 2)) + qkv.shape[0] * 112.0))
    return dqkv


def softmax_fwd(s, key_add, B, heads, Lq, Lk, ld, drop_p=0.0, seed=0, site=0):
    _chk(s, F32, "softmax.s")
    p = torch.empty(B, heads, Lq, ld, device=s.device, dtype=BF16)
    pd = torch.empty_like(p) if drop_p > 0 else p
    lib().mmdti_softmax_fwd(_stream(), s.data_ptr(), _p(key_add), p.data_ptr(), pd.data_ptr(), B, heads, Lq, Lk, ld, float(drop_p),
                            int(seed), int(site))
    return p, pd


def softmax_bwd(p, dp, B, heads, Lq, Lk, ld, scale, drop_p=0.0, seed=0, site=0):
    ds = torch.empty(B, heads, Lq, ld, device=p.device, dtype=BF16)
    lib().mmdti_softmax_bwd(_stream(), p.data_ptr(), dp.data_ptr(), ds.data_ptr(), B, heads, Lq, Lk, ld, float(scale), float(drop_p),
                            int(seed), int(site))
    return ds


FUSED_ATTN = True
ATTN_MAX_LEN = 256
ATTN_LONG_MAX_LEN = 512


def attn_eligible(Lq, Lk, hd, D):
    return FUSED_ATTN and hd in (16, 32, 64) and Lq <= ATTN_LONG_MAX_LEN and Lk <= ATTN_LONG_MAX_LEN and D % 8 == 0


def attn_is_long(Lq, Lk):
    return max(Lq, Lk) > ATTN_MAX_LEN


_warned_long = False


def warn_unfused_length(Lq, Lk):
    global _warned_long
    if not _warned_long and FUSED_ATTN and max(Lq, Lk) > ATTN_LONG_MAX_LEN:
        _warned_long = True
        import warnings
        warnings.warn(f"attention over {Lq} queries x {Lk} keys: longer than the fused kernels' {ATTN_LONG_MAX_LEN}; this batch takes the "
                      "materialised-scores path (slower, more memory)", RuntimeWarning, stacklevel=3)


class AttnVarlen:

    def __init__(self, q_pack, k_pack):
        self.q_off, self.k_off, self.k_cnt = q_pack.off, k_pack.off, k_pack.n_real
        self.q_rows, self.k_rows = q_pack.M, k_pack.M
        self.Lq, self.Lk = q_pack.max_rows, int(k_pack.counts_host.max())
        self.pairs = float((q_pack.rows_host * k_pack.counts_host).sum())

    def args(self):
        return (self.q_off.data_ptr(), self.k_off.data_ptr(), self.k_cnt.data_ptr(), self.q_rows)


_NO_VARLEN = (0, 0, 0, 0)


def _attn_fwd(name, q, k, v, key_add, B, heads, Lq, Lk, scale, drop_p=0.0, seed=0, site=0, vl=None):
    for t_, n_ in ((q, "attn.q"), (k, "attn.k"), (v, "attn.v")):
        _chk(t_, BF16, n_, contiguous=False)
        if t_.stride(1) != 1:
            raise MMDTIError(f"{n_}: unit column stride required")
    D = q.shape[1]
    hd = D // heads
    rows_q = B * Lq if vl is None else vl.q_rows
    if q.shape[0] != rows_q or k.shape[0] != (B * Lk if vl is None else vl.k_rows) or (vl is not None and key_add is not None):
        raise MMDTIError(f"{name}: row counts do not match the layout (packed sequences take no key_add)")
    ctx = torch.empty(rows_q, D, device=q.device, dtype=act16())
    stats = torch.empty((B, heads, Lq, 2) if vl is None else (heads, rows_q, 2), device=q.device, dtype=F32)
    t0 = kernel_timer.begin(name)
    getattr(lib(), "mmdti_" + name)(_stream(), q.data_ptr(), k.data_ptr(), v.data_ptr(), _p(key_add), ctx.data_ptr(), stats.data_ptr(), B, heads, Lq, Lk,
                         hd, q.stride(0), k.stride(0), D, float(scale), float(drop_p), int(seed), int(site), *(_NO_VARLEN if vl is None else vl.args()),
                         int(ctx.dtype == F16))
    kernel_timer.end(name, t0, 4.0 * heads * hd * (B * Lq * Lk if vl is None else vl.pairs))
    return ctx, stats

# ... 374 lines not shown
```

Before: 5013.

## Store pair-attention gradient chain as row-scaled fp16 with per-row bounds

Adds a new default gradient-chain format for the pair bias: fp16 values scaled by a per-row power-of-two bound stored behind the planes. The pair attention backward and the GBF bias backward read and write this format directly, and a decode kernel converts it to fp32 where other consumers need it. The goal is to halve the memory traffic of the N×N gradient planes compared with fp32 while keeping more precision than bf16. The cost is extra bound bookkeeping, extra decode kernels on some paths, and a risk of reduced gradient precision.

```diff
diff --git a/include/mmdti_hip.h b/include/mmdti_hip.h
--- a/include/mmdti_hip.h
+++ b/include/mmdti_hip.h
@@ -211,6 +211,7 @@
 int mmdti_gbf_bias_bwd_full_workspace(int E);
 int mmdti_pair_permute_fwd(mmdti_stream_t stream, const float* x, float* out, int B, int N, int H, int ld);
 int mmdti_pair_permute_bwd(mmdti_stream_t stream, const float* g, void* out_bf16, int B, int N, int H, int ld, int tiled);
+int mmdti_pair_g_decode(mmdti_stream_t stream, const void* g_sf16, void* out_f32, int B, int N, int H);
 
 int mmdti_pair_attn_fwd(mmdti_stream_t stream, const void* qkv_bf16, const void* bias_in, void* s_out,
                         void* o_bf16, const unsigned char* key_pad, int B, int N, int H, int ld, float scale,
diff --git a/mm-dti_amd/csrc/common.h b/mm-dti_amd/csrc/common.h
--- a/mm-dti_amd/csrc/common.h
+++ b/mm-dti_amd/csrc/common.h
@@ -122,6 +122,7 @@
 void salt_pull_pair_attn(hipStream_t s, const unsigned long long* src);
 void salt_pull_pair_attn_bwd(hipStream_t s, const unsigned long long* src);
 void salt_pull_pair_attn_bwd_g16(hipStream_t s, const unsigned long long* src);
+void salt_pull_pair_attn_bwd_gs16(hipStream_t s, const unsigned long long* src);
 void salt_pull_attn(hipStream_t s, const unsigned long long* src);
 void salt_pull_elementwise(hipStream_t s, const unsigned long long* src);
 __device__ __forceinline__ uint32_t mix32(uint32_t x) {
diff --git a/mm-dti_amd/csrc/elementwise.hip b/mm-dti_amd/csrc/elementwise.hip
--- a/mm-dti_amd/csrc/elementwise.hip
+++ b/mm-dti_amd/csrc/elementwise.hip
@@ -919,6 +919,7 @@
   salt_pull_pair_attn(s, salt);
   salt_pull_pair_attn_bwd(s, salt);
   salt_pull_pair_attn_bwd_g16(s, salt);
+  salt_pull_pair_attn_bwd_gs16(s, salt);
   salt_pull_attn(s, salt);
   salt_pull_elementwise(s, salt);
   MMDTI_LAUNCH_CHECK();
diff --git a/mm-dti_amd/csrc/gbf.hip b/mm-dti_amd/csrc/gbf.hip
--- a/mm-dti_amd/csrc/gbf.hip
+++ b/mm-dti_amd/csrc/gbf.hip
@@ -1,4 +1,5 @@
 #include "common.h"
+#include "pair_attn.h"
 
 namespace mmdti {
 
@@ -206,6 +207,7 @@
 __device__ __forceinline__ float gbf_get(const __bf16* p) {
   return __builtin_bit_cast(float, (uint32_t)(*reinterpret_cast<const unsigned short*>(p)) << 16);
 }
+__device__ __forceinline__ float gbf_get(const pa_sf16* p) { return (float)p->v; }
 
 template <bool SAVE, bool TILED, typename OT>
 __global__ __launch_bounds__(512, 2) void gbf_bias_fwd_kernel(const float* __restrict__ dist, const void* __restrict__ et, int esz,
@@ -590,7 +592,8 @@
     const float* __restrict__ bias, const float* __restrict__ means, const float* __restrict__ stds, const bf16_t* __restrict__ W1,
     const float* __restrict__ b1, const bf16_t* __restrict__ W2, float* __restrict__ dW1, float* __restrict__ db1, float* __restrict__ dW2,
     float* __restrict__ db2, float* __restrict__ dmul, float* __restrict__ dbias, float* __restrict__ dmeans, float* __restrict__ dstds, int B,
-    int N, int ld, int E, int tpm, const int* __restrict__ tile_prefix, const int* __restrict__ row_blocks, float* __restrict__ slab) {
+    int N, int ld, int E, int tpm, const int* __restrict__ tile_prefix, const int* __restrict__ row_blocks, float* __restrict__ slab,
+    const float* __restrict__ gbound) {
   extern __shared__ __attribute__((aligned(16))) unsigned char gbf_smem[];
   bf16_t* sW1 = reinterpret_cast<bf16_t*>(gbf_smem);
   bf16_t* sW2T = sW1 + GBF_F * GBF_LW;
@@ -707,6 +710,13 @@
     for (int c = 0; c < 2; ++c)
 #pragma unroll
       for (int j = 0; j < 8; ++j) gv[c * 8 + j] = gbf_get(mb + (long long)(32 * c + j) * plane + voff);
+    if constexpr (std::is_same<GT, pa_sf16>::value) {
+      const float* bb = gbound + ((long long)b * GBF_H + 8 * g) * N + (valid ? ii : 0);
+#pragma unroll
+      for (int c = 0; c < 2; ++c)
+#pragma unroll
+        for (int j = 0; j < 8; ++j) gv[c * 8 + j] *= pa_sf16_dec(bb[(32 * c + j) * N]);
+    }
   };
 
   bool act, valid, n_act, n_valid;
@@ -724,7 +734,7 @@
     const float* b1row = reinterpret_cast<const float*>(gbf_smem + o_b1row);
     const float* kconst = reinterpret_cast<const float*>(gbf_smem + o_kconst);
     fetch(tile + stride, n_act, n_valid, n_d, n_e, n_gv);
-    constexpr bool SPLIT_G = sizeof(GT) == 4;
+    constexpr bool SPLIT_G = !std::is_same<GT, __bf16>::value;
     gbf16x8 oB[2], oL[2], hB[4];
     if (!valid) {
 #pragma unroll
@@ -1174,8 +1184,8 @@
                                        const float* b1, const void* w2_bf16, int B, int N, int ld, int K, int F, int H, int E, int flags,
                                        float* dw1, float* db1, float* dw2, float* db2, float* dmul, float* dbias, float* dmeans,
                                        float* dstds, const int* tile_prefix, const int* row_blocks, void* workspace, long long workspace_bytes) {
-  const int tiled = flags & 1, compact = (flags >> 2) & 1;
-  MMDTI_REQUIRE(!compact || tiled, "gbf_bias_bwd_full: compact planes (flags bit 2) exist in the tiled layout only");
+  const int tiled = flags & 1, compact = (flags >> 2) & 1, gs16 = (flags >> 3) & 1;
+  MMDTI_REQUIRE((!compact && !gs16) || (tiled && !(compact && gs16)), "gbf_bias_bwd_full: 16-bit gradient planes (flags bit 2 or bit 3, not both) exist in the tiled layout only");
   MMDTI_REQUIRE(!tile_prefix || tiled, "gbf_bias_bwd_full: tile_prefix (ragged batches) needs the tiled pair layout");
   MMDTI_REQUIRE(!row_blocks || tile_prefix, "gbf_bias_bwd_full: row_blocks (packed token rows) comes with tile_prefix");
   MMDTI_REQUIRE(g && dist && edge_type && mul && bias && means && stds && w1_bf16 && b1 && w2_bf16 && dw1 && db1 && dw2 && db2 && dmul && dbias &&
@@ -1196,7 +1206,8 @@
     const int cap = (int)gbf_full_smem(GBF_FULL_MAXE);
     if (hipFuncSetAttribute(reinterpret_cast<const void*>(gbf_bias_bwd_full_kernel<true, float>), hipFuncAttributeMaxDynamicSharedMemorySize, cap) != hipSuccess ||
         hipFuncSetAttribute(reinterpret_cast<const void*>(gbf_bias_bwd_full_kernel<false, float>), hipFuncAttributeMaxDynamicSharedMemorySize, cap) != hipSuccess ||
-        hipFuncSetAttribute(reinterpret_cast<const void*>(gbf_bias_bwd_full_kernel<true, __bf16>), hipFuncAttributeMaxDynamicSharedMemorySize, cap) != hipSuccess) {
+        hipFuncSetAttribute(reinterpret_cast<const void*>(gbf_bias_bwd_full_kernel<true, __bf16>), hipFuncAttributeMaxDynamicSharedMemorySize, cap) != hipSuccess ||
+        hipFuncSetAttribute(reinterpret_cast<const void*>(gbf_bias_bwd_full_kernel<true, pa_sf16>), hipFuncAttributeMaxDynamicSharedMemorySize, cap) != hipSuccess) {
       set_error("gbf_bias_bwd_full: hipFuncSetAttribute failed");
       return MMDTI_ERR_LAUNCH;
     }
@@ -1205,10 +1216,11 @@
 #define GBF_FB(TILED, GT)                                                                                                          \
   hipLaunchKernelGGL((gbf_bias_bwd_full_kernel<TILED, GT>), dim3(grid), dim3(512), smem, (hipStream_t)stream, (const GT*)g, dist, edge_type, edge_bytes, mul, \
                      bias, means, stds, (const bf16_t*)w1_bf16, b1, (const bf16_t*)w2_bf16, dw1, db1, dw2, db2, dmul, dbias, dmeans, dstds, B, \
-                     N, ld, E, tpm, tile_prefix, row_blocks, slab)
+                     N, ld, E, tpm, tile_prefix, row_blocks, slab, gbound)
   const long long SL = GBF_SLAB + 2 * (long long)E;
   float* slab = (workspace && aligned16(workspace) && workspace_bytes >= (long long)grid * SL * 4) ? reinterpret_cast<float*>(workspace) : nullptr;
-  if (compact) GBF_FB(true, __bf16); else if (tiled) GBF_FB(true, float); else GBF_FB(false, float);
+  const float* gbound = gs16 ? reinterpret_cast<const float*>(reinterpret_cast<const _Float16*>(g) + (long long)B * GBF_H * pair_plane(N)) : nullptr;
+  if (gs16) GBF_FB(true, pa_sf16); else if (compact) GBF_FB(true, __bf16); else if (tiled) GBF_FB(true, float); else GBF_FB(false, float);
 #undef GBF_FB
   if (slab)
     hipLaunchKernelGGL(gbf_slab_reduce_kernel, dim3(cdiv(SL, 64)), dim3(256), 0, (hipStream_t)stream, slab, grid, E, dw1, db1, dw2, db2, dmul, dbias, dmeans, dstds);
diff --git a/mm-dti_amd/csrc/pair_attn.h b/mm-dti_amd/csrc/pair_attn.h
--- a/mm-dti_amd/csrc/pair_attn.h
+++ b/mm-dti_amd/csrc/pair_attn.h
@@ -111,6 +111,37 @@
 __device__ __forceinline__ f32x4 pa_load4_nt(const __bf16* p) { return pa_widen_bf16(__builtin_nontemporal_load(reinterpret_cast<const pa_s16x4*>(p))); }
 __device__ __forceinline__ void pa_store4_nt(__bf16* p, const f32x4& v) { __builtin_nontemporal_store(pa_pack4(v), reinterpret_cast<pa_s16x4*>(p)); }
 
+struct pa_sf16 { _Float16 v; };
+__device__ __forceinline__ int pa_sf16_exp(float bound) {
+  const uint32_t u = __float_as_uint(bound);
+  const int e = (int)((u >> 23) & 0xffu) - 127 + ((u & 0x7fffffu) ? 1 : 0);
+  return min(max(e, -100), 127);
+}
+__device__ __forceinline__ float pa_pow2(int k) { return __uint_as_float((uint32_t)(k + 127) << 23); }
+__device__ __forceinline__ float pa_sf16_enc(float bound) { return pa_pow2(15 - pa_sf16_exp(bound)); }
+__device__ __forceinline__ float pa_sf16_dec(float bound) { return pa_pow2(pa_sf16_exp(bound) - 15); }
+__device__ __forceinline__ f32x4 pa_load4(const pa_sf16* p, float dec) { return pa_widen_f16(*reinterpret_cast<const pa_f16x4*>(p)) * dec; }
+__device__ __forceinline__ f32x4 pa_load4_nt(const pa_sf16* p, float dec) {
+  return pa_widen_f16(__builtin_nontemporal_load(reinterpret_cast<const pa_f16x4*>(p))) * dec;
+}
+__device__ __forceinline__ void pa_store4_nt(pa_sf16* p, const f32x4& v, float enc) {
+  __builtin_nontemporal_store(pa_narrow_f16(v * enc), reinterpret_cast<pa_f16x4*>(p));
+}
+
+template <typename GT> struct pa_rawq { typedef pa_s16x4 type; };
+template <> struct pa_rawq<float> { typedef f32x4 type; };
+__device__ __forceinline__ f32x4 pa_load4_raw(const float* p) { return pa_load4(p); }
+__device__ __forceinline__ f32x4 pa_load4_raw_nt(const float* p) { return pa_load4_nt(p); }
+__device__ __forceinline__ pa_s16x4 pa_load4_raw(const __bf16* p) { return *reinterpret_cast<const pa_s16x4*>(p); }
+__device__ __forceinline__ pa_s16x4 pa_load4_raw_nt(const __bf16* p) { return __builtin_nontemporal_load(reinterpret_cast<const pa_s16x4*>(p)); }
+__device__ __forceinline__ pa_s16x4 pa_load4_raw(const pa_sf16* p) { return *reinterpret_cast<const pa_s16x4*>(p); }
+__device__ __forceinline__ pa_s16x4 pa_load4_raw_nt(const pa_sf16* p) { return __builtin_nontemporal_load(reinterpret_cast<const pa_s16x4*>(p)); }
+__device__ __forceinline__ f32x4 pa_widen_raw(const float*, const f32x4& r, float) { return r; }
+__device__ __forceinline__ f32x4 pa_widen_raw(const __bf16*, const pa_s16x4& r, float) { return pa_widen_bf16(r); }
+__device__ __forceinline__ f32x4 pa_widen_raw(const pa_sf16*, const pa_s16x4& r, float dec) {
+  return pa_widen_f16(__builtin_bit_cast(pa_f16x4, r)) * dec;
+}
+
 __host__ __device__ constexpr int pa_kt_step(int nt) { return nt <= 9 ? 1 : (nt <= 13 ? 2 : 4); }
 __host__ __device__ constexpr int pa_kt_effective(int kt, int nt) {
   const int s = pa_kt_step(nt), k = ((kt < 1 ? 1 : kt) + s - 1) / s * s;
diff --git a/mm-dti_amd/csrc/pair_attn_bwd.hip b/mm-dti_amd/csrc/pair_attn_bwd.hip
--- a/mm-dti_amd/csrc/pair_attn_bwd.hip
+++ b/mm-dti_amd/csrc/pair_attn_bwd.hip
@@ -151,11 +151,12 @@
                                    void* g, void* dqkv_bf16, int B, int N, int H, int ld, float scale,
                                    int g_in_zero, float drop_p, unsigned long long seed, unsigned int site, int layout,
                                    const int* key_tiles, const int* row_off, int qkv_f16) {
-  const int tiled = layout & 1, compact = (layout >> 1) & 1, g16 = (layout >> 2) & 1;
+  const int tiled = layout & 1, compact = (layout >> 1) & 1, g16 = (layout >> 2) & 1, gs16 = (layout >> 3) & 1;
   if (int e = check_common("pair_attn_bwd", B, N, H, ld)) return e;
-  MMDTI_REQUIRE((layout & ~7) == 0 && (!compact || tiled) && (!g16 || compact),
-                "pair_attn_bwd: layout must be 0 (row-major fp32), 1 (tiled fp32), 3 (tiled, fp16 logits) or 7 (tiled, fp16 logits, bf16 gradients)");
-  MMDTI_REQUIRE(!key_tiles || compact, "pair_attn_bwd: key_tiles (ragged batches) needs the compact planes (layout 3 or 7: tiled, fp16 logits)");
+  MMDTI_REQUIRE((layout & ~15) == 0 && (!compact || tiled) && (!g16 || compact) && (!gs16 || (compact && !g16)),
+                "pair_attn_bwd: layout must be 0 (row-major fp32), 1 (tiled fp32), 3 (tiled, fp16 logits), 7 (tiled, fp16 logits, bf16 gradients) or 11 (tiled, "
+                "fp16 logits, row-scaled fp16 gradients)");
+  MMDTI_REQUIRE(!key_tiles || compact, "pair_attn_bwd: key_tiles (ragged batches) needs the compact planes (layout 3, 7 or 11: tiled, fp16 logits)");
   MMDTI_REQUIRE(!row_off || key_tiles, "pair_attn_bwd: packed token rows (row_off) need key_tiles");
   MMDTI_REQUIRE(!tiled || (ld % 4 == 0 && N <= 16 * PA_MAX_NT), "pair_attn_bwd: the tiled pair layout needs ld %% 4 == 0 and N <= 272");
   MMDTI_REQUIRE(qkv_bf16 && s && do_bf16 && g && dqkv_bf16, "pair_attn_bwd: null pointer");
@@ -172,7 +173,7 @@
 #define PA_MB(NT, TL, FL, NWV, RG, ST, GT)                                                                                     \
   hipLaunchKernelGGL((pair_attn_bwd_mfma_kernel<NT, TL, FL, NWV, RG, ST, GT>), grid, blk, 0, st, (const bf16_t*)qkv_bf16,      \
                      (const ST*)s, (const bf16_t*)do_bf16, (const GT*)g, (GT*)g, (bf16_t*)dqkv_bf16, N, H, ld, scale,           \
-                     g_in_zero, th8, sc, (uint64_t)seed, (uint32_t)site, key_tiles, row_off, qkv_f16)
+                     g_in_zero, th8, sc, (uint64_t)seed, (uint32_t)site, key_tiles, row_off, qkv_f16, nullptr)
 #define PA_MBW(NT, TL, FL, RG, ST, GT)                                                      \
   do {                                                                                      \
     if (blk.x == 192) PA_MB(NT, TL, FL, 3, RG, ST, GT); else PA_MB(NT, TL, FL, 4, RG, ST, GT); \
@@ -183,6 +184,9 @@
     else { if (nqb == NT) PA_MBW(NT, true, true, false, float, float); else PA_MBW(NT, true, false, false, float, float); } \
   } while (0)
     if (compact) {
+      if (gs16) pa_bwd_compact_launch_gs16(nqb, grid, blk, st, qkv_bf16, s, do_bf16, g, dqkv_bf16, N, H, ld, scale, g_in_zero, th8, sc, seed, site, key_tiles, row_off, qkv_f16,
+                                           reinterpret_cast<float*>(reinterpret_cast<_Float16*>(g) + (long long)B * H * pair_plane(N)));
+      else
       if (g16) pa_bwd_compact_launch_g16(nqb, grid, blk, st, qkv_bf16, s, do_bf16, g, dqkv_bf16, N, H, ld, scale, g_in_zero, th8, sc, seed, site, key_tiles, row_off, qkv_f16);
       else pa_bwd_compact_launch<float>(nqb, grid, blk, st, qkv_bf16, s, do_bf16, g, dqkv_bf16, N, H, ld, scale, g_in_zero, th8, sc, seed, site, key_tiles, row_off, qkv_f16);
     } else if (nqb <= 5) PA_MBT(5); else if (nqb <= 9) PA_MBT(9); else if (nqb <= 13) PA_MBT(13); else PA_MBT(17);
diff --git a/mm-dti_amd/csrc/pair_attn_bwd_gs16.hip b/mm-dti_amd/csrc/pair_attn_bwd_gs16.hip
--- /dev/null
+++ b/mm-dti_amd/csrc/pair_attn_bwd_gs16.hip
@@ -0,0 +1,42 @@
+#include "pair_attn_bwd_mfma.h"
+
+MMDTI_DEFINE_SALT_PULL(pair_attn_bwd_gs16)
+
+namespace mmdti {
+void pa_bwd_compact_launch_gs16(int nqb, dim3 grid, dim3 blk, hipStream_t st, const void* qkv_bf16, const void* s, const void* do_bf16, void* g,
+                                void* dqkv_bf16, int N, int H, int ld, float scale, int g_in_zero, uint32_t th8, float sc,
+                                unsigned long long seed, unsigned int site, const int* key_tiles, const int* row_off, int qkv_f16, float* gbound) {
+  pa_bwd_compact_launch<pa_sf16>(nqb, grid, blk, st, qkv_bf16, s, do_bf16, g, dqkv_bf16, N, H, ld, scale, g_in_zero, th8, sc, seed, site, key_tiles, row_off, qkv_f16,
+                                 gbound);
+}
+
+__global__ __launch_bounds__(256) void pair_g_decode_kernel(const _Float16* __restrict__ g, const float* __restrict__ bound, float* __restrict__ out,
+                                                            int N, long long planes) {
+  const int n4 = pair_n4(N);
+  const long long plane = pair_plane(N), quads = plane >> 2;
+  const long long idx = (long long)blockIdx.x * 256 + threadIdx.x;
+  if (idx >= planes * quads) return;
+  const long long bh = idx / quads;
+  const int off = (int)(idx - bh * quads) << 2;
+  f32x4 v = {0.f, 0.f, 0.f, 0.f};
+  if (off < N * n4) {
+    const int qb = off / (16 * n4), rem = off - qb * 16 * n4, vr = min(16, N - 16 * qb);
+    const int q = 16 * qb + (rem % (4 * vr)) / 4;
+    v = pa_load4(reinterpret_cast<const pa_sf16*>(g) + bh * plane + off, pa_sf16_dec(bound[bh * N + q]));
+  }
+  *reinterpret_cast<f32x4*>(out + bh * plane + off) = v;
+}
+}
+using namespace mmdti;
+
+extern "C" int mmdti_pair_g_decode(mmdti_stream_t stream, const void* g_sf16, void* out_f32, int B, int N, int H) {
+  MMDTI_REQUIRE(B > 0 && N > 0 && H > 0 && N <= 16 * PA_MAX_NT, "pair_g_decode: B,N,H must be positive and N <= 272 (tiled planes)");
+  MMDTI_REQUIRE(g_sf16 && out_f32 && aligned16(g_sf16) && aligned16(out_f32), "pair_g_decode: null or unaligned pointer");
+  const long long planes = (long long)B * H, total = planes * (pair_plane(N) >> 2);
+  MMDTI_REQUIRE((total + 255) / 256 <= 2147483647LL, "pair_g_decode: grid too large");
+  const float* bound = reinterpret_cast<const float*>(reinterpret_cast<const _Float16*>(g_sf16) + planes * pair_plane(N));
+  hipLaunchKernelGGL(pair_g_decode_kernel, dim3((unsigned)((total + 255) / 256)), dim3(256), 0, (hipStream_t)stream, (const _Float16*)g_sf16, bound,
+                     (float*)out_f32, N, planes);
+  MMDTI_LAUNCH_CHECK();
+  return MMDTI_OK;
+}
diff --git a/mm-dti_amd/csrc/pair_attn_bwd_mfma.h b/mm-dti_amd/csrc/pair_attn_bwd_mfma.h
--- a/mm-dti_amd/csrc/pair_attn_bwd_mfma.h
+++ b/mm-dti_amd/csrc/pair_attn_bwd_mfma.h
@@ -1,5 +1,9 @@
 #pragma once
 #include "pair_attn.h"
+
+#ifndef PA_LA_SF16
+#define PA_LA_SF16 5
+#endif
 
 namespace mmdti {
 
@@ -9,7 +13,8 @@
                                                                  bf16_t* __restrict__ dqkv, int N, int H, int ld, float scale,
                                                                  int g_in_zero, uint32_t thresh, float dscale, uint64_t seed,
                                                                  uint32_t site, const int* __restrict__ key_tiles,
-                                                                 const int* __restrict__ row_off, int qkv_f16) {
+                                                                 const int* __restrict__ row_off, int qkv_f16, float* __restrict__ gbound) {
+  constexpr bool SCALED = std::is_same<GT, pa_sf16>::value;
   static_assert(TILED || (sizeof(ST) == 4 && sizeof(GT) == 4), "compact pair tensors exist in the tiled layout only");
   static_assert(!RAG || sizeof(ST) == 2, "key-tile skipping is built for the compact layout only");
   constexpr int NP = NT * 16;
@@ -124,6 +129,7 @@
     lsum += __shfl_xor(lsum, 32, 64);
     const float inv = lsum > 0.f ? 1.0f / lsum : 0.f;
     float dl = 0.f;
+    float dpmax = 0.f;
 #pragma unroll
     for (int t = 0; t < KT; ++t) {
       {
@@ -143,22 +149,40 @@
         } else {
           dl += dp[0] * pr[0] + dp[1] * pr[1] + dp[2] * pr[2] + dp[3] * pr[3];
         }
+        if constexpr (SCALED) {
+          dpmax = fmaxf(fmaxf(dpmax, fabsf(dp[0])), fabsf(dp[1]));
+          dpmax = fmaxf(fmaxf(dpmax, fabsf(dp[2])), fabsf(dp[3]));
+          asm volatile("" : "+v"(dpmax));
+        }
         P[t] = pr;
       }
     }
     dl += __shfl_xor(dl, 16, 64);
     dl += __shfl_xor(dl, 32, 64);
-    constexpr int PA_LA = 3;
-    auto load_gin = [&](int t) -> f32x4 {
+    float genc = 0.f, gdec = 0.f;
+    if constexpr (SCALED) {
+      dpmax = fmaxf(dpmax, __shfl_xor(dpmax, 16, 64));
+      dpmax = fmaxf(dpmax, __shfl_xor(dpmax, 32, 64));
+      float* bp = gbound + (long long)bh * N + (qvalid ? qi : 0);
+      const float bin = g_in_zero ? 0.f : *bp;
+      const float bout = bin + (2.015625f * dpmax) * inv;
+      if (qvalid && g == 0) *bp = bout;
+      gdec = pa_sf16_dec(bin);
+      genc = pa_sf16_enc(bout);
+    }
+    constexpr int PA_LA = SCALED ? PA_LA_SF16 : 3;
+    typedef typename pa_rawq<GT>::type rawq;
+    const rawq rawz = {};
+    auto load_gin = [&](int t) -> rawq {
       if (PA_FAST(t)) {
-        const f32x4 ld4 = pa_load4_nt(gin_p + (g_in_zero ? 0 : t * TSTEP + goff));
-        return g_in_zero ? f32x4{0.f, 0.f, 0.f, 0.f} : ld4;
+        const rawq ld4 = pa_load4_raw_nt(gin_p + (g_in_zero ? 0 : t * TSTEP + goff));
+        return g_in_zero ? rawz : ld4;
       }
       const bool inrow = PA_PRED(t) && !g_in_zero;
-      const f32x4 ld4 = pa_load4(gin_p + (inrow ? t * TSTEP + goff : 0));
-      return inrow ? ld4 : f32x4{0.f, 0.f, 0.f, 0.f};
+      const rawq ld4 = pa_load4_raw(gin_p + (inrow ? t * TSTEP + goff : 0));
+      return inrow ? ld4 : rawz;
     };
-    f32x4 Gq[PA_LA];
+    rawq Gq[PA_LA];
 #pragma unroll
     for (int t = 0; t < PA_LA && t < KT; ++t) Gq[t] = load_gin(t);
     f32x4 dq = {0.f, 0.f, 0.f, 0.f};
@@ -166,7 +190,7 @@
 #pragma unroll
     for (int t = 0; t < KT; ++t) {
       const int kcol = t * 16 + 4 * g;
-      const f32x4 Gin = Gq[t % PA_LA];
+      const f32x4 Gin = pa_widen_raw(gin_p, Gq[t % PA_LA], gdec);
       if (t + PA_LA < KT) Gq[t % PA_LA] = load_gin(t + PA_LA);
       __builtin_amdgcn_sched_barrier(0);
       const pa_s16x4 va = g < 2 ? *reinterpret_cast<const pa_s16x4*>(sV + (t * 16 + c16) * 8 + 4 * g) : zero4;
@@ -180,10 +204,9 @@
         for (int r = 0; r < 4; ++r) G[r] = (kcol + r < N) ? G[r] : 0.f;
       }
       if (EDGE && !qvalid) G = f32x4{0.f, 0.f, 0.f, 0.f};
-      if (PA_FAST(t)) {
-        pa_store4_nt(gout_p + t * TSTEP + goff, G);
-      } else if (PA_PRED(t)) {
-        pa_store4_nt(gout_p + t * TSTEP + goff, G);
+      if (PA_FAST(t) || PA_PRED(t)) {
+        if constexpr (SCALED) pa_store4_nt(gout_p + t * TSTEP + goff, G, genc);
+        else pa_store4_nt(gout_p + t * TSTEP + goff, G);
       }
       f32x4 Pd;
 #pragma unroll
@@ -269,11 +292,12 @@
 template <typename GT>
 static inline void pa_bwd_compact_launch(int nqb, dim3 grid, dim3 blk, hipStream_t st, const void* qkv_bf16, const void* s, const void* do_bf16,
                                          void* g, void* dqkv_bf16, int N, int H, int ld, float scale, int g_in_zero, uint32_t th8, float sc,
-                                         unsigned long long seed, unsigned int site, const int* key_tiles, const int* row_off, int qkv_f16) {
+                                         unsigned long long seed, unsigned int site, const int* key_tiles, const int* row_off, int qkv_f16,
+                                         float* gbound = nullptr) {
 #define PA_MBH(NT, NWV, RG)                                                                                                   \
   hipLaunchKernelGGL((pair_attn_bwd_mfma_kernel<NT, true, true, NWV, RG, _Float16, GT>), grid, blk, 0, st, (const bf16_t*)qkv_bf16, \
                      (const _Float16*)s, (const bf16_t*)do_bf16, (const GT*)g, (GT*)g, (bf16_t*)dqkv_bf16, N, H, ld, scale,    \
-                     g_in_zero, th8, sc, (uint64_t)seed, (uint32_t)site, key_tiles, row_off, qkv_f16)
+                     g_in_zero, th8, sc, (uint64_t)seed, (uint32_t)site, key_tiles, row_off, qkv_f16, gbound)
 #define PA_MBC(NT)                                                                                   \
   case NT:                                                                                           \
     if (key_tiles) PA_MBH(NT, ((NT % 3 == 0 || NT >= 16 || NT == 5) ? 3 : 4), true);                 \
@@ -289,5 +313,8 @@
 void pa_bwd_compact_launch_g16(int nqb, dim3 grid, dim3 blk, hipStream_t st, const void* qkv_bf16, const void* s, const void* do_bf16, void* g,
                                void* dqkv_bf16, int N, int H, int ld, float scale, int g_in_zero, uint32_t th8, float sc,
                                unsigned long long seed, unsigned int site, const int* key_tiles, const int* row_off, int qkv_f16);
+void pa_bwd_compact_launch_gs16(int nqb, dim3 grid, dim3 blk, hipStream_t st, const void* qkv_bf16, const void* s, const void* do_bf16, void* g,
+                                void* dqkv_bf16, int N, int H, int ld, float scale, int g_in_zero, uint32_t th8, float sc,
+                                unsigned long long seed, unsigned int site, const int* key_tiles, const int* row_off, int qkv_f16, float* gbound);
 
 }
diff --git a/mm-dti_amd/mmdti_hip/functional.py b/mm-dti_amd/mmdti_hip/functional.py
--- a/mm-dti_amd/mmdti_hip/functional.py
+++ b/mm-dti_amd/mmdti_hip/functional.py
@@ -101,8 +101,11 @@
     return paths.Switches(LAYER_SEQ, STACK_SEQ, STACK_MAX_ROWS, ops.GROUPED_DW, ops.GROUPED_DW_MIN_ROWS, ops.FWD_F16, bool(ops.kernel_timer.names))
 
 
-def _pair_grad_chain(s, key_tiles):
-    return (torch.empty if key_tiles is None else torch.zeros)(s.shape, device=s.device, dtype=ops.pair_grad_dtype(s))
+def _pair_grad_chain(s, key_tiles, N):
+    dt = ops.pair_grad_dtype(s)
+    if dt == torch.float16:
+        return ops.pair_g_alloc(s.shape[0], s.shape[1], N, s.device, zero=key_tiles is not None)
+    return (torch.empty if key_tiles is None else torch.zeros)(s.shape, device=s.device, dtype=dt)
 
 
 def _kept(L, li, plan):
@@ -296,7 +299,7 @@
             if paths.unimol_layer_bwd(seq_path, dx16 is not None, hold, full[li]) == paths.LAYER:
                 g_zero = G is None
                 if g_zero:
-                    G = _pair_grad_chain(L.s, st.kt)
+                    G = _pair_grad_chain(L.s, st.kt, N)
                 dx, dx16 = _unimol_layer_bwd_seq(st, layer, L, dx, dx16, G, g_zero, scale, seq_ws,
                                                  None if (li == 0 or lowest) else (below[li - 1], gbuf(mod.layers[li - 1].fc2.bias)))
                 L.__dict__.clear()
@@ -313,7 +316,7 @@
             do = ops.linear_bwd_input(dy1, wbf16(att.out_proj.weight))
             g_zero = G is None
             if g_zero:
-                G = _pair_grad_chain(L.s, st.kt)
+                G = _pair_grad_chain(L.s, st.kt, N)
             dqkv = ops.pair_attn_bwd(L.qkv, L.s, do, G, B, N, H, ld, scale, g_zero, st.p_att, seed, L.site_att, key_tiles=st.kt, row_off=st.row_off)
             _wgrad(dqkv, L.h1, att.in_proj.weight, att.in_proj.bias)
             if lowest and not (ln1.weight.requires_grad or ln1.bias.requires_grad):
@@ -346,7 +349,7 @@
         if not ctx.needs_input_grad[1]:
             G = None
         elif G is None:
-            G = torch.zeros_like(st.bias0)
+            G = torch.zeros_like(st.bias0, dtype=F32 if st.bias0.dtype == torch.float16 else st.bias0.dtype)
         if G is not None and st.slot is not None:
             st.slot.g = G
             G = torch.zeros((), device=G.device, dtype=torch.float16).expand(G.shape)
@@ -532,8 +535,8 @@
     T = S.T
     M, D = st.M, st.D
     dev = dx.device
-    G = _pair_grad_chain(S.s_last, st.kt)
-    layout = ops._pair_layout_s(S.s_last, "pair_attn_bwd.s") | (4 if G.dtype == BF16 else 0)
+    G = _pair_grad_chain(S.s_last, st.kt, st.N)
+    layout = ops._pair_layout_s(S.s_last, "pair_attn_bwd.s") | ops.pair_layout_g_bits(S.s_last, G, st.B, st.N, st.H)
     dx_final = torch.empty_like(dx)
     ws = torch.empty(S.ws_bytes, device=dev, dtype=torch.uint8)
     side, events = _stack_side()
@@ -591,7 +594,7 @@
     M, D, F = st.M, st.D, layer.fc1.weight.shape[0]
     dx_out = torch.empty_like(dx)
     dx16_out = torch.empty(M, D, device=dx.device, dtype=BF16) if below is not None else None
-    layout = ops._pair_layout_s(L.s, "pair_attn_bwd.s") | (4 if G.dtype == BF16 else 0)
+    layout = ops._pair_layout_s(L.s, "pair_attn_bwd.s") | ops.pair_layout_g_bits(L.s, G, st.B, st.N, st.H)
     p = ops._p
     ops.lib().mmdti_unimol_layer_bwd(
         ops._stream(), M, st.B, st.N, st.H, D, F, st.ld, float(scale), float(st.p_res), float(st.p_att), int(st.seed),
@@ -658,9 +661,13 @@
             if chain is None:
                 g = g.float()
             elif real:
+                if chain.dtype == torch.float16:
+                    chain = ops.pair_g_decode(chain)
                 g = chain.float().add_(g) if chain.dtype != F32 else chain.add_(g)
             else:
                 g = chain
+            if g.dtype == torch.float16 and not st.full:
+                g = ops.pair_g_decode(g)
         if st.full:
             l1, l2 = proj.linear1, proj.linear2
             allp = [l1.weight, l1.bias, l2.weight, l2.bias] + ps
@@ -700,6 +707,8 @@
     def backward(ctx, g):
         chain, ctx.slot.g = ctx.slot.g, None
         real = any(sd != 0 for sd in g.stride())
+        if chain is not None and chain.dtype == torch.float16:
+            chain = ops.pair_g_decode(chain)
         if chain is None:
             chain = g.float()
         elif real:
diff --git a/mm-dti_amd/mmdti_hip/ops.py b/mm-dti_amd/mmdti_hip/ops.py
--- a/mm-dti_amd/mmdti_hip/ops.py
+++ b/mm-dti_amd/mmdti_hip/ops.py
@@ -522,10 +522,41 @@
 
 PAIR_COMPACT = os.environ.get("MMDTI_PAIR_COMPACT", "1") != "0"
 PAIR_G_BF16 = os.environ.get("MMDTI_PAIR_G_BF16", "0") == "1"
+PAIR_G_SF16 = os.environ.get("MMDTI_PAIR_G_SF16", "1") != "0"
 
 
 def pair_grad_dtype(s):
-    return BF16 if (s.dtype == F16 and PAIR_G_BF16) else F32
+    if s.dtype != F16:
+        return F32
+    return BF16 if PAIR_G_BF16 else (F16 if PAIR_G_SF16 else F32)
+
+
+def pair_g_alloc(B, H, N, device, zero=False):
+    n = B * H * pair_plane(N)
+    flat = (torch.zeros if zero else torch.empty)(n + 2 * B * H * N, device=device, dtype=F16)
+    g = flat[:n].view(B, H, pair_plane(N))
+    if not zero and pair_plane(N) != N * pair_ld(N):
+        g[:, :, N * pair_ld(N):] = 0
+    return g
+
+
+def pair_g_bounds(g):
+    if g.dtype != F16 or g.dim() != 3 or not g.is_contiguous() or g.storage_offset() != 0:
+        raise MMDTIError("pair_g_bounds: not a gradient chain from pair_g_alloc")
+    B, H, plane = g.shape
+    st = g.untyped_storage()
+    rest = st.nbytes() - 2 * B * H * plane
+    N = rest // (4 * B * H)
+    if rest <= 0 or rest != 4 * B * H * N or pair_plane(N) != plane:
+        raise MMDTIError("pair_g_bounds: not a gradient chain from pair_g_alloc (no row bounds behind the planes)")
+    return torch.empty(0, device=g.device, dtype=F32).set_(st, B * H * plane // 2, (B, H, N))
+
+
+def pair_g_decode(g):
+    B, H, N = pair_g_bounds(g).shape
+    out = torch.empty(g.shape, device=g.device, dtype=F32)
+    lib().mmdti_pair_g_decode(_stream(), g.data_ptr(), out.data_ptr(), B, N, H)
+    return out
 
 
 def _pair_layout_s(s, what):
@@ -540,6 +571,11 @@
 
 def _pair_layout_g(g, what):
     tiled = pair_is_tiled(g)
+    if g.dtype == F16:
+        if what != "gbf_bias_bwd_full":
+            raise MMDTIError(f"{what}: does not read the row-scaled fp16 gradient chain (decode it: pair_g_decode)")
+        pair_g_bounds(g)
+        return 9
     if g.dtype == BF16:
         if not tiled:
             raise MMDTIError(f"{what}: bf16 pair gradients exist in the tiled layout only")
@@ -618,6 +654,14 @@
     return s_out, o
 
 
+def pair_layout_g_bits(s, g, B, N, H):
+    if pair_is_tiled(g) != pair_is_tiled(s) or not (g.dtype == F32 or (g.dtype in (BF16, F16) and s.dtype == F16)):
+        raise MMDTIError("pair_attn_bwd: S and G must share one pair layout (fp32 gradients, or bf16 / row-scaled fp16 gradients with fp16 logits)")
+    if g.dtype == F16 and tuple(pair_g_bounds(g).shape) != (B, H, N):
+        raise MMDTIError("pair_attn_bwd: the row bounds of the row-scaled fp16 gradient chain do not match B, H, N")
+    return 4 if g.dtype == BF16 else (8 if g.dtype == F16 else 0)
+
+
 def pair_attn_bwd(qkv, s, do, g, B, N, H, ld, scale, g_in_zero, drop_p=0.0, seed=0, site=0, key_tiles=None, row_off=None):
     if (row_off is None and qkv.shape[0] != B * N) or do.shape[0] != qkv.shape[0]:
         raise MMDTIError("pair_attn_bwd: qkv / do row counts do not match the layout")
@@ -628,10 +672,7 @@
         qkv = to_bf16(qkv)
     dqkv = torch.empty(qkv.shape, device=qkv.device, dtype=BF16)
     layout = _pair_layout_s(s, "pair_attn_bwd.s")
-    if pair_is_tiled(g) != tiled or not (g.dtype == F32 or (g.dtype == BF16 and s.dtype == F16)):
-        raise MMDTIError("pair_attn_bwd: S and G must share one pair layout (fp32 gradients, or bf16 gradients with fp16 logits)")
-    if g.dtype == BF16:
-        layout |= 4
+    layout |= pair_layout_g_bits(s, g, B, N, H)
     t0 = kernel_timer.begin("pair_attn_bwd")
     lib().mmdti_pair_attn_bwd(_stream(), qkv.data_ptr(), s.data_ptr(), do.data_ptr(), g.data_ptr(), dqkv.data_ptr(), B, N, H, ld,
                               float(scale), int(g_in_zero), float(drop_p), int(seed), int(site), layout, _p(key_tiles), _p(row_off), int(qkv.dtype == F16))
```

Result: no change. 5054, median of 6 (+0.8%).
